# ducha-aiki/affnet

Hardware: AMD Instinct MI355X
Metric: keypoints/sec (detect+AffNet+OriNet+HardNet) per image, 2000 kp @1024x768 (higher is better)
Workload: dtype f32

## Files before the change

affnet_amd/SparseImgRepresenter.py:

```python
import ctypes as C

import torch
import torch.nn as nn

from . import _lib, engine
from ._lib import lib, check, ptr
from .architectures import _HipPatchNet
from .HandCraftedModules import AffineShapeEstimator, OrientationDetector, _HipHandCrafted
from .HardNet import HardTFeatNet
from .pytorch_sift import SIFTNet

_FOLLOW = (SIFTNet, HardTFeatNet)


class ScaleSpaceAffinePatchExtractor(nn.Module):
    def __init__(self, border=16, num_features=500, patch_size=32, mrSize=3.0, nlevels=3, num_Baum_iters=0,
                 init_sigma=1.6, th=None, RespNet=None, OriNet=None, AffNet=None, arith="fp32"):
        super(ScaleSpaceAffinePatchExtractor, self).__init__()
        self.arith = arith
        _lib.arith_code(arith)
        self.mrSize, self.PS, self.b = mrSize, patch_size, border
        self.num, self.nlevels = num_features, nlevels
        self.num_Baum_iters, self.init_sigma = num_Baum_iters, init_sigma
        self.th = th
        if th is not None:
            self.num = -1
        else:
            self.th = 0
        self.RespNet = RespNet
        if not 1 <= nlevels <= 6:
            raise NotImplementedError("nlevels must be 1..6 (levels per octave = nlevels + 2 <= 8)")
        self.OriNet = OriNet if OriNet is not None else OrientationDetector(patch_size=19)
        self.AffNet = AffNet if AffNet is not None else AffineShapeEstimator(patch_size=19)
        self.scale_pyr = self.sigmas = self.pix_dists = None
        self._ctx = None
        self._ctx_key = None
        self._fctx = self._fctx_key = self._pyr_ctx = None
        self.last_ids = None
        self.max_keep = 16384
        self.raw_div = 4
        self.lazy_shape_rows = -1

    def _context(self, x, allow_batch=False):
        engine.require_cuda(x, "image")
        if x.dim() != 4 or x.size(1) != 1 or x.size(0) < 1 or (x.size(0) != 1 and not allow_batch):
            raise ValueError("expected a (1,1,H,W) image; forward() is batch-size-1 like the reference "
                             "(HandCraftedModules.py:283-284) - use enqueue()/run_batch() for (B,1,H,W) batches")
        pre = int(1.5 * self.num) if self.num_Baum_iters > 0 else self.num
        key = (x.size(0), x.size(2), x.size(3), x.device, pre, self.num, float(self.th), self.mrSize, self.b, self.init_sigma,
               self.nlevels, self.max_keep, self.num_Baum_iters, self.raw_div, self.lazy_shape_rows)
        if self._ctx is not None and self._ctx_key == key and self._ctx.arith != _lib.arith_code(self.arith):
            self._ctx.set_arith(self.arith)
        if self._ctx is None or self._ctx_key != key:
            self._ctx = engine.Context(x.size(2), x.size(3), x.device, self.nlevels, self.init_sigma, self.b, self.mrSize,
                                       float(self.th), self.num, pre, self.max_keep, batch=x.size(0), baum_iters=self.num_Baum_iters, raw_div=self.raw_div,
                                       lazy_shape_rows=self.lazy_shape_rows, arith=self.arith)
            self._ctx_key = key
        return self._ctx

    def _publish_pyramid(self, ctx):
        self._pyr_ctx = ctx
        self.scale_pyr = ctx.pyramid_views()
        self.sigmas = [list(s) for s in ctx.plan.sigmas]
        self.pix_dists = [list(p) for p in ctx.plan.pix_dists]

    def _response_pyramid(self, ctx, img):
        dev = img.device
        st = engine.stream_of(dev)
        check(lib.affnet_pyramid_build(ctx.handle, ptr(img), st), ctx.handle, "affnet_pyramid_build")
        stride = lib.affnet_pyramid_image_stride(ctx.handle)
        base = lib.affnet_pyramid_level_offset(ctx.handle, 0, 0)
        resp = torch.zeros(ctx.batch * stride, dtype=torch.float32, device=dev)
        with torch.no_grad():
            for b in range(ctx.batch):
                pyr = ctx.pyramid_views(b)
                for o, (h, w) in enumerate(ctx.plan.sizes):
                    for l in range(ctx.plan.levels_per_octave):
                        off = b * stride + lib.affnet_pyramid_level_offset(ctx.handle, o, l) - base
                        r = self.RespNet(pyr[o][l], ctx.plan.sigmas[o][l])
                        resp[off:off + h * w].copy_(r.reshape(-1).to(dev, torch.float32))
        return resp

    @staticmethod
    def _native(slot):
        return slot is None or isinstance(slot, (_HipPatchNet, _HipHandCrafted))

    def enqueue(self, x, do_ori=False, desc=None, det_stream=None, input_ready=None):
        ctx = self._context(x, allow_batch=True)
        dev = x.device
        if not (self._native(self.AffNet) and self._native(self.OriNet)):
            raise NotImplementedError("the fused path needs the native AffNetFast / OriNetFast slots (foreign slots: forward())")
        img = x.contiguous().float()
        B, F = x.size(0), ctx.cap_final
        lafs = torch.empty(B, F, 2, 3, dtype=torch.float32, device=dev)
        resp = torch.empty(B, F, dtype=torch.float32, device=dev)
        ids = torch.empty(B, F, 3, dtype=torch.int32, device=dev)
        count = torch.zeros(B, dtype=torch.int32, device=dev)
        dsc = torch.empty(B, F, 128, dtype=torch.float32, device=dev) if desc is not None else None
        nets = self._nets(dev, do_ori, desc)
        follow = isinstance(desc, _FOLLOW)
        if isinstance(desc, HardTFeatNet):
            desc.check_usable()
        fused_dsc = None if follow else dsc
        if self.RespNet is not None:
            rmaps = self._response_pyramid(ctx, img)
            check(lib.affnet_detect_image_responses(ctx.handle, ptr(rmaps), engine.stream_of(dev)), ctx.handle, "affnet_detect_image_responses")
            rc = lib.affnet_describe_detected(ctx.handle, C.byref(nets), int(bool(do_ori)), ptr(lafs), ptr(resp), ptr(ids), ptr(fused_dsc),
                                              ptr(count), engine.stream_of(dev))
            check(rc, ctx.handle, "affnet_describe_detected")
        elif det_stream is None:
            rc = lib.affnet_extract_features(ctx.handle, C.byref(nets), ptr(img), int(bool(do_ori)), ptr(lafs), ptr(resp), ptr(ids),
                                             ptr(fused_dsc), ptr(count), engine.stream_of(dev))
            check(rc, ctx.handle, "affnet_extract_features")
        else:
            cur = torch.cuda.current_stream(dev)
            if input_ready is None:
                det_stream.wait_stream(cur)
            elif input_ready is not False:
                det_stream.wait_event(input_ready)
            if getattr(self, "_busy", None) is not None:
                det_stream.wait_event(self._busy)
            rc = lib.affnet_detect_image(ctx.handle, ptr(img), C.c_void_p(det_stream.cuda_stream))
            check(rc, ctx.handle, "affnet_detect_image")
            ev = torch.cuda.Event()
            ev.record(det_stream)
            cur.wait_event(ev)
            rc = lib.affnet_describe_detected(ctx.handle, C.byref(nets), int(bool(do_ori)), ptr(lafs), ptr(resp), ptr(ids), ptr(fused_dsc),
                                              ptr(count), engine.stream_of(dev))
            check(rc, ctx.handle, "affnet_describe_detected")
            self._busy = torch.cuda.Event()
            self._busy.record(cur)
        if follow:
            self._desc_follow(ctx, desc, lafs, count, dsc)
            if det_stream is not None:
                self._busy = torch.cuda.Event()
                self._busy.record(torch.cuda.current_stream(dev))
        if B == 1:
            lafs, resp, ids, dsc = lafs[0], resp[0], ids[0], (None if dsc is None else dsc[0])
        return {"LAFs": lafs, "responses": resp, "ids": ids, "descriptors": dsc, "count": count, "overflow": ctx.counter_view(0), "_img": img}

    def _desc_follow(self, ctx, desc, lafs, count, dsc):
        dev, (B, F) = lafs.device, lafs.shape[:2]
        st = engine.stream_of(dev)
        lvl = torch.empty(B, F, 3, dtype=torch.int32, device=dev)
        norm = torch.empty(B, F, 2, 3, dtype=torch.float32, device=dev)
        check(lib.affnet_level_select(ctx.handle, ptr(lafs), ptr(count), F, desc.PS, ptr(lvl), ptr(norm), st), ctx.handle, "affnet_level_select")
        if isinstance(desc, HardTFeatNet):
            floats = lib.affnet_tfeat_scratch_floats(B * F)
            cached = getattr(self, "_tfeat_scratch", None)
            if cached is None or cached.device != dev or cached.numel() < floats:
                cached = self._tfeat_scratch = torch.empty(floats, dtype=torch.float32, device=dev)
            check(lib.affnet_tfeat_forward_pyr(ctx.handle, ptr(desc.packed_weights(dev)), ptr(norm), ptr(lvl), ptr(count), F, ptr(dsc), ptr(cached), st),
                  ctx.handle, "affnet_tfeat_forward_pyr")
            return
        check(lib.affnet_sift_forward_pyr(ctx.handle, ptr(norm), ptr(lvl), ptr(count), F, ptr(desc.window(dev)), float(desc.clipval), ptr(dsc), st),
              ctx.handle, "affnet_sift_forward_pyr")

    def _nets(self, dev, do_ori, desc):
        nets = _lib.Nets()
        if self.num_Baum_iters > 0:
            if isinstance(self.AffNet, _HipHandCrafted):
                nets.h_baumberg_window = C.cast(self.AffNet.window(), C.c_void_p)
            else:
                nets.d_affnet = self.AffNet.packed_weights(dev).data_ptr()
        if do_ori:
            if isinstance(self.OriNet, _HipHandCrafted):
                nets.h_orientation_window = C.cast(self.OriNet.window(), C.c_void_p)
            else:
                nets.d_orinet = self.OriNet.packed_weights(dev).data_ptr()
        nets.d_hardnet = desc.packed_weights(dev).data_ptr() if desc is not None and not isinstance(desc, _FOLLOW) else None
        return nets

    def capture(self, x, do_ori=False, desc=None):
        if isinstance(desc, _FOLLOW):
            raise NotImplementedError("graph capture covers the fused C call (HardNet descriptors or none); the SIFT and HardTFeat descriptors "
                                      "follow it as further launches - use enqueue() / run()")
        return CapturedPath(self, x, do_ori, desc)

    def run_batch(self, x, do_ori=False, desc=None):
        r = self.enqueue(x, do_ori=do_ori, desc=desc)
        ctx = self._ctx
        ctx.read_counts(allow_empty=True)
        cnt = r["count"].cpu().tolist()
        if x.size(0) == 1:
            r = {k: (v.unsqueeze(0) if isinstance(v, torch.Tensor) and k not in ("count", "overflow", "_img") else v) for k, v in r.items()}
        out = []
        for b, n in enumerate(cnt):
            dsc = r["descriptors"]
            out.append({"LAFs": r["LAFs"][b, :n], "responses": r["responses"][b, :n], "ids": r["ids"][b, :n],
                        "descriptors": None if dsc is None else dsc[b, :n]})
        return out

    def run(self, x, do_ori=False, desc=None):
        if x.dim() == 4 and x.size(0) != 1:
            raise ValueError("run() is for a single (1,1,H,W) image; use run_batch() for (B,1,H,W) batches")
        r = self.enqueue(x, do_ori=do_ori, desc=desc)
        ctx = self._ctx
        self._publish_pyramid(ctx)
        n = int(ctx.read_counts()[1])
        self.last_ids = r["ids"][:n]
        dsc = r["descriptors"]
        return {"LAFs": r["LAFs"][:n], "responses": r["responses"][:n], "ids": r["ids"][:n],
                "descriptors": None if dsc is None else dsc[:n]}

    def _frames_context(self, x, n_max):
        engine.require_cuda(x, "image")
        if x.dim() != 4 or x.size(1) != 1 or x.size(0) < 1:
            raise ValueError("expected a (B,1,H,W) image batch")
        budget = self.num if (0 < self.num < n_max and self.num_Baum_iters > 0) else n_max
        key = (x.size(0), x.size(2), x.size(3), x.device, n_max, budget, self.mrSize, self.b, self.init_sigma, self.nlevels, self.num_Baum_iters,
               self.raw_div, self.lazy_shape_rows)
        if self._fctx is not None and self._fctx_key == key and self._fctx.arith != _lib.arith_code(self.arith):
            self._fctx.set_arith(self.arith)
        if self._fctx is None or self._fctx_key != key:
            self._fctx = engine.Context(x.size(2), x.size(3), x.device, self.nlevels, self.init_sigma, self.b, self.mrSize, float(self.th), budget, n_max,
                                        self.max_keep, batch=x.size(0), baum_iters=self.num_Baum_iters, raw_div=self.raw_div,
                                        lazy_shape_rows=self.lazy_shape_rows, arith=self.arith)
            self._fctx_key = key
        return self._fctx

    def enqueue_frames(self, x, LAFs, responses=None, counts=None, do_ori=True, desc=None):
        if not (self._native(self.AffNet) and self._native(self.OriNet)):
            raise NotImplementedError("the fused path needs the native AffNetFast / OriNetFast slots (foreign slots: getAffineShape / getOrientation)")
        engine.require_cuda(x, "image")
        engine.require_cuda(LAFs, "LAFs")
        dev, B = x.device, x.size(0)
        fr = LAFs.contiguous().float()
        if fr.dim() == 3:
            fr = fr.unsqueeze(0)
        if fr.dim() != 4 or fr.size(0) != B or tuple(fr.shape[2:]) != (2, 3):
            raise ValueError("LAFs must be (n,2,3) for one image or (B,n_max,2,3) for a (B,1,H,W) batch, got %s" % (tuple(LAFs.shape),))
        n_max = fr.size(1)
        if n_max == 0:
            fr, responses, counts, n_max = torch.zeros(B, 1, 2, 3, dtype=torch.float32, device=dev), None, [0] * B, 1
        rin = None
        if responses is not None:
            engine.require_cuda(responses, "responses")
            rin = responses.contiguous().float().view(B, n_max)
        cin = None
        if counts is not None:
            cin = counts if isinstance(counts, torch.Tensor) else torch.tensor(list(counts), dtype=torch.int32)
            cin = cin.to(dev, torch.int32).contiguous().view(B)
        ctx = self._frames_context(x, n_max)
        img = x.contiguous().float()
        F = ctx.cap_final
        lafs = torch.empty(B, F, 2, 3, dtype=torch.float32, device=dev)
        resp = torch.empty(B, F, dtype=torch.float32, device=dev)
        ids = torch.empty(B, F, 3, dtype=torch.int32, device=dev)
        count = torch.zeros(B, dtype=torch.int32, device=dev)
        dsc = torch.empty(B, F, 128, dtype=torch.float32, device=dev) if desc is not None else None
        nets = self._nets(dev, do_ori, desc)
        follow = isinstance(desc, _FOLLOW)
        if isinstance(desc, HardTFeatNet):
            desc.check_usable()
        rc = lib.affnet_describe_frames(ctx.handle, C.byref(nets), ptr(img), ptr(fr), ptr(rin), ptr(cin), n_max, int(bool(do_ori)), ptr(lafs), ptr(resp),
                                        ptr(ids), None if follow else ptr(dsc), ptr(count), engine.stream_of(dev))
        check(rc, ctx.handle, "affnet_describe_frames")
        if follow:
            self._desc_follow(ctx, desc, lafs, count, dsc)
        self._publish_pyramid(ctx)
        if B == 1:
            lafs, resp, ids, dsc = lafs[0], resp[0], ids[0], (None if dsc is None else dsc[0])
        return {"LAFs": lafs, "responses": resp, "ids": ids, "descriptors": dsc, "count": count, "overflow": ctx.counter_view(0), "_img": img,
                "_frames": (fr, rin, cin)}

    def describe_frames(self, x, LAFs, responses=None, counts=None, do_ori=True, desc=None):
        r = self.enqueue_frames(x, LAFs, responses=responses, counts=counts, do_ori=do_ori, desc=desc)
        ctx = self._fctx
        dsc = r["descriptors"]
        if x.size(0) == 1:
            n = int(ctx.read_counts()[1])
            self.last_ids = r["ids"][:n]
            return {"LAFs": r["LAFs"][:n], "responses": r["responses"][:n], "ids": r["ids"][:n], "descriptors": None if dsc is None else dsc[:n]}
        ctx.read_counts(allow_empty=True)
        return [{"LAFs": r["LAFs"][b, :n], "responses": r["responses"][b, :n], "ids": r["ids"][b, :n],
                 "descriptors": None if dsc is None else dsc[b, :n]} for b, n in enumerate(r["count"].cpu().tolist())]

    def _pyramid_ctx(self):
        ctx = self._pyr_ctx
        if ctx is None or self.scale_pyr is None:
            raise RuntimeError("call forward() / run() first: the pyramid of the last image is reused (stateful like the reference)")
        if ctx.batch != 1:
            raise RuntimeError("getAffineShape / getOrientation work on the pyramid of a single image")
        return ctx

    def _shape_stage(self, ctx, resp, lafs, ids, cnt, n):
        dev, st = lafs.device, engine.stream_of(lafs.device)
        P, F = ctx.cap_pre, ctx.cap_final
        PS = self.AffNet.PS
        patches = torch.empty(n, 1, PS, PS, dtype=torch.float32, device=dev)

        def shape_pass(frames):
            check(lib.affnet_pyr_grid_sample(ctx.handle, ptr(frames), ptr(ids), ptr(cnt), n, PS, ptr(patches), st), ctx.handle,
                  "affnet_pyr_grid_sample")
            with torch.no_grad():
                a = torch.cat([self.AffNet(patches[s:s + 256], {}) for s in range(0, n, 256)], 0)
            full = torch.zeros(P, 2, 2, dtype=torch.float32, device=dev)
            full[:n] = a.to(dev, torch.float32)
            return full
        A = shape_pass(lafs)
        if self.num_Baum_iters > 1:
            frames = torch.empty(P, 2, 3, dtype=torch.float32, device=dev)
            for _ in range(1, self.num_Baum_iters):
                check(lib.affnet_shape_iterate(ctx.handle, None, ptr(A), ptr(lafs), ptr(cnt), 0, ptr(frames), st), ctx.handle, "affnet_shape_iterate")
                Ai = shape_pass(frames)
                check(lib.affnet_shape_iterate(ctx.handle, ptr(Ai), ptr(A), ptr(lafs), ptr(cnt), 1, ptr(frames), st), ctx.handle, "affnet_shape_iterate")
        r2 = torch.empty(F, dtype=torch.float32, device=dev)
        l2 = torch.empty(F, 2, 3, dtype=torch.float32, device=dev)
        i2 = torch.empty(F, 3, dtype=torch.int32, device=dev)
        c2 = torch.zeros(1, dtype=torch.int32, device=dev)
        check(lib.affnet_shape_filter_select(ctx.handle, ptr(resp), ptr(lafs), ptr(ids), ptr(A), ptr(cnt), ptr(r2), ptr(l2),
                                             ptr(i2), ptr(c2), st), ctx.handle, "affnet_shape_filter_select")
        return r2, l2, i2, c2, int(c2.item())

    def _orientation_stage(self, ctx, lafs, ids, cnt, n):
        dev, st = lafs.device, engine.stream_of(lafs.device)
        PS = self.OriNet.PS
        patches = torch.empty(n, 1, PS, PS, dtype=torch.float32, device=dev)
        if n:
            check(lib.affnet_pyr_grid_sample(ctx.handle, ptr(lafs), ptr(ids), ptr(cnt), n, PS, ptr(patches), st), ctx.handle,
                  "affnet_pyr_grid_sample")
        with torch.no_grad():
            ang = self.OriNet(patches)
        if ang.dim() <= 2:
            c, s = torch.cos(ang).view(-1, 1, 1), torch.sin(ang).view(-1, 1, 1)
            ang = torch.cat([torch.cat([c, s], 2), torch.cat([-s, c], 2)], 1)
        R = ang.to(dev, torch.float32).contiguous()
        if n:
            check(lib.affnet_apply_rotation(ctx.handle, ptr(lafs), ptr(R), ptr(cnt), n, st), ctx.handle, "affnet_apply_rotation")

    @staticmethod
    def _frame_rows(ctx, LAFs, pyr_idxs, level_idxs, cap):
        engine.require_cuda(LAFs, "LAFs")
        dev, n = LAFs.device, LAFs.size(0)
        if n > cap:
            raise ValueError("%d frames, the context of the last forward() holds %d rows" % (n, cap))
        lafs = torch.zeros(cap, 2, 3, dtype=torch.float32, device=dev)
        lafs[:n] = LAFs.float()
        ids = torch.zeros(cap, 3, dtype=torch.int32, device=dev)
        ids[:n, 0] = torch.as_tensor(pyr_idxs).to(dev).view(-1).to(torch.int32)
        ids[:n, 1] = torch.as_tensor(level_idxs).to(dev).view(-1).to(torch.int32)
        ids[:n, 2] = torch.arange(n, dtype=torch.int32, device=dev)
        return lafs, ids, torch.full((1,), n, dtype=torch.int32, device=dev), n

    def getAffineShape(self, final_resp, LAFs, final_pyr_idxs, final_level_idxs, num_features=0):
        ctx = self._pyramid_ctx()
        if self.num_Baum_iters <= 0:
            raise ValueError("getAffineShape needs num_Baum_iters > 0 (the reference's loop body never runs otherwise, SparseImgRepresenter.py:127)")
        if num_features != self.num and not (num_features <= 0 and self.num <= 0):
            raise ValueError("num_features = %d: the context of the last forward() is sized for the extractor's own budget (%d)" % (num_features, self.num))
        lafs, ids, cnt, n = self._frame_rows(ctx, LAFs, final_pyr_idxs, final_level_idxs, ctx.cap_pre)
        resp = torch.zeros(ctx.cap_pre, dtype=torch.float32, device=lafs.device)
        resp[:n] = final_resp.to(lafs.device, torch.float32).view(-1)
        resp, lafs, ids, cnt, n = self._shape_stage(ctx, resp, lafs, ids, cnt, n)
        self.last_ids = ids[:n]
        return resp[:n], lafs[:n], ids[:n, 0].long(), ids[:n, 1].long()

    def getOrientation(self, LAFs, final_pyr_idxs, final_level_idxs):
        ctx = self._pyramid_ctx()
        lafs, ids, cnt, n = self._frame_rows(ctx, LAFs, final_pyr_idxs, final_level_idxs, LAFs.size(0))
        self._orientation_stage(ctx, lafs, ids, cnt, n)
        return lafs

    def _staged(self, x, do_ori):
        ctx = self._context(x)
        dev, st = x.device, engine.stream_of(x.device)
        img = x.contiguous().float()
        P = ctx.cap_pre
        rmaps = None
        if self.RespNet is not None:
            rmaps = self._response_pyramid(ctx, img)
        else:
            check(lib.affnet_pyramid_build(ctx.handle, ptr(img), st), ctx.handle, "affnet_pyramid_build")
        self._publish_pyramid(ctx)
        resp = torch.empty(P, dtype=torch.float32, device=dev)
        lafs = torch.empty(P, 2, 3, dtype=torch.float32, device=dev)
        ids = torch.empty(P, 3, dtype=torch.int32, device=dev)
        cnt = torch.zeros(1, dtype=torch.int32, device=dev)
        if rmaps is not None:
            check(lib.affnet_detect_responses(ctx.handle, ptr(rmaps), ptr(resp), ptr(lafs), ptr(ids), ptr(cnt), st), ctx.handle,
                  "affnet_detect_responses")
        else:
            check(lib.affnet_detect(ctx.handle, ptr(resp), ptr(lafs), ptr(ids), ptr(cnt), st), ctx.handle, "affnet_detect")
        n = int(cnt.item())
        ctx.read_counts()
        if self.num_Baum_iters > 0:
            resp, lafs, ids, cnt, n = self._shape_stage(ctx, resp, lafs, ids, cnt, n)
        if do_ori:
            self._orientation_stage(ctx, lafs, ids, cnt, n)
        out = torch.empty_like(lafs)
        check(lib.affnet_scale_lafs(ctx.handle, ptr(lafs), ptr(out), ptr(cnt), lafs.size(0), x.size(3), x.size(2), 0, st), ctx.handle,
              "affnet_scale_lafs")
        self.last_ids = ids[:n]
        return out[:n], resp[:n]

    def forward(self, x, do_ori=False):
        aff_native = self.num_Baum_iters == 0 or self._native(self.AffNet)
        ori_native = (not do_ori) or self._native(self.OriNet)
        if aff_native and ori_native:
            r = self.run(x, do_ori=do_ori)
            return r["LAFs"], r["responses"]
        return self._staged(x, do_ori)

    def extract_patches_from_pyr(self, dLAFs, PS=41):
        if self._ctx is None or self.scale_pyr is None:
            raise RuntimeError("call forward() first: the pyramid of the last image is reused (stateful like the reference)")
        ctx = self._ctx
        if ctx.batch != 1:
            raise RuntimeError("extract_patches_from_pyr works on the pyramid of a single-image forward()")
        engine.require_cuda(dLAFs, "dLAFs")
        dev, st = dLAFs.device, engine.stream_of(dLAFs.device)
        lafs = dLAFs.contiguous().float()
        n = lafs.size(0)
        out = torch.empty(n, 1, PS, PS, dtype=torch.float32, device=dev)
        if n == 0:
            return out
        ids = torch.empty(n, 3, dtype=torch.int32, device=dev)
        norm = torch.empty(n, 2, 3, dtype=torch.float32, device=dev)
        check(lib.affnet_level_select(ctx.handle, ptr(lafs), None, n, PS, ptr(ids), ptr(norm), st), ctx.handle, "affnet_level_select")
        check(lib.affnet_pyr_grid_sample(ctx.handle, ptr(norm), ptr(ids), None, n, PS, ptr(out), st), ctx.handle, "affnet_pyr_grid_sample")
        self.last_level_ids = ids
        return out


class CapturedPath(object):
    def __init__(self, det, x, do_ori, desc):
        if not (det._native(det.AffNet) and det._native(det.OriNet)) or det.RespNet is not None:
            raise NotImplementedError("graph capture needs the native slots (foreign slots run Python between the stages)")
        ctx = det._context(x, allow_batch=True)
        dev = x.device
        self.det, self.ctx, self.do_ori, self.desc = det, ctx, bool(do_ori), desc
        B, F = x.size(0), ctx.cap_final
        self.image = x.contiguous().float().clone()
        self.out = {"LAFs": torch.empty(B, F, 2, 3, dtype=torch.float32, device=dev), "responses": torch.empty(B, F, dtype=torch.float32, device=dev),
                    "ids": torch.empty(B, F, 3, dtype=torch.int32, device=dev), "count": torch.zeros(B, dtype=torch.int32, device=dev),
                    "descriptors": torch.empty(B, F, 128, dtype=torch.float32, device=dev) if desc is not None else None}
        self._nets = det._nets(dev, do_ori, desc)
        self._mods = [m for m in (det.AffNet, det.OriNet if do_ori else None, desc) if m is not None and hasattr(m, "packed_weights")]
        self._blobs = [m.packed_weights(dev) for m in self._mods]
        self._stamps = [m._weights_stamp() for m in self._mods]
        self._arith = ctx.arith
        self._stream = torch.cuda.Stream(device=dev)
        torch.cuda.synchronize(dev)
        o = self.out
        check(lib.affnet_graph_capture_extract(ctx.handle, C.byref(self._nets), ptr(self.image), int(self.do_ori), ptr(o["LAFs"]), ptr(o["responses"]),
                                               ptr(o["ids"]), ptr(o["descriptors"]), ptr(o["count"]), C.c_void_p(self._stream.cuda_stream)),
              ctx.handle, "affnet_graph_capture_extract")

    def launch(self, x=None, check_weights=True):
        if check_weights:
            for m, stamp in zip(self._mods, self._stamps):
                if m._weights_stamp() != stamp:
                    raise RuntimeError("the weights of %s changed after capture(): the graph holds the old packed weights - capture again" % type(m).__name__)
        if self.ctx.arith != self._arith:
            raise RuntimeError("the arithmetic mode of the extractor changed after capture(): the graph runs the mode it was captured with - capture again")
        if x is not None:
            self.image.copy_(x, non_blocking=True)
        busy = getattr(self.det, "_busy", None)
        if busy is not None:
            torch.cuda.current_stream(self.image.device).wait_event(busy)
        check(lib.affnet_graph_launch(self.ctx.handle, engine.stream_of(self.image.device)), self.ctx.handle, "affnet_graph_launch")
        out = dict(self.out, overflow=self.ctx.counter_view(0), _img=self.image)
        if self.image.size(0) == 1:
            return {k: (v[0] if (v is not None and k not in ("count", "overflow", "_img")) else v) for k, v in out.items()}
        return out

    def run(self, x=None, check_weights=True):
        if self.image.size(0) != 1:
            raise ValueError("run() is for single images; use launch() for batches")
        r = self.launch(x, check_weights=check_weights)
        self.det._publish_pyramid(self.ctx)
        n = int(self.ctx.read_counts()[1])
        dsc = r["descriptors"]
        return {"LAFs": r["LAFs"][:n], "responses": r["responses"][:n], "ids": r["ids"][:n], "descriptors": None if dsc is None else dsc[:n]}


def get_geometry_and_descriptors(img, det, desc, do_ori=True):
    from .HardNet import HardNet
    if isinstance(desc, (HardNet,) + _FOLLOW) and det._native(det.AffNet) and det._native(det.OriNet):
        r = det.run(img, do_ori=do_ori, desc=desc)
        return r["LAFs"], r["descriptors"]
    with torch.no_grad():
        LAFs, resp = det(img, do_ori=do_ori)
        patches = det.extract_patches_from_pyr(LAFs, PS=32)
        return LAFs, desc(patches)
```

affnet_amd/_lib.py:

```python
import ctypes as C
import os

_HERE = os.path.dirname(os.path.abspath(__file__))
LIB_PATH = os.environ.get("AFFNET_HIP_LIB") or os.path.join(_HERE, "libaffnet_hip.so")
PROBES_LIB_PATH = os.path.join(_HERE, "libaffnet_hip_probes.so")

MAX_OCTAVES, MAX_LEVELS, MAX_TAPS = 16, 8, 37
NET_AFFNET, NET_ORINET, NET_HARDNET, NET_AFFNET_FULLCONV = 0, 1, 2, 3
ARITH_FP32_MFMA, ARITH_FP32_SPLIT3, ARITH_FP32_SPLIT2H = 0, 1, 2
ARITH_NAMES = {"fp32": ARITH_FP32_MFMA, "fp32_mfma": ARITH_FP32_MFMA, "fp32_split3": ARITH_FP32_SPLIT3, "split3": ARITH_FP32_SPLIT3,
               "fp32_split2h": ARITH_FP32_SPLIT2H, "split2h": ARITH_FP32_SPLIT2H}


def arith_code(arith):
    if arith is None:
        return ARITH_FP32_MFMA
    if isinstance(arith, str):
        if arith.lower() not in ARITH_NAMES:
            raise ValueError("arith must be one of %s" % sorted(ARITH_NAMES))
        return ARITH_NAMES[arith.lower()]
    if int(arith) not in (ARITH_FP32_MFMA, ARITH_FP32_SPLIT3, ARITH_FP32_SPLIT2H):
        raise ValueError("arith must be AFFNET_ARITH_FP32_MFMA (0), AFFNET_ARITH_FP32_SPLIT3 (1) or AFFNET_ARITH_FP32_SPLIT2H (2)")
    return int(arith)
OK, ERR_INVALID, ERR_HIP, ERR_CAPACITY, ERR_EMPTY = 0, -1, -2, -3, -4


class Config(C.Structure):
    _fields_ = [
        ("height", C.c_int32), ("width", C.c_int32), ("n_octaves", C.c_int32), ("levels_per_octave", C.c_int32),
        ("oct_h", C.c_int32 * MAX_OCTAVES), ("oct_w", C.c_int32 * MAX_OCTAVES),
        ("level_sigma", (C.c_float * MAX_LEVELS) * MAX_OCTAVES),
        ("level_sigma4", (C.c_float * MAX_LEVELS) * MAX_OCTAVES),
        ("level_sigma_px", (C.c_double * MAX_LEVELS) * MAX_OCTAVES),
        ("first_blur_taps", C.c_int32), ("first_blur", C.c_float * (MAX_TAPS * MAX_TAPS)),
        ("level_blur_taps", C.c_int32 * MAX_LEVELS),
        ("level_blur", (C.c_float * (MAX_TAPS * MAX_TAPS)) * MAX_LEVELS),
        ("level_blur0_taps", C.c_int32 * MAX_LEVELS),
        ("level_blur0", (C.c_float * (MAX_TAPS * MAX_TAPS)) * MAX_LEVELS),
        ("lazy_shape_rows", C.c_int32),
        ("onepass", C.c_int32),
        ("mr_size", C.c_float), ("threshold", C.c_float),
        ("num_features", C.c_int32), ("num_prefilter", C.c_int32),
        ("max_raw_per_octave_div", C.c_int32), ("max_keep", C.c_int32), ("batch", C.c_int32), ("baum_iters", C.c_int32),
        ("arith", C.c_int32),
    ]


class Nets(C.Structure):
    _fields_ = [("d_affnet", C.c_void_p), ("d_orinet", C.c_void_p), ("d_hardnet", C.c_void_p),
                ("h_orientation_window", C.c_void_p), ("h_baumberg_window", C.c_void_p)]


_P, _I, _SZ = C.c_void_p, C.c_int, C.c_size_t
SYMBOLS = {
    "affnet_config_fill": (_I, [C.POINTER(Config), _I, _I, _I, C.c_double, _I, C.c_double, C.c_double, _I, _I, _I, _I]),
    "affnet_ctx_create": (_I, [C.POINTER(_P), _I, C.POINTER(Config)]),
    "affnet_ctx_destroy": (None, [_P]),
    "affnet_last_error": (C.c_char_p, [_P]),
    "affnet_version": (C.c_char_p, []),
    "affnet_set_arith": (_I, [_P, _I]),
    "affnet_get_arith": (_I, [_P]),
    "affnet_workspace_bytes": (_SZ, [_P]),
    "affnet_bind_workspace": (_I, [_P, _P, _SZ]),
    "affnet_pyramid_level_offset": (C.c_int64, [_P, _I, _I]),
    "affnet_pyramid_image_stride": (C.c_int64, [_P]),
    "affnet_batch": (_I, [_P]),
    "affnet_capacity_prefilter": (_I, [_P]),
    "affnet_capacity_final": (_I, [_P]),
    "affnet_gauss_blur": (_I, [_P, _P, _P, _I, _I, C.POINTER(C.c_float), _I, _P]),
    "affnet_pyramid_build": (_I, [_P, _P, _P]),
    "affnet_hessian_response": (_I, [_P, _P, _P, _I, _I, C.c_float, _P]),
    "affnet_detect": (_I, [_P, _P, _P, _P, _P, _P]),
    "affnet_detect_responses": (_I, [_P, _P, _P, _P, _P, _P, _P]),
    "affnet_laf_grid_sample": (_I, [_P, _P, _I, _I, _P, _I, _I, _P, _P]),
    "affnet_pyr_grid_sample": (_I, [_P, _P, _P, _P, _I, _I, _P, _P]),
    "affnet_cnn32_packed_floats": (_SZ, [_I]),
    "affnet_cnn32_winograd_offset": (C.c_int64, [_I, _I]),
    "affnet_cnn32_pack_weights": (_I, [_I, C.POINTER(_P), C.POINTER(_P), C.POINTER(_P), _P, _P, _P, _P, _P]),
    "affnet_cnn32_forward": (_I, [_P, _I, _P, _P, _P, _I, _P, _P, _P]),
    "affnet_cnn32_forward_pyr": (_I, [_P, _I, _P, _P, _P, _P, _I, _P, _P, _P]),
    "affnet_local_norm": (_I, [_P, _P, _P, _I, _I, _P]),
    "affnet_fullconv_scratch_bytes": (_SZ, [_I, _I]),
    "affnet_fullconv_forward": (_I, [_P, _P, _P, _I, _I, _P, _P, _P]),
    "affnet_nms2d": (_I, [_P, _P, _P, _I, _I, C.c_float, _P]),
    "affnet_shape_filter_select": (_I, [_P, _P, _P, _P, _P, _P, _P, _P, _P, _P, _P]),
    "affnet_apply_rotation": (_I, [_P, _P, _P, _P, _I, _P]),
    "affnet_scale_lafs": (_I, [_P, _P, _P, _P, _I, _I, _I, _I, _P]),
    "affnet_lafs_to_ellipses": (_I, [_P, _P, _P, _I, _P, _P]),
    "affnet_ellipses_to_lafs": (_I, [_P, _P, _P, _I, _P, _P]),
    "affnet_level_select": (_I, [_P, _P, _P, _I, _I, _P, _P, _P]),
    "affnet_handcrafted_forward": (_I, [_P, _I, _P, _I, _P, _P, _P, _P]),
    "affnet_handcrafted_forward_pyr": (_I, [_P, _I, _P, _P, _P, _I, _P, _P, _P]),
    "affnet_sift_host_window": (_I, [_I, C.POINTER(C.c_float)]),
    "affnet_sift_forward": (_I, [_P, _P, _I, _P, C.c_float, _P, _P]),
    "affnet_sift_forward_pyr": (_I, [_P, _P, _P, _P, _I, _P, C.c_float, _P, _P]),
    "affnet_tfeat_packed_floats": (_SZ, []),
    "affnet_tfeat_pack_weights": (_I, [_P, _P, _P, _P, _P, _P, _P]),
    "affnet_tfeat_scratch_floats": (_SZ, [_I]),
    "affnet_tfeat_forward": (_I, [_P, _P, _P, _P, _I, _P, _P, _P]),
    "affnet_tfeat_forward_pyr": (_I, [_P, _P, _P, _P, _P, _I, _P, _P, _P]),
    "affnet_match_scratch_bytes": (_SZ, [_I, _I]),
    "affnet_distance_matrix": (_I, [_P, _P, _I, _P, _I, _I, _P, _P, _P]),
    "affnet_match_snn": (_I, [_P, _P, _I, _P, _I, _I, C.c_float, _P, _P, _P, _P, _P, _P, _P]),
    "affnet_reproject_lafs": (_I, [_P, _P, _I, C.POINTER(C.c_float), _P, _P]),
    "affnet_centre_nn": (_I, [_P, _P, _I, _P, _I, _P, _P, _P]),
    "affnet_extract_features": (_I, [_P, C.POINTER(Nets), _P, _I, _P, _P, _P, _P, _P, _P]),
    "affnet_detect_image": (_I, [_P, _P, _P]),
    "affnet_detect_image_responses": (_I, [_P, _P, _P]),
    "affnet_detect_image_onepass": (_I, [_P, _P, _P, _P]),
    "affnet_detect_image_onepass_responses": (_I, [_P, _P, _P, _P]),
    "affnet_detected_list": (_I, [_P, _P, _P, _P, _P, _P]),
    "affnet_load_frames": (_I, [_P, _P, _I, _P, _P, _P, _I, _I, _P]),
    "affnet_describe_frames": (_I, [_P, C.POINTER(Nets), _P, _P, _P, _P, _I, _I, _P, _P, _P, _P, _P, _P]),
    "affnet_shape_iterate": (_I, [_P, _P, _P, _P, _P, _I, _P, _P]),
    "affnet_affmap_offset": (C.c_int64, [_P, _I]),
    "affnet_affmap_image_stride": (C.c_int64, [_P]),
    "affnet_describe_detected": (_I, [_P, C.POINTER(Nets), _I, _P, _P, _P, _P, _P, _P]),
    "affnet_graph_capture_extract": (_I, [_P, C.POINTER(Nets), _P, _I, _P, _P, _P, _P, _P, _P]),
    "affnet_graph_launch": (_I, [_P, _P]),
    "affnet_profile_enable": (_I, [_P, _I]),
    "affnet_profile_read": (_I, [_P, C.POINTER(C.c_double * 8), C.POINTER(C.c_int32)]),
    "affnet_read_counts": (_I, [_P, C.POINTER(C.c_int32 * 4), _P]),
    "affnet_counter_offset": (C.c_int64, [_P, _I]),
    "affnet_counter_stride": (C.c_int64, [_P]),
    "affnet_host_base_grid": (_I, [_I, C.POINTER(C.c_float)]),
}

DEBUG_SYMBOLS = {
    "affnet_cnn32_debug_timing": (_I, [_P, _P]),
    "affnet_cnn32_debug_layer": (_I, [_P, _I, _P, _P, _I, _P, _P]),
    "affnet_cnn32_debug_winograd_u": (_I, [_P, _I, _P, _I, _P, _P]),
    "affnet_selftest_mfma": (_I, [_P, _P, _P, _P]),
    "affnet_debug_split3_variant": (_I, [_P, _I]),
}

PROBE_SYMBOLS = {
    "affnet_cnn32_probe": (_I, [_P, _I, _I, _I, _I, _P, _P]),
    "affnet_split3_gemm": (_I, [_P, _P, _I, _I, _I, _I, _P, _P]),
    "affnet_split3_rate": (_I, [_I, _I, _I, _P, _P]),
    "affnet_debug_stream": (_I, [_P, _P, _SZ, _I, _I, _I, _P]),
}


class AffnetHipError(RuntimeError):
    pass


class AffnetEmptyError(AffnetHipError):
    """AFFNET_ERR_EMPTY: no image of the call produced a detection (the reference raises in torch.cat([]),
    SparseImgRepresenter.py:100)."""


def _load():
    if not os.path.isfile(LIB_PATH):
        if os.path.basename(LIB_PATH) == os.path.basename(PROBES_LIB_PATH):
            raise ImportError("affnet_amd: %s is missing - the tools under tools/ need the probe build of the library: "
                              "AFFNET_PROBES=1 bash affnet_amd/csrc/build.sh" % LIB_PATH)
        raise ImportError(
            "affnet_amd: %s is missing - the HIP extension is the only implementation of this path "
            "(no CPU fallback). Build it: bash affnet_amd/csrc/build.sh" % LIB_PATH)
    lib = C.CDLL(LIB_PATH)
    for table in (SYMBOLS, DEBUG_SYMBOLS):
        for name, (res, args) in table.items():
            fn = getattr(lib, name)
            fn.restype, fn.argtypes = res, args
    for name, (res, args) in PROBE_SYMBOLS.items():
        if hasattr(lib, name):
            fn = getattr(lib, name)
            fn.restype, fn.argtypes = res, args
    return lib


lib = _load()


def check(rc, ctx=None, what=""):
    if rc != OK:
        msg = lib.affnet_last_error(ctx).decode() if ctx else ""
        if rc == ERR_EMPTY:
            raise AffnetEmptyError("%s: %s" % (what or "libaffnet_hip call", msg))
        raise AffnetHipError("%s failed (code %d): %s" % (what or "libaffnet_hip call", rc, msg))


def ptr(t):
    return None if t is None else C.c_void_p(t.data_ptr())


def current_stream(device):
    import torch
    return C.c_void_p(torch.cuda.current_stream(device).cuda_stream)
```

affnet_amd/csrc/cnn32.hip:

```cpp
#include "common.h"

static void aff_fill_pyr_src(const affnet_ctx* ctx, PyrSrc* s) {
    memset(s, 0, sizeof(*s));
    if (ctx->ws) aff_fill_pyr_table(ctx, &s->t);
    aff_base_grid(32, s->base);
}

static int cnn_check(affnet_ctx* ctx, const CnnCall& c, int* rows) {
    *rows = 0;
    if (c.kind < 0 || c.kind > 2) return aff_fail(ctx, AFFNET_ERR_INVALID, "cnn32: unknown net kind %d", c.kind);
    if (!c.packed || !c.out || c.n_max < 0 || (!c.patches && (!c.lafs || !c.ids))) return aff_fail(ctx, AFFNET_ERR_INVALID, "cnn32: null argument");
    if (!c.patches && !ctx->ws) return aff_fail(ctx, AFFNET_ERR_INVALID, "cnn32: sampling from the pyramid needs a bound workspace");
    if (c.dbg_layer < 0 && !c.scratch)
        return aff_fail(ctx, AFFNET_ERR_INVALID, "cnn32: d_scratch is required (HardNet n*(8192+512) floats, AffNet / OriNet n*144 floats)");
    if (c.dbg_layer >= 0 && ctx->arith != AFFNET_ARITH_FP32_MFMA)
        return aff_fail(ctx, AFFNET_ERR_INVALID, "cnn32: layer dumps exist for AFFNET_ARITH_FP32_MFMA only (context is in arithmetic mode %d)", ctx->arith);
    if (c.n_max == 0) return AFFNET_OK;
    if (c.kind == AFFNET_NET_HARDNET && c.n_max > 65535)
        return aff_fail(ctx, AFFNET_ERR_INVALID, "cnn32: n_max=%d (HardNet head: max 65535 rows per image)", c.n_max);
    const int row_count = c.row_count < 0 ? c.n_max - c.row_begin : c.row_count;
    if (c.row_begin < 0 || row_count < 0 || c.row_begin + row_count > c.n_max) return aff_fail(ctx, AFFNET_ERR_INVALID, "cnn32: bad row window");
    *rows = row_count;
    return AFFNET_OK;
}

int aff_arith_index(const affnet_ctx* ctx) {
    return ctx->arith == AFFNET_ARITH_FP32_SPLIT2H ? 2 : (ctx->arith == AFFNET_ARITH_FP32_SPLIT3 ? 1 : 0);
}

static int trunk_launch(affnet_ctx* ctx, const CnnCall& c, const NetLayout& L, dim3 grid) {
    CnnArgs a;
    a.packed = c.packed; a.off = to_offsets(L, ctx->arith);
    a.wino_u = nullptr;
    if (c.kind == AFFNET_NET_ORINET && ctx->arith == AFFNET_ARITH_FP32_MFMA) {
        const int rc = aff_wino_derive_u(ctx, c.kind, c.packed, L, c.st, &a.wino_u);
        if (rc) return rc;
    }
    a.patches = c.patches; a.lafs = c.lafs; a.ids = c.ids; a.count = c.count; a.n_max = c.n_max;
    a.out = (c.dbg_layer < 0) ? c.scratch : c.out;
    a.dbg_layer = c.dbg_layer; a.dbg_out = c.dbg_out; a.dbg_time = ctx->dbg_time;
    a.row_begin = c.row_begin; a.skip_cnt = c.skip_cnt; a.skip_n = c.skip_n;
    a.shape_cnt = (c.fuse && c.shape_op) ? c.fuse->cnt : nullptr; a.shape_op = c.shape_op;
    a.s3_alt = ctx->split3_variant;
    PyrSrc ps;
    aff_fill_pyr_src(ctx, &ps);
    static_assert(AFFNET_NET_AFFNET == 0 && AFFNET_NET_ORINET == 1 && AFFNET_NET_HARDNET == 2, "trunk getter order");
    static TrunkKernel (*const trunk_of[3])(int, bool) = {aff_trunk_affnet, aff_trunk_orinet, aff_trunk_hardnet};
    hipLaunchKernelGGL(trunk_of[c.kind](aff_arith_index(ctx), a.dbg_time || c.dbg_layer >= 0), grid, dim3(512), 0, c.st, a, ps);
    AFF_LAUNCH_CHECK(ctx);
    return AFFNET_OK;
}

static int cnn_launch(affnet_ctx* ctx, const CnnCall& c) {
    int rows;
    int rc = cnn_check(ctx, c, &rows);
    if (rc || rows == 0) return rc;
    const NetLayout L = net_layout(c.kind);
    const int B = c.patches ? 1 : ctx->B;
    rc = trunk_launch(ctx, c, L, dim3(rows, B));
    if (rc) return rc;
    if (c.dbg_layer < 0 && c.kind != AFFNET_NET_HARDNET) {
        rc = c.kind == AFFNET_NET_AFFNET ? aff_finish_affnet(ctx, c, L, rows, B) : aff_finish_orinet(ctx, c, L, rows, B);
        if (rc) return rc;
    }
    if (c.mark_head) aff_prof_mark(ctx, 7, c.st);
    if (c.dbg_layer < 0 && c.kind == AFFNET_NET_HARDNET) return aff_hardnet_head(ctx, c, L, B);
    return AFFNET_OK;
}

extern "C" int affnet_cnn32_forward(affnet_ctx* ctx, int net_kind, const float* d_packed, const float* d_patches, const int32_t* d_count,
                                    int n_max, float* d_out, float* d_scratch, void* stream) {
    AFF_DEVICE(ctx);
    if (!ctx || !d_patches) return aff_fail(ctx, AFFNET_ERR_INVALID, "cnn32_forward: null argument");
    CnnCall c;
    c.kind = net_kind; c.packed = d_packed; c.patches = d_patches; c.count = d_count; c.n_max = n_max; c.out = d_out; c.scratch = d_scratch; c.st = (hipStream_t)stream;
    return cnn_launch(ctx, c);
}

extern "C" int affnet_cnn32_forward_pyr(affnet_ctx* ctx, int net_kind, const float* d_packed, const float* d_lafs, const int32_t* d_ids,
                                        const int32_t* d_count, int n_max, float* d_out, float* d_scratch, void* stream) {
    AFF_DEVICE(ctx);
    if (!ctx) return AFFNET_ERR_INVALID;
    CnnCall c;
    c.kind = net_kind; c.packed = d_packed; c.lafs = d_lafs; c.ids = d_ids; c.count = d_count; c.n_max = n_max; c.out = d_out; c.scratch = d_scratch; c.st = (hipStream_t)stream;
    return cnn_launch(ctx, c);
}

int aff_affnet_filter_rows(affnet_ctx* ctx, const float* packed, const float* resp, const float* lafs, const int32_t* ids, const int32_t* count,
                           float* out, float* scratch, int row_begin, int row_count, bool lazy, int shape_op, hipStream_t st) {
    ShapeFuse sf;
    sf.resp = resp; sf.lafs = lafs; sf.key = ctx->st_key; sf.good = ctx->st_good; sf.cnt = ctx->cnt;
    CnnCall c;
    c.kind = AFFNET_NET_AFFNET; c.packed = packed; c.lafs = lafs; c.ids = ids; c.count = count; c.n_max = ctx->cap_pre; c.out = out; c.scratch = scratch; c.st = st;
    c.row_begin = row_begin; c.row_count = row_count;
    c.skip_cnt = lazy ? ctx->cnt : nullptr; c.skip_n = ctx->cfg.num_features;
    c.fuse = &sf; c.shape_op = shape_op;
    return cnn_launch(ctx, c);
}

int aff_orinet_rotate(affnet_ctx* ctx, const float* packed, float* lafs, const int32_t* ids, const int32_t* count, int n_max, float* out, float* scratch,
                      hipStream_t st, const DenormSel* denorm) {
    CnnCall c;
    c.kind = AFFNET_NET_ORINET; c.packed = packed; c.lafs = lafs; c.ids = ids; c.count = count; c.n_max = n_max; c.out = out; c.scratch = scratch; c.st = st;
    c.rot_lafs = lafs; c.denorm = denorm;
    return cnn_launch(ctx, c);
}

int aff_hardnet_forward_pyr_marked(affnet_ctx* ctx, const float* packed, const float* lafs, const int32_t* ids, const int32_t* count,
                                   int n_max, float* out, float* scratch, hipStream_t st) {
    CnnCall c;
    c.kind = AFFNET_NET_HARDNET; c.packed = packed; c.lafs = lafs; c.ids = ids; c.count = count; c.n_max = n_max; c.out = out; c.scratch = scratch; c.st = st;
    c.mark_head = true;
    return cnn_launch(ctx, c);
}

extern "C" int affnet_debug_split3_variant(affnet_ctx* ctx, int bits) {
    if (!ctx) return AFFNET_ERR_INVALID;
    ctx->split3_variant = bits;
    return AFFNET_OK;
}

extern "C" int affnet_cnn32_debug_timing(affnet_ctx* ctx, unsigned long long* d_stamps) {
    if (!ctx) return AFFNET_ERR_INVALID;
    ctx->dbg_time = d_stamps;
    return AFFNET_OK;
}

extern "C" int affnet_cnn32_debug_layer(affnet_ctx* ctx, int net_kind, const float* d_packed, const float* d_patch, int layer, float* d_out,
                                        void* stream) {
    AFF_DEVICE(ctx);
    if (!ctx || !d_patch || !d_out || layer < 0 || layer > 5) return aff_fail(ctx, AFFNET_ERR_INVALID, "cnn32_debug_layer: bad argument");
    CnnCall c;
    c.kind = net_kind; c.packed = d_packed; c.patches = d_patch; c.n_max = 1; c.out = d_out; c.st = (hipStream_t)stream;
    c.dbg_layer = layer; c.dbg_out = d_out;
    return cnn_launch(ctx, c);
}

extern "C" int affnet_cnn32_debug_winograd_u(affnet_ctx* ctx, int net_kind, const float* d_packed, int layer, float* d_out, void* stream) {
    AFF_DEVICE(ctx);
    if (!ctx || !d_packed || !d_out || (net_kind != AFFNET_NET_AFFNET && net_kind != AFFNET_NET_ORINET) || (layer != 1 && layer != 3 && layer != 5))
        return aff_fail(ctx, AFFNET_ERR_INVALID, "cnn32_debug_winograd_u: AffNet / OriNet, layer 1, 3 or 5");
    const float* u;
    const int rc = aff_wino_derive_u(ctx, net_kind, d_packed, net_layout(net_kind), (hipStream_t)stream, &u);
    if (rc) return rc;
    return aff_copy_async(ctx, d_out, u + Wino16::offset(layer), (size_t)Wino16::floats(layer) * sizeof(float), (hipStream_t)stream);
}
```

affnet_amd/csrc/cnn_heads.hip:

```cpp
#include <stdlib.h>

#include "common.h"

#include "cnn_mfma.h"
#include "shape_filter.h"

__global__ __launch_bounds__(256) void affnet_finish_kernel(const float* __restrict__ part, const float* __restrict__ hb,
                                                            const int32_t* __restrict__ count, int n_max, float* __restrict__ out, int row_begin,
                                                            int row_end, const int32_t* __restrict__ skip_cnt, int skip_n, ShapeFuse sf) {
    const int row = row_begin + blockIdx.x * 256 + threadIdx.x;
    const int n_img = count ? min(count[blockIdx.y], n_max) : n_max;
    const int n = min(n_img, row_end);
    const bool skip = lazy_skip(skip_cnt, skip_n, blockIdx.y);
    const size_t pidx = (size_t)blockIdx.y * n_max + row;
    if (sf.key) {
        if (blockIdx.x == 0 && threadIdx.x == 0)
            sf.cnt[(size_t)blockIdx.y * CNT_TOTAL + CNT_AFF_EVAL] = skip ? min(n_img, row_begin) : min(n_img, row_end);
        if (skip && row < n) { sf.key[pidx] = 0.0f; sf.good[pidx] = 0; }
    }
    if (row >= n || skip) return;
    float* o = out + 4 * pidx;
    const f32x4* pp = reinterpret_cast<const f32x4*>(part + pidx * HEAD_PART_AFF);
    f32x4 r[8];
#pragma unroll
    for (int w = 0; w < 8; ++w) r[w] = pp[w];
    const f32x4 s = ((r[0] + r[1]) + (r[2] + r[3])) + ((r[4] + r[5]) + (r[6] + r[7]));
    const float x0 = tanhf(s.x + hb[0]), x1 = tanhf(s.y + hb[1]), x2 = tanhf(s.z + hb[2]);
    const float a00 = 1.0f + x0, a01 = 0.0f * x0, a10 = x1, a11 = 1.0f + x2;
    const float det = sqrtf(fabsf(a00 * a11 - a10 * a01 + 1e-10f));
    const float b2a2 = sqrtf(a01 * a01 + a00 * a00);
    const float o0 = b2a2 / det, o1 = 0.0f * det, o2 = (a11 * a01 + a10 * a00) / (b2a2 * det), o3 = det / b2a2;
    o[0] = o0; o[1] = o1; o[2] = o2; o[3] = o3;
    if (sf.key) {
        const size_t bi = blockIdx.y;
        aff_shape_filter_row(sf.resp + bi * n_max, sf.lafs + bi * n_max * 6, o0, o1, o2, o3, row, sf.key + bi * n_max, sf.good + bi * n_max,
                             sf.cnt + bi * CNT_TOTAL);
    }
}

__global__ __launch_bounds__(256) void orinet_finish_kernel(const float* __restrict__ part, const float* __restrict__ hb,
                                                            const int32_t* __restrict__ count, int n_max, float* __restrict__ out, int row_begin,
                                                            int row_end, float* __restrict__ rot_lafs, DenormSel ds) {
    const int row = row_begin + blockIdx.x * 4 + (threadIdx.x >> 6), lane = threadIdx.x & 63;
    const int n = min(count ? min(count[blockIdx.y], n_max) : n_max, row_end);
    if (row >= n) {
        if (ds.out_px && row < n_max && lane < 6) ds.out_px[6 * ((size_t)blockIdx.y * n_max + row) + lane] = 0.f;
        return;
    }
    const size_t pidx = (size_t)blockIdx.y * n_max + row;
    const float* pp = part + pidx * HEAD_PART_ORI;
    float th = 0.f;
    if (lane < 18) {
        float p[8];
#pragma unroll
        for (int w = 0; w < 8; ++w) p[w] = pp[w * 18 + lane];
        float r = 0.f;
#pragma unroll
        for (int w = 0; w < 8; w += 2) r += p[w] + p[w + 1];
        th = tanhf(r + hb[lane >= 9 ? 1 : 0]);
    }
    float t0 = 0.f, t1 = 0.f;
#pragma unroll
    for (int q = 0; q < 9; ++q) { t0 += __shfl(th, q, 64); t1 += __shfl(th, 9 + q, 64); }
    if (lane != 0 && !(rot_lafs && ds.out_px)) return;
    const float yv = t0 / 9.0f, xv = t1 / 9.0f;
    const float ang = atan2f(yv + 1e-8f, xv + 1e-8f);
    const float sn = sinf(ang), cs = cosf(ang);
    float* o = out + 4 * pidx;
    if (lane == 0) { o[0] = cs; o[1] = sn; o[2] = -sn; o[3] = cs; }
    if (rot_lafs) {
        float* L = rot_lafs + 6 * pidx;
        const float l00 = L[0], l01 = L[1], l10 = L[3], l11 = L[4], lx = L[2], ly = L[5];
        const float r0 = fmaf(l01, -sn, l00 * cs), r1 = fmaf(l01, cs, l00 * sn), r3 = fmaf(l11, -sn, l10 * cs), r4 = fmaf(l11, cs, l10 * sn);
        if (ds.out_px)
            aff_denorm_level_row_wave(lane, r0, r1, lx, r3, r4, ly, ds.c_a, ds.c_x, ds.c_y, ds.ps, ds.lt, ds.ca, ds.cx, ds.cy, ds.out_px + 6 * pidx, ds.ids + 3 * pidx,
                                      ds.lafs_norm + 6 * pidx);
        if (lane == 0) { L[0] = r0; L[1] = r1; L[3] = r3; L[4] = r4; }
    }
}

template <int MP>
__global__ __launch_bounds__(256, 2) void hardnet_head_kernel(const float* __restrict__ trunk, const float* __restrict__ Bw,
                                                              const int32_t* __restrict__ count, int n_max, float* __restrict__ partial) {
    constexpr int MI = MP / 16;
    constexpr int NA = MP * HEAD_KC / 4 / 256;
    __shared__ __attribute__((aligned(16))) float As[MP * HEAD_AS];
    const int n = count ? min(count[blockIdx.z], n_max) : n_max;
    const int p0 = blockIdx.x * MP;
    if (p0 >= n) return;
    const size_t rows_total = (size_t)gridDim.z * n_max;
    const int kbeg = blockIdx.y * (HEAD_K / HEAD_KSPLIT);
    const int tid = threadIdx.x, wave = tid >> 6, lane = tid & 63;
    const int m = lane & 15, kq = lane >> 4;
    const __amdgpu_buffer_rsrc_t rA = weight_rsrc(trunk + (size_t)blockIdx.z * n_max * HEAD_K, n * HEAD_K);
    const __amdgpu_buffer_rsrc_t rB = weight_rsrc(Bw, HEAD_K * 128);
    int offA[NA];
#pragma unroll
    for (int r = 0; r < NA; ++r) {
        const int f = tid + 256 * r, row = f >> 5, c4 = f & 31;
        offA[r] = ((p0 + row) * HEAD_K + 4 * c4) * 4;
    }
    const int offB = ((kq * 128) + wave * 32 + m) * 16;
    const unsigned a_addr = lds_byte_addr(As) + (m * HEAD_AS + 4 * kq) * 4;
    f32x4 acc[MI][2], stage[NA];
#pragma unroll
    for (int i = 0; i < MI; ++i)
#pragma unroll
        for (int j = 0; j < 2; ++j) acc[i][j] = (f32x4){0.f, 0.f, 0.f, 0.f};
#pragma unroll
    for (int r = 0; r < NA; ++r) stage[r] = buf_read4(rA, offA[r], kbeg * 4);
#pragma unroll 1
    for (int k0 = kbeg; k0 < kbeg + HEAD_K / HEAD_KSPLIT; k0 += HEAD_KC) {
        __syncthreads();
#pragma unroll
        for (int r = 0; r < NA; ++r) {
            const int f = tid + 256 * r, row = f >> 5, c4 = f & 31;
            *reinterpret_cast<f32x4*>(&As[row * HEAD_AS + 4 * c4]) = stage[r];
        }
        __syncthreads();
        if (k0 + HEAD_KC < kbeg + HEAD_K / HEAD_KSPLIT) {
#pragma unroll
            for (int r = 0; r < NA; ++r) stage[r] = buf_read4(rA, offA[r], (k0 + HEAD_KC) * 4);
        }
        f32x4 fa[2][MI], fb[2][2];
#pragma unroll
        for (int i = 0; i < MI; ++i) fa[0][i] = lds_read4(a_addr + i * 16 * HEAD_AS * 4);
#pragma unroll
        for (int j = 0; j < 2; ++j) fb[0][j] = buf_read4(rB, offB + j * 256, k0 * 512);
#pragma unroll
        for (int g = 0; g < HEAD_KC / 16; ++g) {
            const int cur = g & 1, nxt = cur ^ 1;
            if (g + 1 < HEAD_KC / 16) {
#pragma unroll
                for (int i = 0; i < MI; ++i) fa[nxt][i] = lds_read4(a_addr + i * 16 * HEAD_AS * 4 + (g + 1) * 64);
#pragma unroll
                for (int j = 0; j < 2; ++j) fb[nxt][j] = buf_read4(rB, offB + j * 256, (k0 + 16 * (g + 1)) * 512);
            }
#pragma unroll
            for (int s4 = 0; s4 < 4; ++s4)
#pragma unroll
                for (int i = 0; i < MI; ++i)
#pragma unroll
                    for (int j = 0; j < 2; ++j)
                        acc[i][j] = __builtin_amdgcn_mfma_f32_16x16x4f32(fa[cur][i][s4], fb[cur][j][s4], acc[i][j], 0, 0, 0);
        }
    }
    const int g = lane >> 4;
    float* dst = partial + ((size_t)blockIdx.y * rows_total + (size_t)blockIdx.z * n_max) * 128;
#pragma unroll
    for (int i = 0; i < MI; ++i)
#pragma unroll
        for (int r = 0; r < 4; ++r) {
            const int row = p0 + 16 * i + 4 * g + r;
            if (row >= n) continue;
            dst[(size_t)row * 128 + wave * 32 + m] = acc[i][0][r];
            dst[(size_t)row * 128 + wave * 32 + 16 + m] = acc[i][1][r];
        }
}

#define HEAD_S3_ROWB (HEAD_KC * 6 + 16)
template <int MP, int TERMS = 3>
__global__ __launch_bounds__(256, 2) void hardnet_head_s3_kernel(const float* __restrict__ trunk, const float* __restrict__ Bw3,
                                                                 const int32_t* __restrict__ count, int n_max, float* __restrict__ partial) {
    constexpr int MI = MP / 16;
    constexpr int NA = MP * HEAD_KC / 4 / 256;
    __shared__ __attribute__((aligned(16))) char As[MP * HEAD_S3_ROWB];
    const int n = count ? min(count[blockIdx.z], n_max) : n_max;
    const int p0 = blockIdx.x * MP;
    if (p0 >= n) return;
    const size_t rows_total = (size_t)gridDim.z * n_max;
    const int kbeg = blockIdx.y * (HEAD_K / HEAD_KSPLIT);
    const int tid = threadIdx.x, wave = tid >> 6, lane = tid & 63;
    const int m = lane & 15, kq = lane >> 4;
    const __amdgpu_buffer_rsrc_t rA = weight_rsrc(trunk + (size_t)blockIdx.z * n_max * HEAD_K, n * HEAD_K);
    const __amdgpu_buffer_rsrc_t rB = weight_rsrc(Bw3, HEAD_K * 128 * TERMS / 2);
    int offA[NA];
#pragma unroll
    for (int r = 0; r < NA; ++r) {
        const int f = tid + 256 * r, row = f >> 5, c4 = f & 31;
        offA[r] = ((p0 + row) * HEAD_K + 4 * c4) * 4;
    }
    const int offB = ((kq * 128) + wave * 32 + m) * 16;
    const unsigned a_addr = lds_byte_addr(reinterpret_cast<const float*>(As)) + m * HEAD_S3_ROWB + kq * 48;
    f32x4 acc[MI][2], stage[NA];
#pragma unroll
    for (int i = 0; i < MI; ++i)
#pragma unroll
        for (int j = 0; j < 2; ++j) acc[i][j] = (f32x4){0.f, 0.f, 0.f, 0.f};
#pragma unroll
    for (int r = 0; r < NA; ++r) stage[r] = buf_read4(rA, offA[r], kbeg * 4);
#pragma unroll 1
    for (int k0 = kbeg; k0 < kbeg + HEAD_K / HEAD_KSPLIT; k0 += HEAD_KC) {
        __syncthreads();
#pragma unroll
        for (int r = 0; r < NA; ++r) {
            const int f = tid + 256 * r, row = f >> 5, c4 = f & 31;
            char* dst = As + row * HEAD_S3_ROWB + (c4 >> 1) * 48 + (c4 & 1) * 8;
            split_store4<TERMS>(dst, stage[r]);
        }
        __syncthreads();
        if (k0 + HEAD_KC < kbeg + HEAD_K / HEAD_KSPLIT) {
#pragma unroll
            for (int r = 0; r < NA; ++r) stage[r] = buf_read4(rA, offA[r], (k0 + HEAD_KC) * 4);
        }
        bf16x8 fb[2][TERMS][2];
        auto load_b = [&](int buf, int ks) {
#pragma unroll
            for (int t = 0; t < TERMS; ++t)
#pragma unroll
                for (int j = 0; j < 2; ++j)
                    fb[buf][t][j] = __builtin_bit_cast(bf16x8, __builtin_amdgcn_raw_buffer_load_b128(rB, offB + j * 256, ((ks * TERMS + t) * 4 * 128) * 16, 0));
        };
        load_b(0, k0 >> 5);
#pragma unroll
        for (int s = 0; s < HEAD_KC / 32; ++s) {
            const int cur = s & 1;
            if (s + 1 < HEAD_KC / 32) load_b(cur ^ 1, (k0 >> 5) + s + 1);
            bf16x8 fa[MI][TERMS];
#pragma unroll
            for (int i = 0; i < MI; ++i)
#pragma unroll
                for (int t = 0; t < TERMS; ++t) fa[i][t] = __builtin_bit_cast(bf16x8, lds_read4(a_addr + i * 16 * HEAD_S3_ROWB + s * 192 + t * 16));
            constexpr int NPAIR = TERMS == 3 ? 6 : 3;
            constexpr int TA3[6] = {0, 0, 0, 1, 1, 2}, TB3[6] = {0, 1, 2, 0, 1, 0}, TA2[3] = {0, 0, 1}, TB2[3] = {0, 1, 0};
#pragma unroll
            for (int q = 0; q < NPAIR; ++q)
#pragma unroll
                for (int i = 0; i < MI; ++i)
#pragma unroll
                    for (int j = 0; j < 2; ++j)
                        acc[i][j] = split_mfma<TERMS>(fa[i][TERMS == 3 ? TA3[q] : TA2[q]], fb[cur][TERMS == 3 ? TB3[q] : TB2[q]][j], acc[i][j]);
        }
    }
    if constexpr (TERMS == 2) {
        const float osc = Bw3[(size_t)HEAD_K * 128];
#pragma unroll
        for (int i = 0; i < MI; ++i)
#pragma unroll
            for (int j = 0; j < 2; ++j) acc[i][j] *= osc;
    }
    const int g = lane >> 4;
    float* dst = partial + ((size_t)blockIdx.y * rows_total + (size_t)blockIdx.z * n_max) * 128;
#pragma unroll
    for (int i = 0; i < MI; ++i)
#pragma unroll
        for (int r = 0; r < 4; ++r) {
            const int row = p0 + 16 * i + 4 * g + r;
            if (row >= n) continue;
            dst[(size_t)row * 128 + wave * 32 + m] = acc[i][0][r];
            dst[(size_t)row * 128 + wave * 32 + 16 + m] = acc[i][1][r];
        }
}

__global__ __launch_bounds__(256) void hardnet_finish_kernel(const float* __restrict__ partial, const float* __restrict__ bias,
                                                             const int32_t* __restrict__ count, int n_max, float* __restrict__ out) {
    const int n = count ? min(count[blockIdx.y], n_max) : n_max;
    const int lrow = blockIdx.x * 4 + (threadIdx.x >> 6), lane = threadIdx.x & 63;
    if (lrow >= n_max) return;
    const size_t rows_total = (size_t)gridDim.y * n_max, row = (size_t)blockIdx.y * n_max + lrow;
    if (lrow >= n) { out[row * 128 + lane] = 0.0f; out[row * 128 + 64 + lane] = 0.0f; return; }
    float v0 = 0.f, v1 = 0.f;
#pragma unroll
    for (int s = 0; s < HEAD_KSPLIT; ++s) {
        const float* p = partial + ((size_t)s * rows_total + row) * 128;
        v0 += p[lane]; v1 += p[64 + lane];
    }
    v0 += bias[lane]; v1 += bias[64 + lane];
    const float tot = wave_sum(v0 * v0 + v1 * v1);
    const float nrm = sqrtf(tot + 1e-8f);
    out[row * 128 + lane] = v0 / nrm;
    out[row * 128 + 64 + lane] = v1 / nrm;
}

int aff_finish_affnet(affnet_ctx* ctx, const CnnCall& c, const NetLayout& L, int rows, int B) {
    ShapeFuse sf;
    memset(&sf, 0, sizeof(sf));
    if (c.fuse) sf = *c.fuse;
    hipLaunchKernelGGL(affnet_finish_kernel, dim3(aff_cdiv(rows, 256), B), dim3(256), 0, c.st, c.scratch, c.packed + L.head_b, c.count, c.n_max, c.out,
                       c.row_begin, c.row_begin + rows, c.skip_cnt, c.skip_n, sf);
    AFF_LAUNCH_CHECK(ctx);
    return AFFNET_OK;
}

int aff_finish_orinet(affnet_ctx* ctx, const CnnCall& c, const NetLayout& L, int rows, int B) {
    DenormSel ds;
    memset(&ds, 0, sizeof(ds));
    if (c.denorm && c.rot_lafs) ds = *c.denorm;
    hipLaunchKernelGGL(orinet_finish_kernel, dim3(aff_cdiv(rows, 4), B), dim3(256), 0, c.st, c.scratch, c.packed + L.head_b, c.count, c.n_max, c.out,
                       c.row_begin, c.row_begin + rows, c.rot_lafs, ds);
    AFF_LAUNCH_CHECK(ctx);
    return AFFNET_OK;
}

int aff_hardnet_head(affnet_ctx* ctx, const CnnCall& c, const NetLayout& L, int B) {
    const int n_max = c.n_max;
    float* partial = c.scratch + (size_t)B * n_max * HEAD_K;
    int mp = (aff_cdiv(n_max, 64) * HEAD_KSPLIT * B >= 256) ? 64 : ((aff_cdiv(n_max, 32) * HEAD_KSPLIT * B >= 256) ? 32 : 16);
    if (const char* e = getenv("AFFNET_HEAD_MP")) { const int v = atoi(e); if (v == 16 || v == 32 || v == 64) mp = v; }
    static void (*const heads[3][3])(const float*, const float*, const int32_t*, int, float*) = {
        {hardnet_head_kernel<64>, hardnet_head_kernel<32>, hardnet_head_kernel<16>},
        {hardnet_head_s3_kernel<64, 3>, hardnet_head_s3_kernel<32, 3>, hardnet_head_s3_kernel<16, 3>},
        {hardnet_head_s3_kernel<64, 2>, hardnet_head_s3_kernel<32, 2>, hardnet_head_s3_kernel<16, 2>}};
    const int ai = aff_arith_index(ctx);
    const float* hw = c.packed + (ai == 2 ? L.head_h2 : (ai == 1 ? L.head_s3 : L.head_w));
    hipLaunchKernelGGL(heads[ai][mp == 64 ? 0 : (mp == 32 ? 1 : 2)], dim3(aff_cdiv(n_max, mp), HEAD_KSPLIT, B), dim3(256), 0, c.st, c.scratch, hw, c.count,
                       n_max, partial);
    AFF_LAUNCH_CHECK(ctx);
    hipLaunchKernelGGL(hardnet_finish_kernel, dim3(aff_cdiv(n_max, 4), B), dim3(256), 0, c.st, partial, c.packed + L.head_b, c.count, n_max, c.out);
    AFF_LAUNCH_CHECK(ctx);
    return AFFNET_OK;
}

__global__ void mfma_selftest_kernel(const float* __restrict__ A, const float* __restrict__ B, float* __restrict__ out) {
    const int lane = threadIdx.x, m = lane & 15, kq = lane >> 4;
    f32x4 c = {0.f, 0.f, 0.f, 0.f};
    c = __builtin_amdgcn_mfma_f32_16x16x4f32(A[m * 4 + kq], B[kq * 16 + m], c, 0, 0, 0);
#pragma unroll
    for (int r = 0; r < 4; ++r) out[(4 * kq + r) * 16 + m] = c[r];
}

extern "C" int affnet_selftest_mfma(const float* d_A, const float* d_B, float* d_out, void* stream) {
    if (!d_A || !d_B || !d_out) return AFFNET_ERR_INVALID;
    hipLaunchKernelGGL(mfma_selftest_kernel, dim3(1), dim3(64), 0, (hipStream_t)stream, d_A, d_B, d_out);
    return hipGetLastError() == hipSuccess ? AFFNET_OK : AFFNET_ERR_HIP;
}
```

affnet_amd/csrc/cnn_trunk.h:

```cpp
#pragma once
#include <math.h>

#include <type_traits>

#include "common.h"

#include "cnn_mfma.h"

template <int TM>
__device__ __forceinline__ void head_partials(const float* __restrict__ hw, const f32x4 (&bias)[1], const f32x4 (&acc)[TM][1],
                                              float* __restrict__ part, int wave, int lane) {
    constexpr int MT = 4, MG = MT / TM;
    const int mg = wave % MG, ng = wave / MG;
    const int n = lane & 15, g = lane >> 4;
    const int c4 = ng * 16 + 4 * g;
    f32x4 v[TM];
#pragma unroll
    for (int i = 0; i < TM; ++i) {
        v[i] = acc[i][0] + bias[0];
        v[i].x = fmaxf(v[i].x, 0.0f); v[i].y = fmaxf(v[i].y, 0.0f); v[i].z = fmaxf(v[i].z, 0.0f); v[i].w = fmaxf(v[i].w, 0.0f);
    }
    const __amdgpu_buffer_rsrc_t r = weight_rsrc(hw, 3 * 4096);
    f32x4 w[3][TM];
#pragma unroll
// ... 10 lines not shown
        sacc = wave_sum(sacc);
        if (lane == 0) part[wave * 4 + o] = sacc;
    }
}

#define ORI_HP 68
struct OriHeadLane {
    int mg, n, c4;
    template <int TM>
    __device__ __forceinline__ static OriHeadLane of(int wave, int lane) {
        constexpr int MT = 4, MG = MT / TM;
        const int mg = wave % MG, ng = wave / MG;
        const int n = lane & 15, g = lane >> 4;
        return {mg, n, ng * 16 + 4 * g};
    }
};
template <int TM>
__device__ __forceinline__ void ori_head_weights(const float* __restrict__ hw, const OriHeadLane& L, f32x4 (&w)[2][TM]) {
    const __amdgpu_buffer_rsrc_t r = weight_rsrc(hw, 2 * 4096);
#pragma unroll
    for (int o = 0; o < 2; ++o)
#pragma unroll
        for (int i = 0; i < TM; ++i) w[o][i] = buf_read4(r, (L.n * 64 + L.c4) * 4, (o * 4096 + (L.mg * TM + i) * 16 * 64) * 4);
}
template <int NTHR>
__device__ __forceinline__ void ori_head_zero_halo(float* act, int tid) {
    for (int e = tid; e < 36 * 16; e += NTHR) {
        const int hp = e >> 4, q4 = e & 15;
        const int y = hp < 10 ? 0 : (hp < 20 ? 9 : 1 + ((hp - 20) >> 1)), x = hp < 10 ? hp : (hp < 20 ? hp - 10 : ((hp - 20) & 1) * 9);
        *reinterpret_cast<f32x4*>(&act[(y * 10 + x) * ORI_HP + 4 * q4]) = (f32x4){0.f, 0.f, 0.f, 0.f};
    }
}
template <int TM>
__device__ __forceinline__ void ori_head_pbase(const OriHeadLane& L, int (&pbase)[TM]) {
#pragma unroll
    for (int i = 0; i < TM; ++i) {
        const int p = (L.mg * TM + i) * 16 + L.n;
        pbase[i] = ((p >> 3) * 10 + (p & 7)) * ORI_HP + L.c4;
    }
}
template <int TM>
__device__ __forceinline__ void ori_head_reduce(const f32x4 (&w)[2][TM], const int (&pbase)[TM], float* __restrict__ part, const float* act, int wave, int lane) {
    __syncthreads();
#pragma unroll
    for (int q = 0; q < 9; ++q) {
        float s0 = 0.f, s1 = 0.f;
#pragma unroll
        for (int i = 0; i < TM; ++i) {
            const f32x4 av = *reinterpret_cast<const f32x4*>(&act[pbase[i] + ((q / 3) * 10 + q % 3) * ORI_HP]);
#pragma unroll
            for (int j = 0; j < 4; ++j) { s0 = fmaf(av[j], w[0][i][j], s0); s1 = fmaf(av[j], w[1][i][j], s1); }
        }
        s0 = wave_sum(s0);
        s1 = wave_sum(s1);
        if (lane == 0) { part[wave * 18 + q] = s0; part[wave * 18 + 9 + q] = s1; }
    }
}
template <int TM, int NTHR>
__device__ __forceinline__ void head_partials_ori_lds(const float* __restrict__ hw, const f32x4 (&bias)[1], const f32x4 (&acc)[TM][1],
                                                      float* __restrict__ part, float* act, int wave, int lane, int tid) {
    constexpr int MT = 4, MG = MT / TM;
    const int mg = wave % MG, ng = wave / MG;
    const int n = lane & 15, g = lane >> 4;
    const int c4 = ng * 16 + 4 * g;
    f32x4 v[TM];
#pragma unroll
    for (int i = 0; i < TM; ++i) {
        v[i] = acc[i][0] + bias[0];
        v[i].x = fmaxf(v[i].x, 0.0f); v[i].y = fmaxf(v[i].y, 0.0f); v[i].z = fmaxf(v[i].z, 0.0f); v[i].w = fmaxf(v[i].w, 0.0f);
    }
    const __amdgpu_buffer_rsrc_t r = weight_rsrc(hw, 2 * 4096);
    f32x4 w[2][TM];
#pragma unroll
    for (int o = 0; o < 2; ++o)
#pragma unroll
        for (int i = 0; i < TM; ++i) w[o][i] = buf_read4(r, (n * 64 + c4) * 4, (o * 4096 + (mg * TM + i) * 16 * 64) * 4);
    __syncthreads();
    for (int e = tid; e < 36 * 16; e += NTHR) {
        const int hp = e >> 4, q4 = e & 15;
        const int y = hp < 10 ? 0 : (hp < 20 ? 9 : 1 + ((hp - 20) >> 1)), x = hp < 10 ? hp : (hp < 20 ? hp - 10 : ((hp - 20) & 1) * 9);
        *reinterpret_cast<f32x4*>(&act[(y * 10 + x) * ORI_HP + 4 * q4]) = (f32x4){0.f, 0.f, 0.f, 0.f};
    }
    int pbase[TM];
#pragma unroll
    for (int i = 0; i < TM; ++i) {
        const int p = (mg * TM + i) * 16 + n;
        pbase[i] = ((p >> 3) * 10 + (p & 7)) * ORI_HP + c4;
        *reinterpret_cast<f32x4*>(&act[pbase[i] + 11 * ORI_HP]) = v[i];
    }
    __syncthreads();
#pragma unroll
    for (int q = 0; q < 9; ++q) {
        float s0 = 0.f, s1 = 0.f;
#pragma unroll
        for (int i = 0; i < TM; ++i) {
            const f32x4 av = *reinterpret_cast<const f32x4*>(&act[pbase[i] + ((q / 3) * 10 + q % 3) * ORI_HP]);
#pragma unroll
            for (int j = 0; j < 4; ++j) { s0 = fmaf(av[j], w[0][i][j], s0); s1 = fmaf(av[j], w[1][i][j], s1); }
        }
        s0 = wave_sum(s0);
        s1 = wave_sum(s1);
        if (lane == 0) { part[wave * 18 + q] = s0; part[wave * 18 + 9 + q] = s1; }
    }
}

#define CNN_STAMP(k)                                                                                     \
    do {                                                                                                 \
        if (STAMPS && a.dbg_time && lane == 0) a.dbg_time[((size_t)pidx * NW + wave) * 32 + (k)] = __builtin_readcyclecounter(); \
    } while (0)

template <int CB>
struct TrunkLds {
    static constexpr int ACT = (CB / 4) * LayC0::PSG;
    static constexpr int PATCH = WP32 * WP32;
    static constexpr int RED = 256;
    static constexpr int TOTAL = ACT + PATCH + RED;
};

template <int KIND, int NW>
struct TrunkShape {
    static constexpr int CB = (KIND == AFFNET_NET_HARDNET) ? 32 : 16;
    static constexpr int NTHR = NW * 64;
    static constexpr int T1M = (CB == 16) ? 8 : 64 / NW, T1N = CB / 16;
    static constexpr int T2M = (CB == 16) ? 4 : 64 / NW, T2N = 1;
    static constexpr int T4M = (CB == 16) ? 2 : 32 / NW, T4N = 1;
    static constexpr int AREG = (NW == 8 && CB == 32) ? 128 : 48;
    static constexpr int G2 = pick_groups(CB, T2M, T2N, 32, AREG), G3 = pick_groups(2 * CB, T2M, T2N, 32, AREG);
    static constexpr int G4 = pick_groups(2 * CB, T4M, T4N, 32, AREG), G5 = pick_groups(4 * CB, T4M, T4N, 32, AREG);
};

template <int C, typename L, int NTHR>
__device__ __forceinline__ void dump_planes(const float* act, float* dst) {
    constexpr int H = L::H;
    for (int i = threadIdx.x; i < C * H * H; i += NTHR) {
        const int c = i / (H * H), r = i - c * H * H, y = r / H, x = r - y * H;
        dst[i] = act[L::at(c, y, x)];
    }
}

template <int CB>
struct SplitLays {
    typedef LayQ<16, 32, 34, CB, 0, 3> LQH;
    typedef LayQ<16, 32, 34, CB, 16, 3> LQH2;
    using LR0 = LayR<32, 32, 34, CB, 0>;
    using LR0H = LayR<16, 32, 34, CB, 0, 34>;
    using LR1 = LayR<32, 32, 34, CB, 16>;
    using LR1H = LayR<16, 32, 34, CB, 16, 34>;
    static_assert(LR0::BYTES <= TrunkLds<CB>::ACT * 4 && LR1::BYTES <= TrunkLds<CB>::ACT * 4 && LR0H::GS == LR0::GS && LR1H::GS == LR1::GS, "whole-patch split layouts");
    static_assert(LQH::BYTES <= TrunkLds<CB>::ACT * 4 && LQH2::BYTES <= TrunkLds<CB>::ACT * 4, "pre-split layouts must fit the activation buffer");
};

template <int KIND, int NW, bool STAMPS, int S3 = 0>
__global__ __launch_bounds__(NW * 64, (KIND == AFFNET_NET_HARDNET) ? NW / 4 : 4) void cnn32_trunk_kernel(CnnArgs a, PyrSrc ps) {
    static_assert(S3 == 0 || S3 == 2 || S3 == 3, "S3 = number of terms of the split arithmetic");
    using S = TrunkShape<KIND, NW>;
    constexpr int CB = S::CB, NTHR = S::NTHR;
    static_assert((CB / 4) * LayC1::PSG <= TrunkLds<CB>::ACT && (CB / 2) * LayC3::PSG <= TrunkLds<CB>::ACT, "LDS layout");
    __shared__ __attribute__((aligned(16))) float lds[TrunkLds<CB>::TOTAL];
    float* act = lds;
    float* patch = lds + TrunkLds<CB>::ACT;
    float* red = patch + TrunkLds<CB>::PATCH;
    const int n = a.count ? min(a.count[blockIdx.y], a.n_max) : a.n_max;
    const int prow = blockIdx.x + a.row_begin;
    if (KIND == AFFNET_NET_AFFNET && a.shape_cnt && blockIdx.x == 0 && threadIdx.x == 0) {
        int32_t* c = a.shape_cnt + (size_t)blockIdx.y * CNT_TOTAL;
        if (a.shape_op == 1) { c[CNT_SURVIVED] = 0; c[CNT_SURVIVED1] = 0; c[CNT_AFF_EVAL] = 0; }
        else if (a.shape_op == 2) c[CNT_SURVIVED1] = c[CNT_SURVIVED];
    }
    if (prow >= n || lazy_skip(a.skip_cnt, a.skip_n, blockIdx.y, CNT_SURVIVED)) return;
    const size_t pidx = (size_t)blockIdx.y * a.n_max + prow;
    const int tid = threadIdx.x, wave = tid >> 6, lane = tid & 63;
    if (KIND == AFFNET_NET_HARDNET) __builtin_amdgcn_s_setprio(3);
    CNN_STAMP(0);
    if (STAMPS && a.dbg_time && lane == 0) {
        a.dbg_time[((size_t)pidx * NW + wave) * 32 + 14] = __builtin_amdgcn_s_getreg((31 << 11) | 4);
        a.dbg_time[((size_t)pidx * NW + wave) * 32 + 15] = __builtin_amdgcn_s_getreg((31 << 11) | 20);
    }
    float w0[3][S::T1N];
    f32x4 bias0[S::T1N];
    conv0_load_w<NW, CB, S::T1M, S::T1N>(a.packed + a.off.w[0], a.packed + a.off.b[0], w0, bias0, wave, lane);
    f32x4 b1[1][S::T1N];
    f32x4 Ur[4];
    if constexpr (S3 == 0 && KIND == AFFNET_NET_AFFNET) prefetch_b0<NW, CB, 32, S::T1M, S::T1N, 1>(a.packed + a.off.w[1], b1, wave, lane);
    if constexpr (S3 == 0 && KIND == AFFNET_NET_ORINET) wino_prefetch_u_row<NW, CB, CB, 32, Wino16::NB1>(a.wino_u, Ur, wave, lane);

    constexpr int PPT = 1024 / NTHR;
    constexpr int RPT = 32 / PPT;
    float v[PPT];
    if (a.patches) {
        const float* src = a.patches + pidx * 1024;
#pragma unroll
        for (int q = 0; q < PPT; ++q) v[q] = src[tid + q * NTHR];
    } else {
        int o = a.ids[3 * pidx], l = a.ids[3 * pidx + 1];
        o = o < 0 ? 0 : (o >= ps.t.n_octaves ? ps.t.n_octaves - 1 : o);
        l = l < 0 ? 0 : (l >= ps.t.n_levels ? ps.t.n_levels - 1 : l);
        const float* img = ps.t.lvl[o][l] + blockIdx.y * ps.t.img_stride;
        const int h = ps.t.h[o], w = ps.t.w[o];
        const float* L = a.lafs + 6 * pidx;
        const float m = (float)(h < w ? h : w);
        const float t00 = L[0] * m, t01 = L[1] * m, t02 = L[2] * (float)w;
        const float t10 = L[3] * m, t11 = L[4] * m, t12 = L[5] * (float)h;
#pragma unroll
        for (int q = 0; q < PPT; ++q)
            v[q] = aff_sample_bilinear(img, h, w, t00, t01, t02, t10, t11, t12, ps.base[tid & 31], ps.base[(tid >> 5) + q * RPT]);
    }
    CNN_STAMP(16);
    if (tid < 4 * 33) {
        const int e = tid;
        const int y = e < 34 ? 0 : (e < 68 ? 33 : 1 + ((e - 68) >> 1)), x = e < 34 ? e : (e < 68 ? e - 34 : ((e - 68) & 1) * 33);
        patch[y * WP32 + x] = 0.0f;
    }
    if constexpr (S3 == 0) zero_halo<LayC0, NTHR>(act, CB);
    else if constexpr (S3 == 2) zero_halo_q<typename SplitLays<CB>::LR0, NTHR>(act);
    else zero_halo_q<typename SplitLays<CB>::LQH, NTHR>(act);
    float sum = 0.f;
#pragma unroll
    for (int q = 0; q < PPT; ++q) sum += v[q];
    const float mean = block_sum<NW>(sum, red) * (1.0f / 1024.0f);
    CNN_STAMP(17);
    float sq = 0.f;
#pragma unroll
    for (int q = 0; q < PPT; ++q) { v[q] -= mean; sq += v[q] * v[q]; }
    const float var = block_sum<NW>(sq, red + NW) * (1.0f / 1023.0f);
    const float sd = sqrtf(var) + 1e-7f;
    CNN_STAMP(18);
#pragma unroll
    for (int q = 0; q < PPT; ++q) patch[((tid >> 5) + q * RPT + 1) * WP32 + (tid & 31) + 1] = v[q] / sd;
    __syncthreads();
    CNN_STAMP(1);

    if constexpr (S3 == 0 && KIND == AFFNET_NET_HARDNET) {
        constexpr int T1M = S::T1M, T1N = S::T1N, T2M = S::T2M, T2N = S::T2N, T4M = S::T4M, T4N = S::T4N;
        constexpr int NB1 = (16 * 16 / 16) * (CB / 16) / NW, NB3 = (8 * 8 / 16) * (2 * CB / 16) / NW, NB5 = (4 * 4 / 16) * (4 * CB / 16) / NW;

        f32x4 Up[2][4];
        f32x4 Uw[16];
        {
            f32x4 acc[T1M][T1N];
            conv0_mfma<NW, CB, T1M, T1N>(patch, w0, bias0, acc, wave, lane);
            CNN_STAMP(19);
            store_tiles_lds<CB, LayC0, T1M, T1N, false>(act, bias0, acc, wave, lane);
            CNN_STAMP(20);
            wino_prefetch_u_pair<NW, CB, CB, 32, NB1>(a.packed + a.off.w_wino[0], Up, wave, lane);
            __syncthreads();
        }
        if (STAMPS && a.dbg_layer == 0) { dump_planes<CB, LayC0, NTHR>(act, a.dbg_out); return; }
        CNN_STAMP(2);

        f32x4 b2[S::G2][T2N];
        f32x4 bias2[T2N];
        {
            f32x4 y[NB1][4], bw[NB1];
            __builtin_amdgcn_s_setprio(0);
            conv3x3_wino_mfma_pair_rows<NW, CB, CB, LayC0, NB1>(act, a.packed + a.off.w_wino[0], Up, y, wave, lane);
            __builtin_amdgcn_s_setprio(3);
            CNN_STAMP(3);
            prefetch_b0<NW, 2 * CB, 16, T2M, T2N, S::G2>(a.packed + a.off.w[2], b2, wave, lane);
            prefetch_bias<NW, 16, T2M, T2N>(a.packed + a.off.b[2], bias2, wave, lane);
            wino_bias<NW, 32, CB, NB1>(a.packed + a.off.b[1], bw, wave, lane);
            __syncthreads();
            CNN_STAMP(21);
            zero_halo<LayC1, NTHR>(act, CB);
            wino_store_lds<CB, LayC1, NB1>(act, bw, y, wave, lane);
            CNN_STAMP(22);
            __syncthreads();
            CNN_STAMP(4);
        }
        if (STAMPS && a.dbg_layer == 1) { dump_planes<CB, LayC1, NTHR>(act, a.dbg_out); return; }

        {
            f32x4 acc[T2M][T2N];
            __builtin_amdgcn_s_setprio(0);
            conv3x3_mfma<NW, CB, 2 * CB, LayC1, 2, T2M, T2N, S::G2>(act, a.packed + a.off.w[2], b2, acc, wave, lane);
            __builtin_amdgcn_s_setprio(3);
            CNN_STAMP(5);
            wino_prefetch_u_pair<NW, 2 * CB, 2 * CB, 16, NB3>(a.packed + a.off.w_wino[1], Up, wave, lane);
            __syncthreads();
            zero_halo<LayC2, NTHR>(act, 2 * CB);
            store_tiles_lds<2 * CB, LayC2, T2M, T2N>(act, bias2, acc, wave, lane);
            __syncthreads();
            CNN_STAMP(6);
        }
        if (STAMPS && a.dbg_layer == 2) { dump_planes<2 * CB, LayC2, NTHR>(act, a.dbg_out); return; }

        f32x4 b4[S::G4][T4N];
        f32x4 bias4[T4N];
        {
            f32x4 y[NB3][4], bw[NB3];
            __builtin_amdgcn_s_setprio(0);
            conv3x3_wino_mfma_pair_rows<NW, 2 * CB, 2 * CB, LayC2, NB3>(act, a.packed + a.off.w_wino[1], Up, y, wave, lane);
            __builtin_amdgcn_s_setprio(3);
            CNN_STAMP(7);
            prefetch_b0<NW, 4 * CB, 8, T4M, T4N, S::G4>(a.packed + a.off.w[4], b4, wave, lane);
            prefetch_bias<NW, 8, T4M, T4N>(a.packed + a.off.b[4], bias4, wave, lane);
            wino_bias<NW, 16, 2 * CB, NB3>(a.packed + a.off.b[3], bw, wave, lane);
            __syncthreads();
            zero_halo<LayC3, NTHR>(act, 2 * CB);
            wino_store_lds<2 * CB, LayC3, NB3>(act, bw, y, wave, lane);
            __syncthreads();
            CNN_STAMP(8);
        }
        if (STAMPS && a.dbg_layer == 3) { dump_planes<2 * CB, LayC3, NTHR>(act, a.dbg_out); return; }

        {
            f32x4 acc[T4M][T4N];
            __builtin_amdgcn_s_setprio(0);
            conv3x3_mfma<NW, 2 * CB, 4 * CB, LayC3, 2, T4M, T4N, S::G4>(act, a.packed + a.off.w[4], b4, acc, wave, lane);
            __builtin_amdgcn_s_setprio(3);
            CNN_STAMP(9);
            wino_prefetch_u<NW, 4 * CB, 4 * CB, 8, NB5>(a.packed + a.off.w_wino[2], Uw, wave, lane);
            __syncthreads();
            zero_halo<LayC4, NTHR>(act, 4 * CB);
            store_tiles_lds<4 * CB, LayC4, T4M, T4N>(act, bias4, acc, wave, lane);
            __syncthreads();
            CNN_STAMP(10);
        }
        if (STAMPS && a.dbg_layer == 4) { dump_planes<4 * CB, LayC4, NTHR>(act, a.dbg_out); return; }

        f32x4 y[NB5][4], bw[NB5];
        __builtin_amdgcn_s_setprio(0);
        static_assert(NB5 == 1 && (4 * CB / 16) * 4096 <= TrunkLds<CB>::ACT, "conv5: one pass per wave, V of the layer fits the activation buffer");
        conv3x3_wino_mfma_shared_v<NW, 4 * CB, 4 * CB, LayC4>(act, a.packed + a.off.w_wino[2], Uw, y, wave, lane);
        __builtin_amdgcn_s_setprio(3);
        CNN_STAMP(11);
        wino_bias<NW, 8, 4 * CB, NB5>(a.packed + a.off.b[5], bw, wave, lane);
        if (!STAMPS || a.dbg_layer < 0) {
            wino_store_global<4 * CB, 8, NB5>(a.out + pidx * (64 * 4 * CB), bw, y, wave, lane);
            CNN_STAMP(13);
            return;
        }
        __syncthreads();
        wino_store_lds<4 * CB, LayC5, NB5>(act, bw, y, wave, lane);
        __syncthreads();
        CNN_STAMP(12);
        if (STAMPS && a.dbg_layer == 5) { dump_planes<4 * CB, LayC5, NTHR>(act, a.dbg_out); return; }
    } else if constexpr (S3 == 0) {
        constexpr int T1M = S::T1M, T1N = S::T1N, T2M = S::T2M, T2N = S::T2N, T4M = S::T4M, T4N = S::T4N;
        static_assert(NW == 8 && CB == 16, "Wino16 describes the 16-channel trunks on 8 waves");
        f32x4 b4[S::G4][T4N];
        f32x4 bias4[T4N];
        if constexpr (KIND == AFFNET_NET_ORINET) {
            constexpr int NB1 = Wino16::NB1, NB3 = Wino16::NB3;
            {
                f32x4 acc[T1M][T1N];
                conv0_mfma<NW, CB, T1M, T1N>(patch, w0, bias0, acc, wave, lane);
                CNN_STAMP(19);
                store_tiles_lds<CB, LayC0, T1M, T1N, false>(act, bias0, acc, wave, lane);
                CNN_STAMP(20);
                __syncthreads();
            }
            if (STAMPS && a.dbg_layer == 0) { dump_planes<CB, LayC0, NTHR>(act, a.dbg_out); return; }
            CNN_STAMP(2);

            f32x4 b2[S::G2][T2N];
            f32x4 bias2[T2N];
            {
                f32x4 y[NB1][4], bw[NB1];
                conv3x3_wino_mfma_rows<NW, CB, CB, LayC0, NB1>(act, a.wino_u, Ur, y, wave, lane);
                CNN_STAMP(3);
                prefetch_b0<NW, 2 * CB, 16, T2M, T2N, S::G2>(a.packed + a.off.w[2], b2, wave, lane);
                prefetch_bias<NW, 16, T2M, T2N>(a.packed + a.off.b[2], bias2, wave, lane);
                wino_bias<NW, 32, CB, NB1>(a.packed + a.off.b[1], bw, wave, lane);
                __syncthreads();
                CNN_STAMP(21);
                zero_halo<LayC1, NTHR>(act, CB);
                wino_store_lds<CB, LayC1, NB1>(act, bw, y, wave, lane);
                CNN_STAMP(22);
                __syncthreads();
                CNN_STAMP(4);
            }
            if (STAMPS && a.dbg_layer == 1) { dump_planes<CB, LayC1, NTHR>(act, a.dbg_out); return; }

            {
                f32x4 acc[T2M][T2N];
                conv3x3_mfma<NW, CB, 2 * CB, LayC1, 2, T2M, T2N, S::G2>(act, a.packed + a.off.w[2], b2, acc, wave, lane);
                CNN_STAMP(5);
                wino_prefetch_u_row<NW, 2 * CB, 2 * CB, 16, NB3>(a.wino_u + Wino16::offset(3), Ur, wave, lane);
                __syncthreads();
                zero_halo<LayC2, NTHR>(act, 2 * CB);
                store_tiles_lds<2 * CB, LayC2, T2M, T2N>(act, bias2, acc, wave, lane);
                __syncthreads();
                CNN_STAMP(6);
            }
            if (STAMPS && a.dbg_layer == 2) { dump_planes<2 * CB, LayC2, NTHR>(act, a.dbg_out); return; }

            {
                f32x4 y[NB3][4], bw[NB3];
                conv3x3_wino_mfma_rows<NW, 2 * CB, 2 * CB, LayC2, NB3>(act, a.wino_u + Wino16::offset(3), Ur, y, wave, lane);
                CNN_STAMP(7);
                prefetch_b0<NW, 4 * CB, 8, T4M, T4N, S::G4>(a.packed + a.off.w[4], b4, wave, lane);
                prefetch_bias<NW, 8, T4M, T4N>(a.packed + a.off.b[4], bias4, wave, lane);
                wino_bias<NW, 16, 2 * CB, NB3>(a.packed + a.off.b[3], bw, wave, lane);
                __syncthreads();
                zero_halo<LayC3, NTHR>(act, 2 * CB);
                wino_store_lds<2 * CB, LayC3, NB3>(act, bw, y, wave, lane);
                __syncthreads();
                CNN_STAMP(8);
            }
            if (STAMPS && a.dbg_layer == 3) { dump_planes<2 * CB, LayC3, NTHR>(act, a.dbg_out); return; }

        } else {
            static_assert(T1M * 8 > S::AREG, "conv1: two A sets of T1M float4 do not fit -> rolling single set (conv3x3_mfma_roll)");
            f32x4 bias1[T1N];
            {
                f32x4 acc[T1M][T1N];
                conv0_mfma<NW, CB, T1M, T1N>(patch, w0, bias0, acc, wave, lane);
                CNN_STAMP(19);
                prefetch_bias<NW, 32, T1M, T1N>(a.packed + a.off.b[1], bias1, wave, lane);
                store_tiles_lds<CB, LayC0, T1M, T1N, false>(act, bias0, acc, wave, lane);
                CNN_STAMP(20);
                __syncthreads();
            }
            if (STAMPS && a.dbg_layer == 0) { dump_planes<CB, LayC0, NTHR>(act, a.dbg_out); return; }
            CNN_STAMP(2);

            f32x4 b2[S::G2][T2N];
            f32x4 bias2[T2N];
            {
                f32x4 acc[T1M][T1N];
                conv3x3_mfma_roll<NW, CB, CB, LayC0, 1, T1M, T1N>(act, a.packed + a.off.w[1], b1, acc, wave, lane);
                CNN_STAMP(3);
                prefetch_b0<NW, 2 * CB, 16, T2M, T2N, S::G2>(a.packed + a.off.w[2], b2, wave, lane);
                prefetch_bias<NW, 16, T2M, T2N>(a.packed + a.off.b[2], bias2, wave, lane);
                __syncthreads();
                CNN_STAMP(21);
                zero_halo<LayC1, NTHR>(act, CB);
                store_tiles_lds<CB, LayC1, T1M, T1N>(act, bias1, acc, wave, lane);
                CNN_STAMP(22);
                __syncthreads();
                CNN_STAMP(4);
            }
            if (STAMPS && a.dbg_layer == 1) { dump_planes<CB, LayC1, NTHR>(act, a.dbg_out); return; }

            f32x4 b3[S::G3][T2N];
            f32x4 bias3[T2N];
            {
                f32x4 acc[T2M][T2N];
                conv3x3_mfma<NW, CB, 2 * CB, LayC1, 2, T2M, T2N, S::G2>(act, a.packed + a.off.w[2], b2, acc, wave, lane);
                CNN_STAMP(5);
                prefetch_b0<NW, 2 * CB, 16, T2M, T2N, S::G3>(a.packed + a.off.w[3], b3, wave, lane);
                prefetch_bias<NW, 16, T2M, T2N>(a.packed + a.off.b[3], bias3, wave, lane);
                __syncthreads();
                zero_halo<LayC2, NTHR>(act, 2 * CB);
                store_tiles_lds<2 * CB, LayC2, T2M, T2N>(act, bias2, acc, wave, lane);
                __syncthreads();
                CNN_STAMP(6);
            }
            if (STAMPS && a.dbg_layer == 2) { dump_planes<2 * CB, LayC2, NTHR>(act, a.dbg_out); return; }

            {
                f32x4 acc[T2M][T2N];
                conv3x3_mfma<NW, 2 * CB, 2 * CB, LayC2, 1, T2M, T2N, S::G3>(act, a.packed + a.off.w[3], b3, acc, wave, lane);
                CNN_STAMP(7);
                prefetch_b0<NW, 4 * CB, 8, T4M, T4N, S::G4>(a.packed + a.off.w[4], b4, wave, lane);
                prefetch_bias<NW, 8, T4M, T4N>(a.packed + a.off.b[4], bias4, wave, lane);
                __syncthreads();
                zero_halo<LayC3, NTHR>(act, 2 * CB);
                store_tiles_lds<2 * CB, LayC3, T2M, T2N>(act, bias3, acc, wave, lane);
                __syncthreads();
                CNN_STAMP(8);
            }
            if (STAMPS && a.dbg_layer == 3) { dump_planes<2 * CB, LayC3, NTHR>(act, a.dbg_out); return; }

        }

        f32x4 b5[S::G5][T4N];
        f32x4 bias5[T4N];
        {
            f32x4 acc[T4M][T4N];
            conv3x3_mfma<NW, 2 * CB, 4 * CB, LayC3, 2, T4M, T4N, S::G4>(act, a.packed + a.off.w[4], b4, acc, wave, lane);
            CNN_STAMP(9);
            if constexpr (KIND == AFFNET_NET_ORINET) {
                wino5_prefetch_u(a.wino_u + Wino16::offset(5), Ur, wave, lane);
            } else {
                prefetch_b0<NW, 4 * CB, 8, T4M, T4N, S::G5>(a.packed + a.off.w[5], b5, wave, lane);
                prefetch_bias<NW, 8, T4M, T4N>(a.packed + a.off.b[5], bias5, wave, lane);
            }
            __syncthreads();
            zero_halo<LayC4, NTHR>(act, 4 * CB);
            store_tiles_lds<4 * CB, LayC4, T4M, T4N>(act, bias4, acc, wave, lane);
            __syncthreads();
            CNN_STAMP(10);
        }
        if (STAMPS && a.dbg_layer == 4) { dump_planes<4 * CB, LayC4, NTHR>(act, a.dbg_out); return; }

        if constexpr (KIND == AFFNET_NET_ORINET) {
            static_assert(Wino5::X >= 16 * LayC4::PSG && Wino5::X + Wino5::X_FLOATS <= TrunkLds<CB>::TOTAL && Wino5::HEAD + 100 * ORI_HP <= Wino5::X,
                          "conv5: the exchange lies behind conv4's output inside the LDS array, the head copy in front of the exchange");
            f32x4 acc[2][4], y[2], hw[2][T4M];
            conv3x3_wino_mfma_half_rows<NW, LayC4>(act, a.wino_u + Wino16::offset(5), Ur, acc, wave, lane);
            CNN_STAMP(11);
            const f32x4 bw = *reinterpret_cast<const f32x4*>(&a.packed[a.off.b[5] + (wave >> 1) * 16 + 4 * (lane >> 4)]);
            const OriHeadLane HL = OriHeadLane::of<T4M>(wave, lane);
            if (!STAMPS || a.dbg_layer < 0) ori_head_weights<T4M>(a.packed + a.off.head_w, HL, hw);
// ... 293 lines not shown
```

affnet_amd/csrc/cnn_trunk_affnet.hip:

```cpp
#include "cnn_trunk.h"

TrunkKernel aff_trunk_affnet(int arith_index, bool stamps) {
    static const TrunkKernel k[3][2] = {{cnn32_trunk_kernel<AFFNET_NET_AFFNET, 8, false>, cnn32_trunk_kernel<AFFNET_NET_AFFNET, 8, true>},
                                        {cnn32_trunk_kernel<AFFNET_NET_AFFNET, 8, false, 3>, cnn32_trunk_kernel<AFFNET_NET_AFFNET, 8, true, 3>},
                                        {cnn32_trunk_kernel<AFFNET_NET_AFFNET, 8, false, 2>, cnn32_trunk_kernel<AFFNET_NET_AFFNET, 8, true, 2>}};
    return k[arith_index][stamps];
}
```

affnet_amd/csrc/common.h:

```cpp
#pragma once
#include <hip/hip_runtime.h>
#include <stdint.h>
#include <stdio.h>
#include <string.h>

#include <string>
#include <vector>

#include "../../include/affnet_hip.h"
#include "../../include/affnet_hip_debug.h"
#include "weights_layout.h"

#define AFF_WAVE 64

enum {
    CNT_RAW0 = 0,
    CNT_CAND = AFFNET_MAX_OCTAVES,
    CNT_OVERFLOW,
    CNT_SEL,
    CNT_EQ_TAKEN,
    CNT_SEL_MODE,
    CNT_SEL_THRESH,
    CNT_SEL_NEED_EQ,
    CNT_DET,
    CNT_SHAPED,
    CNT_SURVIVED,
    CNT_CAND2,
    CNT_AFF_EVAL,
    CNT_SURVIVED1,
    CNT_SEL_EQ_TOTAL,
    CNT_SEL_TIE_LO, CNT_SEL_TIE_HI,
    CNT_POS0 = AFFNET_MAX_OCTAVES + 24,
    CNT_HYP0 = AFFNET_MAX_OCTAVES + 24 + (AFFNET_MAX_LEVELS - 2) * AFFNET_MAX_OCTAVES,
    CNT_TOTAL = AFFNET_MAX_OCTAVES + 24 + (AFFNET_MAX_LEVELS - 2) * AFFNET_MAX_OCTAVES + 8 * AFFNET_MAX_OCTAVES
};

#define OVF_FRAMES_COUNT 16
#define OVF_FRAMES_NONFINITE 32

#define SEL_HIST_BINS 2048

struct RawMax {
    int32_t pix;
    int32_t lvl;
    float val;
    float s, y, x;
    float prev[2];
};

struct OctaveGeom {
    int32_t h, w;
    int64_t pyr_off;
    int64_t map_off;
    int64_t raw_off;
    int32_t raw_cap;
};

struct affnet_ctx {
    int device = 0;
    affnet_config cfg;
    int B = 1;
    size_t pyr_stride = 0;
    size_t map_stride = 0;
    size_t raw_stride = 0;
    std::string err;
    OctaveGeom oct[AFFNET_MAX_OCTAVES];
    size_t off_pyr = 0, off_map = 0, off_raw = 0, off_cnt = 0, off_hist = 0, off_cand = 0, off_sel = 0, off_stage = 0;
    size_t off_affmap = 0, off_dense = 0, off_cand2 = 0, off_lvltab = 0;
    size_t aff_stride = 0;
    size_t aff_off[AFFNET_MAX_OCTAVES] = {0};
    size_t dense_stride = 0;
    float* affmap = nullptr; float* dense = nullptr;
    float* cand2_resp = nullptr; float* cand2_syx = nullptr; int32_t* cand2_ids = nullptr;
    int32_t* lvltab = nullptr;
    size_t ws_bytes = 0;
    size_t pyr_floats = 0, map_bytes = 0, raw_total = 0, cand_cap = 0;
    int cap_pre = 0, cap_final = 0;
    char* ws = nullptr;
    float* pyr = nullptr;
    uint8_t* omap = nullptr;
    RawMax* raw = nullptr;
    int32_t* cnt = nullptr;
    uint32_t* sel_hist = nullptr;
    float* cand_resp = nullptr; float* cand_syx = nullptr; int32_t* cand_ids = nullptr;
    float* sel_resp = nullptr; float* sel_syx = nullptr; int32_t* sel_ids = nullptr;
    float* st_det_resp = nullptr; float* st_det_lafs = nullptr; int32_t* st_det_ids = nullptr;
    int32_t* st_det_count = nullptr;
    float* st_A = nullptr; float* st_key = nullptr; int32_t* st_good = nullptr;
    float* st_A2 = nullptr; float* st_lafs_iter = nullptr;
    float* st_R = nullptr; float* st_lafs_norm = nullptr; int32_t* st_lvl_ids = nullptr;
    float* st_hard_scratch = nullptr;
    float* st_lafs_shaped = nullptr;
    int32_t* st_rank = nullptr;
    bool prof_on = false;
    std::vector<hipEvent_t> prof_ev;
    int prof_calls = 0;
    unsigned long long* dbg_time = nullptr;
    int arith = AFFNET_ARITH_FP32_MFMA;
    int split3_variant = 0;
    hipGraph_t graph = nullptr;
    hipGraphExec_t graph_exec = nullptr;
    float* wino_u = nullptr;
    ~affnet_ctx() {
        if (wino_u) (void)hipFree(wino_u);
        if (graph_exec) (void)hipGraphExecDestroy(graph_exec);
        if (graph) (void)hipGraphDestroy(graph);
        for (auto& e : prof_ev) (void)hipEventDestroy(e);
    }
};

struct AffDeviceGuard {
    int prev = -1;
    bool switched = false;
    explicit AffDeviceGuard(const affnet_ctx* ctx) {
        if (!ctx) return;
        if (hipGetDevice(&prev) != hipSuccess) { (void)hipGetLastError(); prev = -1; return; }
        if (prev != ctx->device) switched = hipSetDevice(ctx->device) == hipSuccess;
    }
    ~AffDeviceGuard() {
        if (switched) (void)hipSetDevice(prev);
    }
    AffDeviceGuard(const AffDeviceGuard&) = delete;
    AffDeviceGuard& operator=(const AffDeviceGuard&) = delete;
};
#define AFF_DEVICE(ctx) AffDeviceGuard aff_device_guard_(ctx)

#define PROF_RING 256
#define PROF_EVENTS (AFFNET_PROFILE_STAGES + 2)

#define AFF_HIP(ctx, expr)                                                                         \
    do {                                                                                           \
        hipError_t e_ = (expr);                                                                    \
        if (e_ != hipSuccess)                                                                      \
            return aff_fail(ctx, AFFNET_ERR_HIP, "%s failed: %s (%s:%d)", #expr, hipGetErrorString(e_), \
                            __FILE__, __LINE__);                                                   \
    } while (0)

#define AFF_LAUNCH_CHECK(ctx)                                                                      \
    do {                                                                                           \
        hipError_t e_ = hipGetLastError();                                                         \
        if (e_ != hipSuccess)                                                                      \
            return aff_fail(ctx, AFFNET_ERR_HIP, "kernel launch failed: %s (%s:%d)",                \
                            hipGetErrorString(e_), __FILE__, __LINE__);                            \
    } while (0)

struct AffZeroSegs {
    unsigned char* p[8];
    size_t bytes[8];
    int n = 0;
    bool overflow = false;
    void add(void* ptr, size_t nbytes) {
        if (!ptr || !nbytes) return;
        if (n >= 8) { overflow = true; return; }
        p[n] = (unsigned char*)ptr; bytes[n] = nbytes; ++n;
    }
};

static inline size_t aff_align(size_t x, size_t a = 256) { return (x + a - 1) / a * a; }
static inline int aff_cdiv(int a, int b) { return (a + b - 1) / b; }

struct PyrTable {
    const float* lvl[AFFNET_MAX_OCTAVES][AFFNET_MAX_LEVELS];
    int h[AFFNET_MAX_OCTAVES], w[AFFNET_MAX_OCTAVES];
    int n_octaves, n_levels;
    size_t img_stride;
};

struct LevelTable { double sig[AFFNET_MAX_OCTAVES * AFFNET_MAX_LEVELS]; int n_oct, n_lvl; };
struct DenormSel {
    float* out_px; int32_t* ids; float* lafs_norm;
    float c_a, c_x, c_y, ps, ca, cx, cy;
    LevelTable lt;
};


#define HEAD_PART_AFF 32
#define HEAD_PART_ORI 144
#define HEAD_KSPLIT 4
#define HEAD_KC 128
#define HEAD_AS (HEAD_KC + 4)

struct PyrSrc {
    PyrTable t;
    float base[32];
};

struct CnnArgs {
    const float* packed;
    NetOffsets off;
    const float* wino_u;
    const float* patches;
    const float* lafs;
    const int32_t* ids;
    const int32_t* count;
    int n_max;
    float* out;
    int dbg_layer;
    int s3_alt;
    float* dbg_out;
    unsigned long long* dbg_time;
    int row_begin;
    const int32_t* skip_cnt;
    int skip_n;
    int32_t* shape_cnt;
    int shape_op;
};

__device__ __forceinline__ bool lazy_skip(const int32_t* skip_cnt, int skip_n, int image, int which = CNT_SURVIVED1) {
    if (!skip_cnt) return false;
    const int32_t* c = skip_cnt + (size_t)image * CNT_TOTAL;
    return c[CNT_SEL_MODE] == 1 && c[which] >= skip_n;
}

struct Wino16 {
    static constexpr int U1 = 16 * 16 * 16, U3 = 16 * 32 * 32, U5 = 16 * 64 * 64, FLOATS = U1 + U3 + U5;
    static constexpr int PAIRS = 16 * 16 + 32 * 32 + 64 * 64;
    static constexpr int NB1 = 2, NB3 = 1;
    static constexpr int offset(int layer) { return layer == 1 ? 0 : (layer == 3 ? U1 : U1 + U3); }
    static constexpr int floats(int layer) { return layer == 1 ? U1 : (layer == 3 ? U3 : U5); }
};

struct ShapeFuse {
    const float* resp; const float* lafs; float* key; int32_t* good; int32_t* cnt;
};

struct CnnCall {
    int kind = -1;
    const float* packed = nullptr;
    const float* patches = nullptr;
    const float* lafs = nullptr; const int32_t* ids = nullptr;
    const int32_t* count = nullptr; int n_max = 0;
    float* out = nullptr; float* scratch = nullptr;
    hipStream_t st = nullptr;
    int dbg_layer = -1; float* dbg_out = nullptr;
    bool mark_head = false;
    int row_begin = 0, row_count = -1;
    const int32_t* skip_cnt = nullptr; int skip_n = 0;
    const ShapeFuse* fuse = nullptr; int shape_op = 0;
    float* rot_lafs = nullptr; const DenormSel* denorm = nullptr;
};

typedef void (*TrunkKernel)(CnnArgs, PyrSrc);

int aff_fail(affnet_ctx* ctx, int code, const char* fmt, ...);
int aff_zero_async(affnet_ctx* ctx, void* dst, size_t bytes, hipStream_t st);
int aff_zero_multi_async(affnet_ctx* ctx, const AffZeroSegs& z, hipStream_t st);
int aff_copy_async(affnet_ctx* ctx, void* dst, const void* src, size_t bytes, hipStream_t st);
int aff_copy2d_async(affnet_ctx* ctx, void* dst, size_t dpitch, const void* src, size_t spitch, size_t width_bytes, size_t rows, hipStream_t st);
void aff_base_grid(int ps, float* base);

void aff_prof_mark(affnet_ctx* ctx, int idx, hipStream_t st);

int aff_detect_impl(affnet_ctx* ctx, const float* d_responses, float* d_resp, float* d_lafs, int32_t* d_ids, int32_t* d_count, void* stream);
int aff_detect_onepass_impl(affnet_ctx* ctx, const float* d_packed_fullconv, const float* d_responses, hipStream_t st);

int aff_fullconv_launch(affnet_ctx* ctx, const float* packed, const float* img, size_t img_stride, int h, int w, float* out, size_t out_stride,
                        float* scratch, size_t scratch_stride, int B, hipStream_t st);

int aff_handcrafted_launch(affnet_ctx* ctx, int kind, const float* patches, const float* lafs, const int32_t* ids, const int32_t* count,
                           int n_max, const float* h_weights, float* out, float* out_angle, hipStream_t st);

void aff_fill_pyr_table(const affnet_ctx* ctx, PyrTable* t);
int aff_shape_select(affnet_ctx* ctx, const float* d_resp_in, const float* d_lafs_in, const int32_t* d_ids_in, const float* d_A,
                     const int32_t* d_count_in, float* d_resp_out, float* d_lafs_out, int32_t* d_ids_out, int32_t* d_count_out, hipStream_t st);
int aff_shape_iterate(affnet_ctx* ctx, const float* A, float* base, const float* lafs, const int32_t* count, int mode, float* lafs_out,
                      hipStream_t st);
void aff_denorm_sel_fill(affnet_ctx* ctx, int ps, float* d_lafs_px, int32_t* d_ids, float* d_lafs_norm, DenormSel* ds);
int aff_denorm_level_select(affnet_ctx* ctx, const float* d_lafs_norm_in, float* d_lafs_px, const int32_t* d_count, int n_max, int ps, int32_t* d_ids,
                            float* d_lafs_norm, hipStream_t st);

int aff_arith_index(const affnet_ctx* ctx);
int aff_affnet_filter_rows(affnet_ctx* ctx, const float* packed, const float* resp, const float* lafs, const int32_t* ids, const int32_t* count,
                           float* out, float* scratch, int row_begin, int row_count, bool lazy, int shape_op, hipStream_t st);
int aff_orinet_rotate(affnet_ctx* ctx, const float* packed, float* lafs, const int32_t* ids, const int32_t* count, int n_max, float* out, float* scratch,
                      hipStream_t st, const DenormSel* denorm);
int aff_hardnet_forward_pyr_marked(affnet_ctx* ctx, const float* packed, const float* lafs, const int32_t* ids, const int32_t* count,
                                   int n_max, float* out, float* scratch, hipStream_t st);

TrunkKernel aff_trunk_affnet(int arith_index, bool stamps);
TrunkKernel aff_trunk_orinet(int arith_index, bool stamps);
TrunkKernel aff_trunk_hardnet(int arith_index, bool stamps);
int aff_wino_u_ensure(affnet_ctx* ctx);
int aff_wino_derive_u(affnet_ctx* ctx, int kind, const float* packed, const NetLayout& L, hipStream_t st, const float** u);

int aff_finish_affnet(affnet_ctx* ctx, const CnnCall& c, const NetLayout& L, int rows, int B);
int aff_finish_orinet(affnet_ctx* ctx, const CnnCall& c, const NetLayout& L, int rows, int B);
int aff_hardnet_head(affnet_ctx* ctx, const CnnCall& c, const NetLayout& L, int B);

struct AffTile {
    int x0, y0, tw, th;
};

__device__ __forceinline__ AffTile aff_tile_box(float t00, float t01, float t02, float t10, float t11, float t12, int ps, int cap) {
    const float um = (float)(ps - 1) / (float)ps;
    const float hx = (fabsf(t00) + fabsf(t01)) * um, hy = (fabsf(t10) + fabsf(t11)) * um;
    const float cx = t02 - 0.5f, cy = t12 - 0.5f;
    AffTile t;
    t.tw = 0; t.th = 0; t.x0 = 0; t.y0 = 0;
    if (!(hx < 4096.0f && hy < 4096.0f && fabsf(cx) < 1.0e6f && fabsf(cy) < 1.0e6f)) return t;
    const int x0 = (int)floorf(cx - hx) - 1, x1 = (int)floorf(cx + hx) + 2;
    const int y0 = (int)floorf(cy - hy) - 1, y1 = (int)floorf(cy + hy) + 2;
    const int tw = x1 - x0 + 1, th = y1 - y0 + 1;
    if (tw * th > cap || tw * th > 2 * ps * ps) return t;
    t.x0 = x0; t.y0 = y0; t.tw = tw; t.th = th;
    return t;
}

template <int NTHR>
__device__ __forceinline__ void aff_tile_load(float* tile, const AffTile t, const float* __restrict__ img, int h, int w, int tid) {
    const int n = t.tw * t.th;
    for (int i = tid; i < n; i += NTHR) {
        const int ty = i / t.tw, tx = i - ty * t.tw;
        const int gy = t.y0 + ty, gx = t.x0 + tx;
        tile[i] = (gy >= 0 && gy < h && gx >= 0 && gx < w) ? img[(size_t)gy * w + gx] : 0.0f;
    }
}

__device__ __forceinline__ float aff_sample_bilinear(const float* __restrict__ img, int h, int w,
                                                     float t00, float t01, float t02, float t10,
                                                     float t11, float t12, float u, float v) {
    float gx = fmaf(1.0f, t02, fmaf(v, t01, u * t00));
    float gy = fmaf(1.0f, t12, fmaf(v, t11, u * t10));
    const float fw = (float)w, fh = (float)h;
    gx = 2.0f * gx / fw - 1.0f;
    gy = 2.0f * gy / fh - 1.0f;
    const float ix = fmaf(gx + 1.0f, fw * 0.5f, -0.5f);
    const float iy = fmaf(gy + 1.0f, fh * 0.5f, -0.5f);
    const float x0f = floorf(ix), y0f = floorf(iy);
    const float x1f = x0f + 1.0f, y1f = y0f + 1.0f;
    const float wx1 = ix - x0f, wx0 = x1f - ix, wy1 = iy - y0f, wy0 = y1f - iy;
    const float nw = wx0 * wy0, ne = wx1 * wy0, sw = wx0 * wy1, se = wx1 * wy1;
    const float cx0 = fminf(fmaxf(x0f, -2.0f), fw + 1.0f), cy0 = fminf(fmaxf(y0f, -2.0f), fh + 1.0f);
    const int x0 = (int)cx0, y0 = (int)cy0, x1 = x0 + 1, y1 = y0 + 1;
    const bool xin0 = (x0 >= 0) & (x0 < w), xin1 = (x1 >= 0) & (x1 < w);
    const bool yin0 = (y0 >= 0) & (y0 < h), yin1 = (y1 >= 0) & (y1 < h);
    const float vnw = (xin0 & yin0) ? img[(size_t)y0 * w + x0] : 0.0f;
    const float vne = (xin1 & yin0) ? img[(size_t)y0 * w + x1] : 0.0f;
    const float vsw = (xin0 & yin1) ? img[(size_t)y1 * w + x0] : 0.0f;
    const float vse = (xin1 & yin1) ? img[(size_t)y1 * w + x1] : 0.0f;
    return fmaf(vse, se, fmaf(vsw, sw, fmaf(vne, ne, vnw * nw)));
}

__device__ __forceinline__ float aff_sample_bilinear_tile(const float* tile, const AffTile tl, const float* __restrict__ img, int h, int w,
                                                          float t00, float t01, float t02, float t10, float t11, float t12, float u, float v) {
    float gx = fmaf(1.0f, t02, fmaf(v, t01, u * t00));
    float gy = fmaf(1.0f, t12, fmaf(v, t11, u * t10));
    const float fw = (float)w, fh = (float)h;
    gx = 2.0f * gx / fw - 1.0f;
    gy = 2.0f * gy / fh - 1.0f;
    const float ix = fmaf(gx + 1.0f, fw * 0.5f, -0.5f);
    const float iy = fmaf(gy + 1.0f, fh * 0.5f, -0.5f);
    const float x0f = floorf(ix), y0f = floorf(iy);
    const float x1f = x0f + 1.0f, y1f = y0f + 1.0f;
    const float wx1 = ix - x0f, wx0 = x1f - ix, wy1 = iy - y0f, wy0 = y1f - iy;
    const float nw = wx0 * wy0, ne = wx1 * wy0, sw = wx0 * wy1, se = wx1 * wy1;
    const float cx0 = fminf(fmaxf(x0f, -2.0f), fw + 1.0f), cy0 = fminf(fmaxf(y0f, -2.0f), fh + 1.0f);
    const int x0 = (int)cx0, y0 = (int)cy0;
    const int lx = x0 - tl.x0, ly = y0 - tl.y0;
    float vnw, vne, vsw, vse;
    if (lx >= 0 && ly >= 0 && lx + 1 < tl.tw && ly + 1 < tl.th) {
        const float* p = tile + ly * tl.tw + lx;
        vnw = p[0]; vne = p[1]; vsw = p[tl.tw]; vse = p[tl.tw + 1];
    } else {
        const int x1 = x0 + 1, y1 = y0 + 1;
        const bool xin0 = (x0 >= 0) & (x0 < w), xin1 = (x1 >= 0) & (x1 < w);
        const bool yin0 = (y0 >= 0) & (y0 < h), yin1 = (y1 >= 0) & (y1 < h);
        vnw = (xin0 & yin0) ? img[(size_t)y0 * w + x0] : 0.0f;
        vne = (xin1 & yin0) ? img[(size_t)y0 * w + x1] : 0.0f;
        vsw = (xin0 & yin1) ? img[(size_t)y1 * w + x0] : 0.0f;
        vse = (xin1 & yin1) ? img[(size_t)y1 * w + x1] : 0.0f;
    }
    return fmaf(vse, se, fmaf(vsw, sw, fmaf(vne, ne, vnw * nw)));
}
```

affnet_amd/csrc/context.hip:

```cpp
#include <stdarg.h>

#include "common.h"

int aff_fail(affnet_ctx* ctx, int code, const char* fmt, ...) {
    char buf[1024];
    va_list ap;
    va_start(ap, fmt);
    vsnprintf(buf, sizeof(buf), fmt, ap);
    va_end(ap);
    if (ctx) ctx->err = buf;
    return code;
}

__global__ __launch_bounds__(256) void aff_zero_kernel(unsigned char* __restrict__ p, size_t bytes) {
    const size_t head = ((16 - ((size_t)p & 15)) & 15) < bytes ? ((16 - ((size_t)p & 15)) & 15) : bytes;
    const size_t n16 = (bytes - head) / 16, tail0 = head + n16 * 16;
    uint4* q = reinterpret_cast<uint4*>(p + head);
    for (size_t i = (size_t)blockIdx.x * 256 + threadIdx.x; i < n16; i += (size_t)gridDim.x * 256) q[i] = make_uint4(0u, 0u, 0u, 0u);
    if (blockIdx.x == 0) {
        for (size_t i = threadIdx.x; i < head; i += 256) p[i] = 0;
        for (size_t i = tail0 + threadIdx.x; i < bytes; i += 256) p[i] = 0;
    }
}

// ... 40 lines not shown
    return AFFNET_OK;
}

int aff_copy2d_async(affnet_ctx* ctx, void* dst, size_t dpitch, const void* src, size_t spitch, size_t width_bytes, size_t rows, hipStream_t st) {
    if (rows == 0 || width_bytes == 0) return AFFNET_OK;
    if (!dst || !src || ((size_t)dst & 3) || ((size_t)src & 3) || (dpitch & 3) || (spitch & 3) || (width_bytes & 3) || rows > 65535)
        return aff_fail(ctx, AFFNET_ERR_INVALID, "copy2d: pointers, pitches and width must be multiples of 4 bytes, rows <= 65535");
    size_t bx = (width_bytes / 4 + 255) / 256;
    bx = bx < 1 ? 1 : (bx > 2048 ? 2048 : bx);
    hipLaunchKernelGGL(aff_copy2d_kernel, dim3((unsigned)bx, (unsigned)rows), dim3(256), 0, st, (uint32_t*)dst, dpitch / 4, (const uint32_t*)src, spitch / 4,
                       width_bytes / 4);
    AFF_LAUNCH_CHECK(ctx);
    return AFFNET_OK;
}

int aff_copy_async(affnet_ctx* ctx, void* dst, const void* src, size_t bytes, hipStream_t st) {
    return aff_copy2d_async(ctx, dst, bytes, src, bytes, bytes, 1, st);
}

extern "C" const char* affnet_version(void) { return "affnet_hip 0.2 (gfx950, hipcc, fp32 MFMA 16x16x4)"; }

extern "C" const char* affnet_last_error(const affnet_ctx* ctx) { return ctx ? ctx->err.c_str() : "null context"; }

void aff_base_grid(int ps, float* base) {
    if (ps == 1) { base[0] = 0.0f; return; }
    const float step = 2.0f / (float)(ps - 1);
    const int half = ps / 2;
    for (int i = 0; i < ps; ++i) {
        float v = (i < half) ? fmaf(step, (float)i, -1.0f) : fmaf(-step, (float)(ps - 1 - i), 1.0f);
        base[i] = (v * (float)(ps - 1)) / (float)ps;
    }
}

extern "C" int affnet_host_base_grid(int ps, float* out) {
    if (ps < 1 || !out) return AFFNET_ERR_INVALID;
    aff_base_grid(ps, out);
    return AFFNET_OK;
}

static int validate(affnet_ctx* ctx, const affnet_config* c) {
    if (c->height < 8 || c->width < 8) return aff_fail(ctx, AFFNET_ERR_INVALID, "image %dx%d too small", c->height, c->width);
    if (c->batch > 4096) return aff_fail(ctx, AFFNET_ERR_INVALID, "batch=%d (max 4096)", c->batch);
    if (c->arith < AFFNET_ARITH_FP32_MFMA || c->arith > AFFNET_ARITH_FP32_SPLIT2H) return aff_fail(ctx, AFFNET_ERR_INVALID, "arith=%d (AFFNET_ARITH_*)", c->arith);
    if (c->n_octaves < 1 || c->n_octaves > AFFNET_MAX_OCTAVES) return aff_fail(ctx, AFFNET_ERR_INVALID, "n_octaves=%d", c->n_octaves);
    if (c->levels_per_octave < 3 || c->levels_per_octave > AFFNET_MAX_LEVELS)
        return aff_fail(ctx, AFFNET_ERR_INVALID, "levels_per_octave=%d", c->levels_per_octave);
    if (c->oct_h[0] != c->height || c->oct_w[0] != c->width) return aff_fail(ctx, AFFNET_ERR_INVALID, "octave 0 size mismatch");
    for (int o = 1; o < c->n_octaves; ++o)
        if (c->oct_h[o] != (c->oct_h[o - 1] - 1) / 2 + 1 || c->oct_w[o] != (c->oct_w[o - 1] - 1) / 2 + 1)
            return aff_fail(ctx, AFFNET_ERR_INVALID, "octave %d size is not ceil(prev/2)", o);
    if (c->first_blur_taps != 0 && (c->first_blur_taps % 2 == 0 || c->first_blur_taps > AFFNET_MAX_TAPS))
        return aff_fail(ctx, AFFNET_ERR_INVALID, "first_blur_taps=%d", c->first_blur_taps);
    for (int l = 1; l < c->levels_per_octave; ++l)
        if (c->level_blur_taps[l] % 2 == 0 || c->level_blur_taps[l] < 1 || c->level_blur_taps[l] > AFFNET_MAX_TAPS)
            return aff_fail(ctx, AFFNET_ERR_INVALID, "level_blur_taps[%d]=%d", l, c->level_blur_taps[l]);
    if (c->level_blur0_taps[1] != 0)
        for (int l = 1; l < c->levels_per_octave; ++l)
            if (c->level_blur0_taps[l] % 2 == 0 || c->level_blur0_taps[l] < 1 || c->level_blur0_taps[l] > AFFNET_MAX_TAPS)
                return aff_fail(ctx, AFFNET_ERR_INVALID, "level_blur0_taps[%d]=%d", l, c->level_blur0_taps[l]);
    return AFFNET_OK;
}

extern "C" int affnet_ctx_create(affnet_ctx** out, int device, const affnet_config* cfg) {
    if (!out) return AFFNET_ERR_INVALID;
    affnet_ctx* ctx = new affnet_ctx();
    ctx->device = device;
    if (!cfg) {
        memset(&ctx->cfg, 0, sizeof(ctx->cfg));
        *out = ctx;
        return AFFNET_OK;
    }
    ctx->cfg = *cfg;
    ctx->arith = cfg->arith;
    int rc = validate(ctx, cfg);
    if (rc != AFFNET_OK) { *out = ctx; return rc; }
    const affnet_config& c = ctx->cfg;
    const int div = c.max_raw_per_octave_div > 0 ? c.max_raw_per_octave_div : 4;
    size_t pyr = 0, mapb = 0, raw = 0;
    for (int o = 0; o < c.n_octaves; ++o) {
        OctaveGeom& g = ctx->oct[o];
        g.h = c.oct_h[o]; g.w = c.oct_w[o];
        g.pyr_off = (int64_t)pyr; pyr += (size_t)c.levels_per_octave * g.h * g.w;
        g.map_off = (int64_t)mapb; mapb += aff_align((size_t)g.h * g.w, 16);
        int cap = (int)((size_t)g.h * g.w / div); if (cap < 256) cap = 256;
        g.raw_off = (int64_t)raw; g.raw_cap = cap; raw += cap;
    }
    ctx->B = c.batch > 0 ? c.batch : 1;
    const size_t B = (size_t)ctx->B;
    ctx->pyr_floats = pyr; ctx->map_bytes = mapb; ctx->raw_total = raw; ctx->cand_cap = raw;
    ctx->pyr_stride = aff_align(pyr * sizeof(float)) / sizeof(float);
    ctx->map_stride = aff_align(mapb);
    ctx->raw_stride = raw;
    const int keep = c.max_keep > 0 ? c.max_keep : 65536;
    ctx->cap_pre = c.num_prefilter > 0 ? c.num_prefilter : keep;
    ctx->cap_final = c.num_features > 0 ? c.num_features : ctx->cap_pre;
    if (ctx->cap_final > ctx->cap_pre) ctx->cap_final = ctx->cap_pre;
    size_t off = 0;
    ctx->off_pyr = off; off += B * ctx->pyr_stride * sizeof(float);
    ctx->off_map = off; off += B * ctx->map_stride;
    ctx->off_raw = off; off += aff_align(B * raw * sizeof(RawMax));
    ctx->off_cnt = off; off += aff_align(B * CNT_TOTAL * sizeof(int32_t));
    ctx->off_hist = off; off += aff_align(B * SEL_HIST_BINS * sizeof(uint32_t));
    ctx->off_cand = off; off += aff_align(B * ctx->cand_cap * 7 * sizeof(float));
    ctx->off_sel = off; off += aff_align(B * (size_t)ctx->cap_pre * 7 * sizeof(float));
    ctx->off_stage = off;
    const size_t P = B * (size_t)ctx->cap_pre, F = B * (size_t)ctx->cap_final;
    off += aff_align(P * 10 * sizeof(float));
    off += aff_align(P * 4 * sizeof(float));
    off += aff_align(P * 10 * sizeof(float));
    off += aff_align(P * 2 * sizeof(float));
    off += aff_align(P * sizeof(int32_t));
    off += aff_align(B * sizeof(int32_t));
    off += aff_align(F * 6 * sizeof(float));
    off += aff_align(F * 4 * sizeof(float));
    off += aff_align(F * 9 * sizeof(float));
    {
        const size_t hard = F * (8192 + 4 * 128), aff = P * 144;
        off += aff_align((hard > aff ? hard : aff) * sizeof(float));
    }
    if (c.onepass) {
        if (c.num_prefilter != c.num_features) { *out = ctx; return aff_fail(ctx, AFFNET_ERR_INVALID, "onepass: num_prefilter must equal num_features"); }
        size_t aff = 0;
        for (int o = 0; o < c.n_octaves; ++o) {
            if (c.oct_h[o] < 34 || c.oct_w[o] < 34) {
                *out = ctx;
                return aff_fail(ctx, AFFNET_ERR_INVALID, "onepass: octave %d is %dx%d, LocalNorm2d(33) needs >= 34 px in this library (17 in the reference: use "
                                "border >= 15 like its scripts, so that the pyramid stops earlier)", o, c.oct_w[o], c.oct_h[o]);
            }
            ctx->aff_off[o] = aff; aff += aff_align((size_t)4 * c.oct_h[o] * c.oct_w[o] * sizeof(float)) / sizeof(float);
        }
        ctx->aff_stride = aff;
        ctx->dense_stride = affnet_fullconv_scratch_bytes(c.oct_h[0], c.oct_w[0]) / sizeof(float);
        ctx->off_affmap = off; off += aff_align(B * aff * sizeof(float));
        ctx->off_dense = off; off += aff_align(B * ctx->dense_stride * sizeof(float));
        ctx->off_cand2 = off; off += aff_align(B * ctx->cand_cap * 7 * sizeof(float));
        ctx->off_lvltab = off; off += aff_align(B * (size_t)AFFNET_MAX_OCTAVES * AFFNET_MAX_LEVELS * 4 * sizeof(int32_t));
    }
    ctx->ws_bytes = off;
    *out = ctx;
    return AFFNET_OK;
}

extern "C" void affnet_ctx_destroy(affnet_ctx* ctx) { delete ctx; }

extern "C" int affnet_set_arith(affnet_ctx* ctx, int arith) {
    if (!ctx) return AFFNET_ERR_INVALID;
    if (arith < AFFNET_ARITH_FP32_MFMA || arith > AFFNET_ARITH_FP32_SPLIT2H) return aff_fail(ctx, AFFNET_ERR_INVALID, "arith=%d (AFFNET_ARITH_*)", arith);
    ctx->arith = arith;
    ctx->cfg.arith = arith;
    return AFFNET_OK;
}
extern "C" int affnet_get_arith(const affnet_ctx* ctx) { return ctx ? ctx->arith : AFFNET_ERR_INVALID; }

extern "C" size_t affnet_workspace_bytes(const affnet_ctx* ctx) { return ctx ? ctx->ws_bytes : 0; }

extern "C" int affnet_capacity_prefilter(const affnet_ctx* ctx) { return ctx ? ctx->cap_pre : 0; }
extern "C" int affnet_capacity_final(const affnet_ctx* ctx) { return ctx ? ctx->cap_final : 0; }

extern "C" int64_t affnet_pyramid_level_offset(const affnet_ctx* ctx, int octave, int level) {
    if (!ctx || octave < 0 || octave >= ctx->cfg.n_octaves || level < 0 || level >= ctx->cfg.levels_per_octave) return -1;
    const OctaveGeom& g = ctx->oct[octave];
    return (int64_t)(ctx->off_pyr / sizeof(float)) + g.pyr_off + (int64_t)level * g.h * g.w;
}

extern "C" int64_t affnet_pyramid_image_stride(const affnet_ctx* ctx) { return ctx ? (int64_t)ctx->pyr_stride : 0; }

extern "C" int64_t affnet_counter_offset(const affnet_ctx* ctx, int which) {
    if (!ctx || ctx->ws_bytes == 0 || which < 0 || which > 3) return -1;
    const int idx = which == 0 ? CNT_OVERFLOW : (which == 1 ? CNT_DET : (which == 2 ? CNT_SHAPED : CNT_AFF_EVAL));
    return (int64_t)(ctx->off_cnt / sizeof(int32_t)) + idx;
}
extern "C" int64_t affnet_counter_stride(const affnet_ctx* ctx) { return ctx ? (int64_t)CNT_TOTAL : 0; }

extern "C" int64_t affnet_affmap_offset(const affnet_ctx* ctx, int octave) {
    if (!ctx || !ctx->cfg.onepass || octave < 0 || octave >= ctx->cfg.n_octaves) return -1;
    return (int64_t)(ctx->off_affmap / sizeof(float)) + (int64_t)ctx->aff_off[octave];
}
extern "C" int64_t affnet_affmap_image_stride(const affnet_ctx* ctx) { return (ctx && ctx->cfg.onepass) ? (int64_t)ctx->aff_stride : 0; }
extern "C" int affnet_batch(const affnet_ctx* ctx) { return ctx ? ctx->B : 0; }

extern "C" int affnet_bind_workspace(affnet_ctx* ctx, void* d_workspace, size_t bytes) {
    if (!ctx) return AFFNET_ERR_INVALID;
    if (!d_workspace || bytes < ctx->ws_bytes)
        return aff_fail(ctx, AFFNET_ERR_INVALID, "workspace too small: %zu < %zu", bytes, ctx->ws_bytes);
    if (((uintptr_t)d_workspace & 255) != 0) return aff_fail(ctx, AFFNET_ERR_INVALID, "workspace must be 256-byte aligned");
    {
        hipPointerAttribute_t at;
        if (hipPointerGetAttributes(&at, d_workspace) == hipSuccess) {
            if (at.type == hipMemoryTypeDevice && at.device != ctx->device)
                return aff_fail(ctx, AFFNET_ERR_INVALID, "workspace belongs to device %d, the context to device %d", at.device, ctx->device);
        } else {
            (void)hipGetLastError();
        }
    }
    char* b = (char*)d_workspace;
    ctx->ws = b;
    ctx->pyr = (float*)(b + ctx->off_pyr);
    ctx->omap = (uint8_t*)(b + ctx->off_map);
    ctx->raw = (RawMax*)(b + ctx->off_raw);
    ctx->cnt = (int32_t*)(b + ctx->off_cnt);
    ctx->sel_hist = (uint32_t*)(b + ctx->off_hist);
    const size_t B = (size_t)ctx->B;
    float* cand = (float*)(b + ctx->off_cand);
    const size_t CC = B * ctx->cand_cap;
    ctx->cand_resp = cand; ctx->cand_syx = cand + CC; ctx->cand_ids = (int32_t*)(cand + 4 * CC);
    float* sel = (float*)(b + ctx->off_sel);
    const size_t P = B * (size_t)ctx->cap_pre, F = B * (size_t)ctx->cap_final;
    ctx->sel_resp = sel; ctx->sel_syx = sel + P; ctx->sel_ids = (int32_t*)(sel + 4 * P);
    char* s = b + ctx->off_stage;
    ctx->st_det_resp = (float*)s; ctx->st_det_lafs = (float*)s + P; ctx->st_det_ids = (int32_t*)((float*)s + 7 * P);
    s += aff_align(P * 10 * sizeof(float));
    ctx->st_A = (float*)s; s += aff_align(P * 4 * sizeof(float));
    ctx->st_A2 = (float*)s; ctx->st_lafs_iter = (float*)s + 4 * P; s += aff_align(P * 10 * sizeof(float));
    ctx->st_key = (float*)s; ctx->st_good = (int32_t*)((float*)s + P); s += aff_align(P * 2 * sizeof(float));
    ctx->st_rank = (int32_t*)s; s += aff_align(P * sizeof(int32_t));
    ctx->st_det_count = (int32_t*)s; s += aff_align(B * sizeof(int32_t));
    ctx->st_lafs_shaped = (float*)s; s += aff_align(F * 6 * sizeof(float));
    ctx->st_R = (float*)s; s += aff_align(F * 4 * sizeof(float));
    ctx->st_lafs_norm = (float*)s; ctx->st_lvl_ids = (int32_t*)((float*)s + 6 * F); s += aff_align(F * 9 * sizeof(float));
    ctx->st_hard_scratch = (float*)s;
    if (ctx->cfg.onepass) {
        ctx->affmap = (float*)(b + ctx->off_affmap);
        ctx->dense = (float*)(b + ctx->off_dense);
        float* c2 = (float*)(b + ctx->off_cand2);
        ctx->cand2_resp = c2; ctx->cand2_syx = c2 + CC; ctx->cand2_ids = (int32_t*)(c2 + 4 * CC);
        ctx->lvltab = (int32_t*)(b + ctx->off_lvltab);
    }
    return AFFNET_OK;
}

extern "C" int affnet_read_counts(affnet_ctx* ctx, int32_t out[4], void* stream) {
    AFF_DEVICE(ctx);
    if (!ctx || !ctx->ws) return AFFNET_ERR_INVALID;
    std::vector<int32_t> all((size_t)ctx->B * CNT_TOTAL);
    AFF_HIP(ctx, hipMemcpyAsync(all.data(), ctx->cnt, all.size() * sizeof(int32_t), hipMemcpyDeviceToHost, (hipStream_t)stream));
    AFF_HIP(ctx, hipStreamSynchronize((hipStream_t)stream));
    int32_t host[CNT_TOTAL];
    memset(host, 0, sizeof(host));
    int raw = 0;
    for (int b = 0; b < ctx->B; ++b) {
        const int32_t* h = all.data() + (size_t)b * CNT_TOTAL;
        host[CNT_DET] += h[CNT_DET]; host[CNT_SHAPED] += h[CNT_SHAPED]; host[CNT_OVERFLOW] |= h[CNT_OVERFLOW];
        for (int o = 0; o < ctx->cfg.n_octaves; ++o) raw += h[CNT_RAW0 + o];
    }
    out[0] = host[CNT_DET]; out[1] = host[CNT_SHAPED]; out[2] = host[CNT_OVERFLOW];
    out[3] = raw;
    if (host[CNT_OVERFLOW] & OVF_FRAMES_NONFINITE)
        return aff_fail(ctx, AFFNET_ERR_INVALID, "load_frames: a caller-supplied frame or response was not finite (stored as a zero row; flag %d)",
                        host[CNT_OVERFLOW]);
    if (host[CNT_OVERFLOW]) return aff_fail(ctx, AFFNET_ERR_CAPACITY, "a fixed-capacity detector list overflowed (flag %d)", host[CNT_OVERFLOW]);
    if (host[CNT_DET] == 0)
        return aff_fail(ctx, AFFNET_ERR_EMPTY, "no keypoints detected in %d image(s) (the reference raises in torch.cat, SparseImgRepresenter.py:100)", ctx->B);
    return AFFNET_OK;
}
```

affnet_amd/csrc/debug.hip:

```cpp
#include "common.h"

#include "../../include/affnet_hip_probes.h"

template <typename T>
__global__ __launch_bounds__(256) void stream_read_kernel(const T* __restrict__ src, float* __restrict__ dst, size_t n_items) {
    float acc = 0.f;
    for (size_t i = (size_t)blockIdx.x * 256 + threadIdx.x; i < n_items; i += (size_t)gridDim.x * 256) {
        const T v = src[i];
        const float* f = reinterpret_cast<const float*>(&v);
#pragma unroll
        for (int k = 0; k < (int)(sizeof(T) / 4); ++k) acc += f[k];
    }
    if (acc == 123.456f) dst[blockIdx.x] = acc;
    if (threadIdx.x == 0 && blockIdx.x == 0) dst[0] = acc;
}

template <typename T>
__global__ __launch_bounds__(256) void stream_write_kernel(T* __restrict__ dst, size_t n_items) {
    T v;
    float* f = reinterpret_cast<float*>(&v);
#pragma unroll
    for (int k = 0; k < (int)(sizeof(T) / 4); ++k) f[k] = (float)(threadIdx.x + k);
    for (size_t i = (size_t)blockIdx.x * 256 + threadIdx.x; i < n_items; i += (size_t)gridDim.x * 256) dst[i] = v;
}

__global__ __launch_bounds__(256) void tile_read_kernel(const float* __restrict__ img, float* __restrict__ dst, int h, int w, int halo) {
    const int LW = 64 + 2 * halo, n_el = LW * LW;
    const int x0 = blockIdx.x * 64, y0 = blockIdx.y * 64;
    float acc = 0.f;
    for (int i = threadIdx.x; i < n_el; i += 256) {
        const int ty = i / LW, tx = i - ty * LW;
        int gy = y0 + ty - halo, gx = x0 + tx - halo;
        gy = gy < 0 ? 0 : (gy >= h ? h - 1 : gy);
        gx = gx < 0 ? 0 : (gx >= w ? w - 1 : gx);
        acc += img[(size_t)gy * w + gx];
    }
    if (acc == 123.456f) dst[blockIdx.x] = acc;
}

struct f32x2s { float a, b; };

extern "C" int affnet_debug_stream(const void* d_src, void* d_dst, size_t n_bytes, int width, int mode, int halo, void* stream) {
    if (!d_dst || n_bytes == 0 || (n_bytes & 65535) != 0) return AFFNET_ERR_INVALID;
    hipStream_t st = (hipStream_t)stream;
    const int blocks = 256 * 16;
    if (mode == 0) {
        if (!d_src) return AFFNET_ERR_INVALID;
        if (width == 4) hipLaunchKernelGGL(stream_read_kernel<float>, dim3(blocks), dim3(256), 0, st, (const float*)d_src, (float*)d_dst, n_bytes / 4);
        else if (width == 8) hipLaunchKernelGGL(stream_read_kernel<f32x2s>, dim3(blocks), dim3(256), 0, st, (const f32x2s*)d_src, (float*)d_dst, n_bytes / 8);
        else if (width == 16) hipLaunchKernelGGL(stream_read_kernel<float4>, dim3(blocks), dim3(256), 0, st, (const float4*)d_src, (float*)d_dst, n_bytes / 16);
        else return AFFNET_ERR_INVALID;
    } else if (mode == 1) {
        if (width == 4) hipLaunchKernelGGL(stream_write_kernel<float>, dim3(blocks), dim3(256), 0, st, (float*)d_dst, n_bytes / 4);
        else if (width == 8) hipLaunchKernelGGL(stream_write_kernel<f32x2s>, dim3(blocks), dim3(256), 0, st, (f32x2s*)d_dst, n_bytes / 8);
        else if (width == 16) hipLaunchKernelGGL(stream_write_kernel<float4>, dim3(blocks), dim3(256), 0, st, (float4*)d_dst, n_bytes / 16);
        else return AFFNET_ERR_INVALID;
    } else if (mode == 2) {
        if (!d_src || halo < 0 || halo > 16) return AFFNET_ERR_INVALID;
        const int w = 4096, h = (int)(n_bytes / 4 / w);
        hipLaunchKernelGGL(tile_read_kernel, dim3(w / 64, (h + 63) / 64), dim3(256), 0, st, (const float*)d_src, (float*)d_dst, h, w, halo);
    } else {
        return AFFNET_ERR_INVALID;
    }
    return hipGetLastError() == hipSuccess ? AFFNET_OK : AFFNET_ERR_HIP;
}
```

affnet_amd/csrc/pipeline.hip:

```cpp
#include "common.h"

void aff_prof_mark(affnet_ctx* ctx, int idx, hipStream_t st) {
    if (!ctx->prof_on || ctx->prof_calls >= PROF_RING) return;
    (void)hipEventRecord(ctx->prof_ev[(size_t)ctx->prof_calls * PROF_EVENTS + idx], st);
}

extern "C" int affnet_profile_enable(affnet_ctx* ctx, int on) {
    if (!ctx) return AFFNET_ERR_INVALID;
    if (on && ctx->prof_ev.empty()) {
        ctx->prof_ev.resize((size_t)PROF_RING * PROF_EVENTS);
        for (auto& e : ctx->prof_ev) AFF_HIP(ctx, hipEventCreate(&e));
    }
    ctx->prof_on = on != 0;
    ctx->prof_calls = 0;
    return AFFNET_OK;
}

extern "C" int affnet_profile_read(affnet_ctx* ctx, double sum_ms[AFFNET_PROFILE_STAGES], int32_t* n_calls) {
    AFF_DEVICE(ctx);
    if (!ctx || !sum_ms || !n_calls) return AFFNET_ERR_INVALID;
    for (int s = 0; s < AFFNET_PROFILE_STAGES; ++s) sum_ms[s] = 0.0;
    *n_calls = ctx->prof_calls;
    for (int c = 0; c < ctx->prof_calls; ++c)
        for (int s = 0; s < AFFNET_PROFILE_STAGES; ++s) {
            float ms = 0.f;
            const size_t b = (size_t)c * PROF_EVENTS;
            AFF_HIP(ctx, hipEventElapsedTime(&ms, ctx->prof_ev[b + s], ctx->prof_ev[b + (s == 1 ? 9 : s + 1)]));
            sum_ms[s] += ms;
        }
    ctx->prof_calls = 0;
    return AFFNET_OK;
}

static int detect_half(affnet_ctx* ctx, const float* d_img, bool onepass, const float* d_packed_fullconv, const float* d_responses, void* stream) {
    hipStream_t st = (hipStream_t)stream;
    aff_prof_mark(ctx, 0, st);
    if (d_img) {
        int rc = affnet_pyramid_build(ctx, d_img, stream);
        if (rc) return rc;
    }
    aff_prof_mark(ctx, 1, st);
    int rc = onepass ? aff_detect_onepass_impl(ctx, d_packed_fullconv, d_responses, st)
                     : aff_detect_impl(ctx, d_responses, ctx->st_det_resp, ctx->st_det_lafs, ctx->st_det_ids, ctx->st_det_count, stream);
    if (rc) return rc;
    aff_prof_mark(ctx, 9, st);
    return AFFNET_OK;
}

extern "C" int affnet_detect_image_responses(affnet_ctx* ctx, const float* d_responses, void* stream) {
    AFF_DEVICE(ctx);
    if (!ctx || !ctx->ws || !d_responses) return aff_fail(ctx, AFFNET_ERR_INVALID, "detect_image_responses: context not bound or null responses");
    return detect_half(ctx, nullptr, false, nullptr, d_responses, stream);
}

extern "C" int affnet_detect_image(affnet_ctx* ctx, const float* d_img, void* stream) {
    AFF_DEVICE(ctx);
    if (!ctx || !ctx->ws || !d_img) return aff_fail(ctx, AFFNET_ERR_INVALID, "detect_image: context not bound or null image");
    return detect_half(ctx, d_img, false, nullptr, nullptr, stream);
}

extern "C" int affnet_detect_image_onepass(affnet_ctx* ctx, const float* d_packed_fullconv, const float* d_img, void* stream) {
    AFF_DEVICE(ctx);
    if (!ctx || !ctx->ws) return aff_fail(ctx, AFFNET_ERR_INVALID, "detect_image_onepass: context not bound");
    return detect_half(ctx, d_img, true, d_packed_fullconv, nullptr, stream);
}

extern "C" int affnet_detect_image_onepass_responses(affnet_ctx* ctx, const float* d_packed_fullconv, const float* d_responses, void* stream) {
    AFF_DEVICE(ctx);
    if (!ctx || !ctx->ws || !d_responses) return aff_fail(ctx, AFFNET_ERR_INVALID, "detect_image_onepass_responses: context not bound or null responses");
    return detect_half(ctx, nullptr, true, d_packed_fullconv, d_responses, stream);
}

extern "C" int affnet_detected_list(affnet_ctx* ctx, float* d_resp, float* d_lafs, int32_t* d_ids, int32_t* d_count, void* stream) {
    AFF_DEVICE(ctx);
    if (!ctx || !ctx->ws || !d_resp || !d_lafs || !d_ids || !d_count) return aff_fail(ctx, AFFNET_ERR_INVALID, "detected_list: context not bound or null output");
    hipStream_t st = (hipStream_t)stream;
    const size_t P = (size_t)ctx->B * ctx->cap_pre;
    int rc = aff_copy_async(ctx, d_resp, ctx->st_det_resp, P * sizeof(float), st);
    if (!rc) rc = aff_copy_async(ctx, d_lafs, ctx->st_det_lafs, P * 6 * sizeof(float), st);
    if (!rc) rc = aff_copy_async(ctx, d_ids, ctx->st_det_ids, P * 3 * sizeof(int32_t), st);
    if (!rc) rc = aff_copy_async(ctx, d_count, ctx->st_det_count, (size_t)ctx->B * sizeof(int32_t), st);
    return rc;
}

extern "C" int affnet_shape_iterate(affnet_ctx* ctx, const float* d_A, float* d_base, const float* d_lafs, const int32_t* d_count, int mode,
                                    float* d_lafs_out, void* stream) {
    AFF_DEVICE(ctx);
    if (!ctx || !ctx->ws || !d_base || !d_lafs || !d_count || !d_lafs_out || (mode != 0 && mode != 1) || (mode == 1 && !d_A))
        return aff_fail(ctx, AFFNET_ERR_INVALID, "shape_iterate: bad argument");
    return aff_shape_iterate(ctx, d_A, d_base, d_lafs, d_count, mode, d_lafs_out, (hipStream_t)stream);
}

extern "C" int affnet_describe_detected(affnet_ctx* ctx, const affnet_nets* nets, int do_ori, float* d_lafs_px, float* d_resp,
                                        int32_t* d_ids, float* d_desc, int32_t* d_count, void* stream) {
    AFF_DEVICE(ctx);
    if (!ctx || !ctx->ws || !nets || !d_lafs_px || !d_resp || !d_ids || !d_count)
        return aff_fail(ctx, AFFNET_ERR_INVALID, "describe_detected: context not bound or null argument");
    if (do_ori && !nets->d_orinet && !nets->h_orientation_window)
        return aff_fail(ctx, AFFNET_ERR_INVALID, "describe_detected: do_ori needs OriNet weights or the OrientationDetector window");
    if (d_desc && !nets->d_hardnet) return aff_fail(ctx, AFFNET_ERR_INVALID, "describe_detected: descriptors need HardNet weights");
    hipStream_t st = (hipStream_t)stream;
    const int P = ctx->cap_pre, F = ctx->cap_final;
    const size_t B = (size_t)ctx->B;
    int rc;
    int32_t* det_count = ctx->st_det_count;
    aff_prof_mark(ctx, 2, st);
    const bool baumberg = !nets->d_affnet && nets->h_baumberg_window && ctx->cfg.baum_iters > 0;
    auto shape_pass = [&](const float* lafs, float* A_out) -> int {
        if (baumberg)
            return aff_handcrafted_launch(ctx, AFFNET_HC_BAUMBERG, nullptr, lafs, ctx->st_det_ids, det_count, P, nets->h_baumberg_window, A_out,
                                          nullptr, st);
        return affnet_cnn32_forward_pyr(ctx, AFFNET_NET_AFFNET, nets->d_affnet, lafs, ctx->st_det_ids, det_count, P, A_out, ctx->st_hard_scratch,
                                        stream);
    };
    const int N = ctx->cfg.num_features;
    const int lazy = (nets->d_affnet && ctx->cfg.baum_iters <= 1 && N > 0 && ctx->cfg.lazy_shape_rows != 0)
                         ? (ctx->cfg.lazy_shape_rows > 0 ? ctx->cfg.lazy_shape_rows : N + (N + 4) / 5) : 0;
    if (lazy > 0 && lazy < P) {
        rc = aff_affnet_filter_rows(ctx, nets->d_affnet, ctx->st_det_resp, ctx->st_det_lafs, ctx->st_det_ids, det_count, ctx->st_A, ctx->st_hard_scratch,
                                    0, lazy, false, 1, st);
        if (rc) return rc;
        rc = aff_affnet_filter_rows(ctx, nets->d_affnet, ctx->st_det_resp, ctx->st_det_lafs, ctx->st_det_ids, det_count, ctx->st_A, ctx->st_hard_scratch,
                                    lazy, P - lazy, true, 2, st);
        if (rc) return rc;
        aff_prof_mark(ctx, 3, st);
        rc = aff_shape_select(ctx, ctx->st_det_resp, ctx->st_det_lafs, ctx->st_det_ids, ctx->st_A, det_count, d_resp, ctx->st_lafs_shaped, d_ids,
                              d_count, st);
        if (rc) return rc;
    } else if (nets->d_affnet || baumberg) {
        rc = shape_pass(ctx->st_det_lafs, ctx->st_A);
        if (rc) return rc;
        const int iters = ctx->cfg.baum_iters > 0 ? ctx->cfg.baum_iters : 1;
        for (int it = 1; it < iters; ++it) {
            rc = aff_shape_iterate(ctx, nullptr, ctx->st_A, ctx->st_det_lafs, det_count, 0, ctx->st_lafs_iter, st);
            if (rc) return rc;
            rc = shape_pass(ctx->st_lafs_iter, ctx->st_A2);
            if (rc) return rc;
            rc = aff_shape_iterate(ctx, ctx->st_A2, ctx->st_A, ctx->st_det_lafs, det_count, 1, ctx->st_lafs_iter, st);
            if (rc) return rc;
        }
        aff_prof_mark(ctx, 3, st);
        rc = affnet_shape_filter_select(ctx, ctx->st_det_resp, ctx->st_det_lafs, ctx->st_det_ids, ctx->st_A, det_count, d_resp,
                                        ctx->st_lafs_shaped, d_ids, d_count, stream);
        if (rc) return rc;
    } else {
        aff_prof_mark(ctx, 3, st);
        if (F != P) return aff_fail(ctx, AFFNET_ERR_INVALID, "describe_detected: without AffNet num_prefilter must equal num_features");
        { int crc = aff_copy_async(ctx, d_resp, ctx->st_det_resp, B * F * sizeof(float), st); if (crc) return crc; }
        { int crc = aff_copy_async(ctx, ctx->st_lafs_shaped, ctx->st_det_lafs, B * F * 6 * sizeof(float), st); if (crc) return crc; }
        { int crc = aff_copy_async(ctx, d_ids, ctx->st_det_ids, B * F * 3 * sizeof(int32_t), st); if (crc) return crc; }
        { int crc = aff_copy_async(ctx, d_count, det_count, B * sizeof(int32_t), st); if (crc) return crc; }
        { int crc = aff_copy2d_async(ctx, ctx->cnt + CNT_SHAPED, CNT_TOTAL * sizeof(int32_t), det_count, sizeof(int32_t), sizeof(int32_t), B, st); if (crc) return crc; }
    }
    aff_prof_mark(ctx, 4, st);
    bool denorm_done = false;
    if (do_ori) {
        if (nets->d_orinet) {
            DenormSel ds;
            if (d_desc) aff_denorm_sel_fill(ctx, 32, d_lafs_px, ctx->st_lvl_ids, ctx->st_lafs_norm, &ds);
            rc = aff_orinet_rotate(ctx, nets->d_orinet, ctx->st_lafs_shaped, d_ids, d_count, F, ctx->st_R, ctx->st_hard_scratch, st, d_desc ? &ds : nullptr);
            if (rc) return rc;
            denorm_done = d_desc != nullptr;
        } else {
            rc = aff_handcrafted_launch(ctx, AFFNET_HC_ORIENTATION, nullptr, ctx->st_lafs_shaped, d_ids, d_count, F, nets->h_orientation_window,
                                        ctx->st_R, nullptr, st);
            if (rc) return rc;
            rc = affnet_apply_rotation(ctx, ctx->st_lafs_shaped, ctx->st_R, d_count, F, stream);
            if (rc) return rc;
        }
    }
    aff_prof_mark(ctx, 5, st);
    if (d_desc) {
        if (!denorm_done) {
            rc = aff_denorm_level_select(ctx, ctx->st_lafs_shaped, d_lafs_px, d_count, F, 32, ctx->st_lvl_ids, ctx->st_lafs_norm, st);
            if (rc) return rc;
        }
        aff_prof_mark(ctx, 6, st);
        rc = aff_hardnet_forward_pyr_marked(ctx, nets->d_hardnet, ctx->st_lafs_norm, ctx->st_lvl_ids, d_count, F, d_desc,
                                            ctx->st_hard_scratch, st);
        if (rc) return rc;
    } else {
        rc = affnet_scale_lafs(ctx, ctx->st_lafs_shaped, d_lafs_px, d_count, F, ctx->cfg.width, ctx->cfg.height, 0, stream);
        if (rc) return rc;
        aff_prof_mark(ctx, 6, st);
        aff_prof_mark(ctx, 7, st);
    }
    aff_prof_mark(ctx, 8, st);
    if (ctx->prof_on && ctx->prof_calls < PROF_RING) ++ctx->prof_calls;
    return AFFNET_OK;
}

extern "C" int affnet_extract_features(affnet_ctx* ctx, const affnet_nets* nets, const float* d_img, int do_ori, float* d_lafs_px,
                                       float* d_resp, int32_t* d_ids, float* d_desc, int32_t* d_count, void* stream) {
    AFF_DEVICE(ctx);
    int rc = affnet_detect_image(ctx, d_img, stream);
    if (rc) return rc;
    return affnet_describe_detected(ctx, nets, do_ori, d_lafs_px, d_resp, d_ids, d_desc, d_count, stream);
}

extern "C" int affnet_describe_frames(affnet_ctx* ctx, const affnet_nets* nets, const float* d_img, const float* d_lafs_px, const float* d_resp_in,
                                      const int32_t* d_count_in, int n_max, int do_ori, float* d_lafs_px_out, float* d_resp, int32_t* d_ids,
                                      float* d_desc, int32_t* d_count, void* stream) {
    AFF_DEVICE(ctx);
    if (!ctx || !ctx->ws || !nets || !d_lafs_px || !d_lafs_px_out || !d_resp || !d_ids || !d_count)
        return aff_fail(ctx, AFFNET_ERR_INVALID, "describe_frames: context not bound or null argument");
    if (do_ori && !nets->d_orinet && !nets->h_orientation_window)
        return aff_fail(ctx, AFFNET_ERR_INVALID, "describe_frames: do_ori needs OriNet weights or the OrientationDetector window");
    if (d_desc && !nets->d_hardnet) return aff_fail(ctx, AFFNET_ERR_INVALID, "describe_frames: descriptors need HardNet weights");
    hipStream_t st = (hipStream_t)stream;
    aff_prof_mark(ctx, 0, st);
    if (d_img) {
        int rc = affnet_pyramid_build(ctx, d_img, stream);
        if (rc) return rc;
    }
    aff_prof_mark(ctx, 1, st);
    int ps = 32;
    if (nets->d_affnet) ps = 32;
    else if (nets->h_baumberg_window && ctx->cfg.baum_iters > 0) ps = 19;
    else if (do_ori && !nets->d_orinet) ps = 19;
    int rc = affnet_load_frames(ctx, d_lafs_px, 0, d_resp_in, nullptr, d_count_in, n_max, ps, stream);
    if (rc) return rc;
    aff_prof_mark(ctx, 9, st);
    return affnet_describe_detected(ctx, nets, do_ori, d_lafs_px_out, d_resp, d_ids, d_desc, d_count, stream);
}


extern "C" int affnet_graph_capture_extract(affnet_ctx* ctx, const affnet_nets* nets, const float* d_img, int do_ori, float* d_lafs_px, float* d_resp,
                                            int32_t* d_ids, float* d_desc, int32_t* d_count, void* stream) {
    AFF_DEVICE(ctx);
    if (!ctx || !ctx->ws) return aff_fail(ctx, AFFNET_ERR_INVALID, "graph_capture: context not bound");
    hipStream_t st = (hipStream_t)stream;
    if (!st) return aff_fail(ctx, AFFNET_ERR_INVALID, "graph_capture: needs an explicit (non-null) stream - the legacy null stream cannot be captured");
    if (ctx->prof_on) return aff_fail(ctx, AFFNET_ERR_INVALID, "graph_capture: switch stage profiling off first (its events are per call)");
    if (ctx->graph_exec) { (void)hipGraphExecDestroy(ctx->graph_exec); ctx->graph_exec = nullptr; }
    if (ctx->graph) { (void)hipGraphDestroy(ctx->graph); ctx->graph = nullptr; }
    { const int rcu = aff_wino_u_ensure(ctx); if (rcu) return rcu; }
    AFF_HIP(ctx, hipStreamBeginCapture(st, hipStreamCaptureModeThreadLocal));
    const int rc = affnet_extract_features(ctx, nets, d_img, do_ori, d_lafs_px, d_resp, d_ids, d_desc, d_count, stream);
    hipGraph_t g = nullptr;
    const hipError_t e = hipStreamEndCapture(st, &g);
    if (rc != AFFNET_OK) { if (g) (void)hipGraphDestroy(g); return rc; }
    if (e != hipSuccess || !g) return aff_fail(ctx, AFFNET_ERR_HIP, "hipStreamEndCapture failed: %s", hipGetErrorString(e));
    ctx->graph = g;
    AFF_HIP(ctx, hipGraphInstantiate(&ctx->graph_exec, ctx->graph, nullptr, nullptr, 0));
    return AFFNET_OK;
}

extern "C" int affnet_graph_launch(affnet_ctx* ctx, void* stream) {
    AFF_DEVICE(ctx);
    if (!ctx || !ctx->graph_exec) return aff_fail(ctx, AFFNET_ERR_INVALID, "graph_launch: nothing captured (affnet_graph_capture_extract first)");
    AFF_HIP(ctx, hipGraphLaunch(ctx->graph_exec, (hipStream_t)stream));
    return AFFNET_OK;
}
```

affnet_amd/csrc/shape_filter.h:

```cpp
#pragma once
#include "common.h"

__device__ __forceinline__ void aff_shape_filter_row(const float* __restrict__ resp, const float* __restrict__ lafs, float a00, float a01, float a10,
                                                     float a11, int i, float* __restrict__ key, int32_t* __restrict__ good, int32_t* cnt) {
    const float* L = lafs + 6 * (size_t)i;
    const float n00 = fmaf(a01, L[3], a00 * L[0]), n01 = fmaf(a01, L[4], a00 * L[1]);
    const float n10 = fmaf(a11, L[3], a10 * L[0]), n11 = fmaf(a11, L[4], a10 * L[1]);
    const float cx = L[2], cy = L[5];
    const float tr = a00 + a11;
    const float p1 = a00 * a11, p2 = a10 * a01;
    const float d1 = tr * tr - 4.0f * (p1 - p2);
    const float mk = d1 > 0.f ? 1.0f : 0.0f;
    const float dl = sqrtf(fabsf(d1));
    const float l1 = mk * (tr + dl) / 2.0f + 1000.0f * (1.0f - mk);
    const float l2 = mk * (tr - dl) / 2.0f + 0.0001f * (1.0f - mk);
    const float ratio = fabsf(l1 / (l2 + 1e-8f));
    bool ok = (ratio < 6.0f) && (ratio > (float)(1.0 / 6.0));
    const float px[4] = {-1.f, -1.f, 1.f, 1.f}, py[4] = {-1.f, 1.f, -1.f, 1.f};
#pragma unroll
    for (int k = 0; k < 4; ++k) {
        const float ox = fmaf(cx, 1.0f, fmaf(n01, py[k], n00 * px[k]));
        const float oy = fmaf(cy, 1.0f, fmaf(n11, py[k], n10 * px[k]));
        if (ox > 1.0f || ox < 0.0f || oy > 1.0f || oy < 0.0f) ok = false;
    }
    good[i] = ok ? 1 : 0;
    key[i] = resp[i] * (ok ? 1.0f : 0.0f);
    if (ok) atomicAdd(&cnt[CNT_SURVIVED], 1);
}

__device__ __forceinline__ int aff_level_argmin(float q0, float q1, float q3, float q4, float ps, const LevelTable& lt) {
    const float p1 = q0 * q4, p2 = q1 * q3;
    const float sc = sqrtf(fabsf(p1 - p2) + 1e-12f);
    const double need = (double)(sc / ps);
    int best = 0;
    double bd = INFINITY;
    const int tot = lt.n_oct * lt.n_lvl;
    for (int k = 0; k < tot; ++k) {
        const double df = lt.sig[k] - need;
        const double d = sqrt(df * df);
        if (d < bd) { bd = d; best = k; }
    }
    return best;
}

__device__ __forceinline__ void aff_denorm_level_row(float l0, float l1, float l2, float l3, float l4, float l5, float c_a, float c_x, float c_y, float ps,
                                                     const LevelTable& lt, float ca, float cx, float cy, float* __restrict__ P, int32_t* __restrict__ I,
                                                     float* __restrict__ O) {
    const float q0 = c_a * l0, q1 = c_a * l1, q2 = c_x * l2, q3 = c_a * l3, q4 = c_a * l4, q5 = c_y * l5;
    P[0] = q0; P[1] = q1; P[2] = q2; P[3] = q3; P[4] = q4; P[5] = q5;
    const int best = aff_level_argmin(q0, q1, q3, q4, ps, lt);
    I[0] = best / lt.n_lvl; I[1] = best % lt.n_lvl; I[2] = 0;
    O[0] = ca * q0; O[1] = ca * q1; O[2] = cx * q2;
    O[3] = ca * q3; O[4] = ca * q4; O[5] = cy * q5;
}

__device__ __forceinline__ void aff_denorm_level_row_wave(int lane, float l0, float l1, float l2, float l3, float l4, float l5, float c_a, float c_x, float c_y, float ps,
                                                          const LevelTable& lt, float ca, float cx, float cy, float* __restrict__ P, int32_t* __restrict__ I,
                                                          float* __restrict__ O) {
    const float q0 = c_a * l0, q1 = c_a * l1, q2 = c_x * l2, q3 = c_a * l3, q4 = c_a * l4, q5 = c_y * l5;
    const float p1 = q0 * q4, p2 = q1 * q3;
    const float sc = sqrtf(fabsf(p1 - p2) + 1e-12f);
    const double need = (double)(sc / ps);
    const int tot = lt.n_oct * lt.n_lvl;
    double bd = INFINITY;
    int best = 0x7fffffff;
    for (int k = lane; k < tot; k += 64) {
        const double df = lt.sig[k] - need;
        const double d = sqrt(df * df);
        if (d < bd) { bd = d; best = k; }
    }
#pragma unroll
    for (int off = 32; off >= 1; off >>= 1) {
        const double od = __shfl_xor(bd, off, 64);
        const int ok = __shfl_xor(best, off, 64);
        if (od < bd || (od == bd && ok < best)) { bd = od; best = ok; }
    }
    if (lane != 0) return;
    if (best == 0x7fffffff) best = 0;
    P[0] = q0; P[1] = q1; P[2] = q2; P[3] = q3; P[4] = q4; P[5] = q5;
    I[0] = best / lt.n_lvl; I[1] = best % lt.n_lvl; I[2] = 0;
    O[0] = ca * q0; O[1] = ca * q1; O[2] = cx * q2;
    O[3] = ca * q3; O[4] = ca * q4; O[5] = cy * q5;
}
```

affnet_amd/engine.py:

```python
import ctypes as C

import numpy as np
import torch

from . import _lib
from ._lib import lib, check, ptr
from .host_plan import PyramidPlan

_UTILITY = {}


def require_cuda(t, what="tensor"):
    if not (isinstance(t, torch.Tensor) and t.is_cuda):
        raise RuntimeError("affnet_amd: %s must live on the MI355X (tensor.cuda()); this implementation has no CPU path" % what)


def utility_ctx(device, arith=0):
    idx = device.index if device.index is not None else torch.cuda.current_device()
    key = (idx, _lib.arith_code(arith))
    if key not in _UTILITY:
        h = C.c_void_p()
        check(lib.affnet_ctx_create(C.byref(h), idx, None), None, "affnet_ctx_create(utility)")
        check(lib.affnet_set_arith(h, key[1]), h, "affnet_set_arith")
        _UTILITY[key] = h
    h = _UTILITY[key]
    if lib.affnet_get_arith(h) != key[1]:
        check(lib.affnet_set_arith(h, key[1]), h, "affnet_set_arith")
    return h


def stream_of(device):
    return C.c_void_p(torch.cuda.current_stream(device).cuda_stream)


class Context(object):

    def __init__(self, height, width, device, n_levels, init_sigma, border, mr_size, threshold,
                 num_features, num_prefilter, max_keep=16384, batch=1, baum_iters=0, raw_div=4, onepass=False, lazy_shape_rows=-1, arith=0):
        self.plan = PyramidPlan(height, width, n_levels, init_sigma, border)
        self.batch = int(batch)
        self.onepass = bool(onepass)
        self.cfg = self.plan.fill_config(mr_size, threshold, num_features, num_prefilter, max_keep, raw_div=raw_div, batch=self.batch, baum_iters=baum_iters,
                                         onepass=onepass, lazy_shape_rows=lazy_shape_rows, arith=arith)
        self.arith = _lib.arith_code(arith)
        self.device = device
        self.handle = C.c_void_p()
        idx = device.index if device.index is not None else torch.cuda.current_device()
        rc = lib.affnet_ctx_create(C.byref(self.handle), idx, C.byref(self.cfg))
        check(rc, self.handle, "affnet_ctx_create")
        nbytes = lib.affnet_workspace_bytes(self.handle)
        self.workspace = torch.empty(nbytes, dtype=torch.uint8, device=device)
        check(lib.affnet_bind_workspace(self.handle, ptr(self.workspace), nbytes), self.handle, "affnet_bind_workspace")
        self.cap_pre = lib.affnet_capacity_prefilter(self.handle)
        self.cap_final = lib.affnet_capacity_final(self.handle)
        self._ws_f32 = self.workspace.view(torch.float32)

    def set_arith(self, arith):
        self.arith = _lib.arith_code(arith)
        check(lib.affnet_set_arith(self.handle, self.arith), self.handle, "affnet_set_arith")

    def pyramid_views(self, image=0):
        pyr = []
        base = image * lib.affnet_pyramid_image_stride(self.handle)
        for o, (h, w) in enumerate(self.plan.sizes):
            levels = []
            for l in range(self.plan.levels_per_octave):
                off = base + lib.affnet_pyramid_level_offset(self.handle, o, l)
                levels.append(self._ws_f32[off:off + h * w].view(1, 1, h, w))
            pyr.append(levels)
        return pyr

    def affmap_views(self, image=0):
        base = image * lib.affnet_affmap_image_stride(self.handle)
        out = []
        for o, (h, w) in enumerate(self.plan.sizes):
            off = base + lib.affnet_affmap_offset(self.handle, o)
            out.append(self._ws_f32[off:off + 4 * h * w].view(1, 4, h, w))
        return out

    def counter_view(self, which=0):
        off, stride = lib.affnet_counter_offset(self.handle, which), lib.affnet_counter_stride(self.handle)
        return self.workspace.view(torch.int32)[off:off + stride * self.batch:stride]

    def read_counts(self, allow_empty=False):
        out = (C.c_int32 * 4)()
        rc = lib.affnet_read_counts(self.handle, C.byref(out), stream_of(self.device))
        if not (allow_empty and rc == _lib.ERR_EMPTY):
            check(rc, self.handle, "affnet_read_counts")
        return list(out)

    def __del__(self):
        try:
            if self.handle:
                lib.affnet_ctx_destroy(self.handle)
                self.handle = None
        except Exception:
            pass


def pack_state_dict(kind, sd, winograd=False):
    conv_idx, bn_idx = (0, 3, 6, 9, 12, 15), (1, 4, 7, 10, 13, 16)

    def f32(name):
        return sd[name].detach().to("cpu", torch.float32).contiguous()

    keep = []
    convs = [f32("features.%d.weight" % i) for i in conv_idx]
    means = [f32("features.%d.running_mean" % i) for i in bn_idx]
    vars_ = [f32("features.%d.running_var" % i) for i in bn_idx]
    head_w = f32("features.19.weight")
    head_b = f32("features.19.bias") if "features.19.bias" in sd else None
    if kind == _lib.NET_AFFNET_FULLCONV and head_b is None:
        raise ValueError("AffNetFastFullConv: features.19.bias missing from the state dict")
    hbm = f32("features.20.running_mean") if kind == _lib.NET_HARDNET else None
    hbv = f32("features.20.running_var") if kind == _lib.NET_HARDNET else None
    keep += convs + means + vars_ + [head_w, head_b, hbm, hbv]
    arr = lambda ts: (C.c_void_p * 6)(*[t.data_ptr() for t in ts])
    n = lib.affnet_cnn32_packed_floats(kind)
    out = torch.empty(n, dtype=torch.float32)
    rc = lib.affnet_cnn32_pack_weights(kind, arr(convs), arr(means), arr(vars_), ptr(head_w), ptr(head_b), ptr(hbm), ptr(hbv), ptr(out))
    check(rc, None, "affnet_cnn32_pack_weights")
    del keep
    if not winograd:
        offs = [lib.affnet_cnn32_winograd_offset(kind, i) for i in range(6)]
        offs = [o for o in offs if o >= 0]
        if offs:
            out = out[:min(offs)].clone()
    return out


def save_flat_weights(kind, sd, path):
    conv_idx, bn_idx = (0, 3, 6, 9, 12, 15), (1, 4, 7, 10, 13, 16)
    names = ["features.%d.weight" % i for i in conv_idx] + ["features.%d.running_mean" % i for i in bn_idx] + \
            ["features.%d.running_var" % i for i in bn_idx] + ["features.19.weight"]
    names += ["features.20.running_mean", "features.20.running_var"] if kind == _lib.NET_HARDNET else ["features.19.bias"]
    flat = np.concatenate([sd[n].detach().to("cpu", torch.float32).contiguous().numpy().reshape(-1) for n in names])
    with open(path, "wb") as f:
        f.write(b"AFNW0001")
        f.write(np.array([kind, flat.size], dtype=np.int32).tobytes())
        f.write(flat.astype(np.float32).tobytes())
    return flat.size


def cnn_forward(kind, packed, patches, scratch=None, arith=0):
    require_cuda(patches, "patches")
    if patches.dim() == 4:
        if patches.size(1) != 1:
            raise ValueError("expected single-channel patches")
        patches = patches[:, 0]
    if tuple(patches.shape[1:]) != (32, 32):
        raise ValueError("the HIP CNN kernels are specialised for 32x32 patches, got %s" % (tuple(patches.shape),))
    patches = patches.contiguous().float()
    if packed.numel() != lib.affnet_cnn32_packed_floats(kind):
        raise ValueError("packed blob of %d floats, the kernels of net kind %d read %d (pack_state_dict(..., winograd=True))"
                         % (packed.numel(), kind, lib.affnet_cnn32_packed_floats(kind)))
    n = patches.size(0)
    dev = patches.device
    out = torch.empty((n, 128) if kind == _lib.NET_HARDNET else (n, 2, 2), dtype=torch.float32, device=dev)
    if n == 0:
        return out
    if scratch is None:
        scratch = torch.empty(n * ((8192 + 512) if kind == _lib.NET_HARDNET else 144), dtype=torch.float32, device=dev)
    ctx = utility_ctx(dev, arith)
    rc = lib.affnet_cnn32_forward(ctx, kind, ptr(packed), ptr(patches), None, n, ptr(out), ptr(scratch), stream_of(dev))
    check(rc, ctx, "affnet_cnn32_forward")
    return out


def fullconv_forward(packed, img, arith=0):
    img = img.contiguous().float()
    h, w = img.size(2), img.size(3)
    nbytes = lib.affnet_fullconv_scratch_bytes(h, w)
    if nbytes == 0:
        raise ValueError("image %dx%d too small for AffNetFastFullConv (this library requires H, W >= 34; the reference's LocalNorm2d(33) needs 17)" % (w, h))
    dev = img.device
    scratch = torch.empty(nbytes // 4, dtype=torch.float32, device=dev)
    out = torch.empty(1, 4, h, w, dtype=torch.float32, device=dev)
    ctx = utility_ctx(dev, arith)
    check(lib.affnet_fullconv_forward(ctx, ptr(packed), ptr(img), h, w, ptr(out), ptr(scratch), stream_of(dev)), ctx, "affnet_fullconv_forward")
    return out


def local_norm(img):
    require_cuda(img, "image")
    img = img.contiguous().float()
    out = torch.empty_like(img)
    ctx = utility_ctx(img.device)
    check(lib.affnet_local_norm(ctx, ptr(img), ptr(out), img.size(2), img.size(3), stream_of(img.device)), ctx, "affnet_local_norm")
    return out


def base_grid(ps):
    buf = (C.c_float * ps)()
    check(lib.affnet_host_base_grid(ps, buf), None, "affnet_host_base_grid")
    return np.array(buf, dtype=np.float32)
```

include/affnet_hip.h:

```cpp
#ifndef AFFNET_HIP_H
#define AFFNET_HIP_H

#include <stddef.h>
#include <stdint.h>

#ifdef __cplusplus
extern "C" {
#endif

#define AFFNET_OK 0
#define AFFNET_ERR_INVALID (-1)
#define AFFNET_ERR_HIP (-2)
#define AFFNET_ERR_CAPACITY (-3)
#define AFFNET_ERR_EMPTY (-4)

#define AFFNET_MAX_OCTAVES 16
#define AFFNET_MAX_LEVELS 8
#define AFFNET_MAX_TAPS 37

#define AFFNET_NET_AFFNET 0
#define AFFNET_NET_ORINET 1
#define AFFNET_NET_HARDNET 2
#define AFFNET_NET_AFFNET_FULLCONV 3

#define AFFNET_ARITH_FP32_MFMA 0
#define AFFNET_ARITH_FP32_SPLIT3 1
#define AFFNET_ARITH_FP32_SPLIT2H 2

typedef struct affnet_ctx affnet_ctx;

typedef struct affnet_config {
    int32_t height, width;
    int32_t n_octaves;
    int32_t levels_per_octave;
    int32_t oct_h[AFFNET_MAX_OCTAVES];
    int32_t oct_w[AFFNET_MAX_OCTAVES];
    float level_sigma[AFFNET_MAX_OCTAVES][AFFNET_MAX_LEVELS];
    float level_sigma4[AFFNET_MAX_OCTAVES][AFFNET_MAX_LEVELS];
    double level_sigma_px[AFFNET_MAX_OCTAVES][AFFNET_MAX_LEVELS];
    int32_t first_blur_taps;
    float first_blur[AFFNET_MAX_TAPS * AFFNET_MAX_TAPS];
    int32_t level_blur_taps[AFFNET_MAX_LEVELS];
    float level_blur[AFFNET_MAX_LEVELS][AFFNET_MAX_TAPS * AFFNET_MAX_TAPS];
    int32_t level_blur0_taps[AFFNET_MAX_LEVELS];
    float level_blur0[AFFNET_MAX_LEVELS][AFFNET_MAX_TAPS * AFFNET_MAX_TAPS];
    int32_t lazy_shape_rows;
    int32_t onepass;
    float mr_size;
    float threshold;
    int32_t num_features;
    int32_t num_prefilter;
    int32_t max_raw_per_octave_div;
    int32_t max_keep;
    int32_t batch;
    int32_t baum_iters;
    int32_t arith;
} affnet_config;

int affnet_config_fill(affnet_config* cfg, int height, int width, int n_levels, double init_sigma, int border, double mr_size,
                       double threshold, int num_features, int num_prefilter, int batch, int baum_iters);


int affnet_ctx_create(affnet_ctx** out, int device, const affnet_config* cfg);
void affnet_ctx_destroy(affnet_ctx* ctx);
const char* affnet_last_error(const affnet_ctx* ctx);
const char* affnet_version(void);
int affnet_set_arith(affnet_ctx* ctx, int arith);
int affnet_get_arith(const affnet_ctx* ctx);

size_t affnet_workspace_bytes(const affnet_ctx* ctx);
int affnet_bind_workspace(affnet_ctx* ctx, void* d_workspace, size_t bytes);
int64_t affnet_pyramid_level_offset(const affnet_ctx* ctx, int octave, int level);
int64_t affnet_pyramid_image_stride(const affnet_ctx* ctx);
int affnet_batch(const affnet_ctx* ctx);
int affnet_capacity_prefilter(const affnet_ctx* ctx);
int affnet_capacity_final(const affnet_ctx* ctx);


int affnet_gauss_blur(affnet_ctx* ctx, const float* d_in, float* d_out, int h, int w,
                      const float* h_taps, int k, void* stream);

int affnet_pyramid_build(affnet_ctx* ctx, const float* d_img, void* stream);

int affnet_hessian_response(affnet_ctx* ctx, const float* d_in, float* d_out, int h, int w,
                            float sigma4, void* stream);

int affnet_detect(affnet_ctx* ctx, float* d_resp, float* d_lafs, int32_t* d_ids,
                  int32_t* d_count, void* stream);

int affnet_detect_responses(affnet_ctx* ctx, const float* d_responses, float* d_resp, float* d_lafs, int32_t* d_ids,
                            int32_t* d_count, void* stream);

int affnet_laf_grid_sample(affnet_ctx* ctx, const float* d_img, int h, int w,
                           const float* d_lafs, int n, int ps, float* d_out, void* stream);

int affnet_pyr_grid_sample(affnet_ctx* ctx, const float* d_lafs, const int32_t* d_ids,
                           const int32_t* d_count, int n_max, int ps, float* d_out, void* stream);


size_t affnet_cnn32_packed_floats(int net_kind);
int64_t affnet_cnn32_winograd_offset(int net_kind, int layer);
int affnet_cnn32_pack_weights(int net_kind, const float* const* conv_w, const float* const* bn_mean,
                              const float* const* bn_var, const float* head_w, const float* head_b,
                              const float* head_bn_mean, const float* head_bn_var, float* h_out);

int affnet_cnn32_forward(affnet_ctx* ctx, int net_kind, const float* d_packed, const float* d_patches,
                         const int32_t* d_count, int n_max, float* d_out, float* d_scratch, void* stream);

int affnet_cnn32_forward_pyr(affnet_ctx* ctx, int net_kind, const float* d_packed, const float* d_lafs,
                             const int32_t* d_ids, const int32_t* d_count, int n_max, float* d_out,
                             float* d_scratch, void* stream);


int affnet_local_norm(affnet_ctx* ctx, const float* d_in, float* d_out, int h, int w, void* stream);

size_t affnet_fullconv_scratch_bytes(int h, int w);

int affnet_fullconv_forward(affnet_ctx* ctx, const float* d_packed, const float* d_img, int h, int w, float* d_out, float* d_scratch,
                            void* stream);

int affnet_nms2d(affnet_ctx* ctx, const float* d_in, float* d_out, int h, int w, float threshold, void* stream);


#define AFFNET_HC_ORIENTATION 0
#define AFFNET_HC_BAUMBERG 1

int affnet_handcrafted_forward(affnet_ctx* ctx, int kind, const float* d_patches, int n, const float* h_weights, float* d_out,
                               float* d_angles, void* stream);
int affnet_handcrafted_forward_pyr(affnet_ctx* ctx, int kind, const float* d_lafs, const int32_t* d_ids, const int32_t* d_count,
                                   int n_max, const float* h_weights, float* d_out, void* stream);


int affnet_sift_host_window(int patch_size, float* h_out);
int affnet_sift_forward(affnet_ctx* ctx, const float* d_patches, int n, const float* d_window, float clipval, float* d_desc, void* stream);
int affnet_sift_forward_pyr(affnet_ctx* ctx, const float* d_lafs_norm, const int32_t* d_ids, const int32_t* d_count, int n_max,
                            const float* d_window, float clipval, float* d_desc, void* stream);


size_t affnet_tfeat_packed_floats(void);
int affnet_tfeat_pack_weights(const float* conv1_w, const float* conv1_b, const float* conv2_w, const float* conv2_b, const float* cls_w,
                              const float* cls_b, float* h_out);
size_t affnet_tfeat_scratch_floats(int rows);
int affnet_tfeat_forward(affnet_ctx* ctx, const float* d_packed, const float* d_patches, const int32_t* d_count, int n_max, float* d_desc,
                         float* d_scratch, void* stream);
int affnet_tfeat_forward_pyr(affnet_ctx* ctx, const float* d_packed, const float* d_lafs_norm, const int32_t* d_ids, const int32_t* d_count,
                             int n_max, float* d_desc, float* d_scratch, void* stream);


int affnet_shape_filter_select(affnet_ctx* ctx, const float* d_resp_in, const float* d_lafs_in,
                               const int32_t* d_ids_in, const float* d_A, const int32_t* d_count_in,
                               float* d_resp_out, float* d_lafs_out, int32_t* d_ids_out,
                               int32_t* d_count_out, void* stream);

int affnet_shape_iterate(affnet_ctx* ctx, const float* d_A, float* d_base, const float* d_lafs, const int32_t* d_count, int mode,
                         float* d_lafs_out, void* stream);

int affnet_apply_rotation(affnet_ctx* ctx, float* d_lafs, const float* d_R, const int32_t* d_count,
                          int n_max, void* stream);

int affnet_scale_lafs(affnet_ctx* ctx, const float* d_in, float* d_out, const int32_t* d_count, int n_max,
                      int w, int h, int inverse, void* stream);

int affnet_lafs_to_ellipses(affnet_ctx* ctx, const float* d_lafs, const int32_t* d_count, int n_max, float* d_out, void* stream);

int affnet_ellipses_to_lafs(affnet_ctx* ctx, const float* d_ell, const int32_t* d_count, int n_max, float* d_lafs, void* stream);

int affnet_level_select(affnet_ctx* ctx, const float* d_lafs_px, const int32_t* d_count, int n_max,
                        int ps, int32_t* d_ids, float* d_lafs_norm, void* stream);


size_t affnet_match_scratch_bytes(int n1, int n2);

int affnet_distance_matrix(affnet_ctx* ctx, const float* d_desc1, int n1, const float* d_desc2, int n2, int dim, float* d_out,
                           void* d_scratch, void* stream);

int affnet_match_snn(affnet_ctx* ctx, const float* d_desc1, int n1, const float* d_desc2, int n2, int dim, float snn_threshold,
                     float* d_min_dist, int32_t* d_idx, float* d_min2_dist, int32_t* d_tent, int32_t* d_count, void* d_scratch,
                     void* stream);

int affnet_reproject_lafs(affnet_ctx* ctx, const float* d_lafs, int n, const float* h_H, float* d_out, void* stream);

int affnet_centre_nn(affnet_ctx* ctx, const float* d_query_lafs, int nq, const float* d_ref_lafs, int nr, float* d_min_dist,
                     int32_t* d_idx, void* stream);


typedef struct affnet_nets {
    const float* d_affnet;
    const float* d_orinet;
    const float* d_hardnet;
    const float* h_orientation_window;
    const float* h_baumberg_window;
} affnet_nets;

int affnet_extract_features(affnet_ctx* ctx, const affnet_nets* nets, const float* d_img, int do_ori,
                            float* d_lafs_px, float* d_resp, int32_t* d_ids, float* d_desc,
                            int32_t* d_count, void* stream);

int affnet_detect_image(affnet_ctx* ctx, const float* d_img, void* stream);
int affnet_detect_image_responses(affnet_ctx* ctx, const float* d_responses, void* stream);
int affnet_describe_detected(affnet_ctx* ctx, const affnet_nets* nets, int do_ori, float* d_lafs_px, float* d_resp,
                             int32_t* d_ids, float* d_desc, int32_t* d_count, void* stream);

int affnet_detect_image_onepass(affnet_ctx* ctx, const float* d_packed_fullconv, const float* d_img, void* stream);
int affnet_detect_image_onepass_responses(affnet_ctx* ctx, const float* d_packed_fullconv, const float* d_responses, void* stream);

int affnet_detected_list(affnet_ctx* ctx, float* d_resp, float* d_lafs, int32_t* d_ids, int32_t* d_count, void* stream);
int affnet_load_frames(affnet_ctx* ctx, const float* d_lafs, int normalised, const float* d_resp, const int32_t* d_ids,
                       const int32_t* d_count, int n_max, int ps, void* stream);

int affnet_describe_frames(affnet_ctx* ctx, const affnet_nets* nets, const float* d_img, const float* d_lafs_px, const float* d_resp_in,
                           const int32_t* d_count_in, int n_max, int do_ori, float* d_lafs_px_out, float* d_resp, int32_t* d_ids,
                           float* d_desc, int32_t* d_count, void* stream);

int64_t affnet_affmap_offset(const affnet_ctx* ctx, int octave);
int64_t affnet_affmap_image_stride(const affnet_ctx* ctx);

int affnet_graph_capture_extract(affnet_ctx* ctx, const affnet_nets* nets, const float* d_img, int do_ori, float* d_lafs_px, float* d_resp,
                                 int32_t* d_ids, float* d_desc, int32_t* d_count, void* stream);
int affnet_graph_launch(affnet_ctx* ctx, void* stream);

#define AFFNET_PROFILE_STAGES 8
int affnet_profile_enable(affnet_ctx* ctx, int on);
// ... 14 lines not shown
```

include/affnet_hip_probes.h:

```cpp
#ifndef AFFNET_HIP_PROBES_H
#define AFFNET_HIP_PROBES_H

#include "affnet_hip.h"

#ifdef __cplusplus
extern "C" {
#endif

int affnet_cnn32_probe(const float* d_packed, int layer, int probe, int reps, int n_blocks, float* d_out, void* stream);

int affnet_debug_stream(const void* d_src, void* d_dst, size_t n_bytes, int width, int mode, int halo, void* stream);

int affnet_split3_gemm(const float* d_A, const float* d_Bt, int M, int N, int K, int mode, float* d_C, void* stream);
int affnet_split3_rate(int reps, int terms, int n_blocks, float* d_out, void* stream);

#ifdef __cplusplus
}
#endif
#endif
```

Measured before the change: 1.457 million.

## Run AffNet shape pass with Winograd conv, re-evaluating near-threshold rows exactly

```diff
diff --git a/affnet_amd/SparseImgRepresenter.py b/affnet_amd/SparseImgRepresenter.py
--- a/affnet_amd/SparseImgRepresenter.py
+++ b/affnet_amd/SparseImgRepresenter.py
@@ -40,6 +40,7 @@
         self.max_keep = 16384
         self.raw_div = 4
         self.lazy_shape_rows = -1
+        self.shape_form = 1
 
     def _context(self, x, allow_batch=False):
         engine.require_cuda(x, "image")
@@ -56,6 +57,8 @@
                                        float(self.th), self.num, pre, self.max_keep, batch=x.size(0), baum_iters=self.num_Baum_iters, raw_div=self.raw_div,
                                        lazy_shape_rows=self.lazy_shape_rows, arith=self.arith)
             self._ctx_key = key
+        if self._ctx.shape_form != int(self.shape_form):
+            self._ctx.set_shape_form(self.shape_form)
         return self._ctx
 
     def _publish_pyramid(self, ctx):
@@ -217,6 +220,8 @@
                                         self.max_keep, batch=x.size(0), baum_iters=self.num_Baum_iters, raw_div=self.raw_div,
                                         lazy_shape_rows=self.lazy_shape_rows, arith=self.arith)
             self._fctx_key = key
+        if self._fctx.shape_form != int(self.shape_form):
+            self._fctx.set_shape_form(self.shape_form)
         return self._fctx
 
     def enqueue_frames(self, x, LAFs, responses=None, counts=None, do_ori=True, desc=None):
@@ -398,7 +403,11 @@
         aff_native = self.num_Baum_iters == 0 or self._native(self.AffNet)
         ori_native = (not do_ori) or self._native(self.OriNet)
         if aff_native and ori_native:
-            r = self.run(x, do_ori=do_ori)
+            form, self.shape_form = self.shape_form, 0
+            try:
+                r = self.run(x, do_ori=do_ori)
+            finally:
+                self.shape_form = form
             return r["LAFs"], r["responses"]
         return self._staged(x, do_ori)
 
diff --git a/affnet_amd/_lib.py b/affnet_amd/_lib.py
--- a/affnet_amd/_lib.py
+++ b/affnet_amd/_lib.py
@@ -22,6 +22,7 @@
     if int(arith) not in (ARITH_FP32_MFMA, ARITH_FP32_SPLIT3, ARITH_FP32_SPLIT2H):
         raise ValueError("arith must be AFFNET_ARITH_FP32_MFMA (0), AFFNET_ARITH_FP32_SPLIT3 (1) or AFFNET_ARITH_FP32_SPLIT2H (2)")
     return int(arith)
+SHAPE_FORM_DIRECT, SHAPE_FORM_WINOGRAD = 0, 1
 OK, ERR_INVALID, ERR_HIP, ERR_CAPACITY, ERR_EMPTY = 0, -1, -2, -3, -4
 
 
@@ -60,6 +61,8 @@
     "affnet_version": (C.c_char_p, []),
     "affnet_set_arith": (_I, [_P, _I]),
     "affnet_get_arith": (_I, [_P]),
+    "affnet_set_shape_form": (_I, [_P, _I]),
+    "affnet_get_shape_form": (_I, [_P]),
     "affnet_workspace_bytes": (_SZ, [_P]),
     "affnet_bind_workspace": (_I, [_P, _P, _SZ]),
     "affnet_pyramid_level_offset": (C.c_int64, [_P, _I, _I]),
@@ -139,6 +142,7 @@
     "affnet_split3_gemm": (_I, [_P, _P, _I, _I, _I, _I, _P, _P]),
     "affnet_split3_rate": (_I, [_I, _I, _I, _P, _P]),
     "affnet_debug_stream": (_I, [_P, _P, _SZ, _I, _I, _I, _P]),
+    "affnet_probe_shape_offsets": (_I, [_P, C.POINTER(C.c_int64 * 3)]),
 }
 
 
diff --git a/affnet_amd/csrc/cnn32.hip b/affnet_amd/csrc/cnn32.hip
--- a/affnet_amd/csrc/cnn32.hip
+++ b/affnet_amd/csrc/cnn32.hip
@@ -28,11 +28,11 @@
     return ctx->arith == AFFNET_ARITH_FP32_SPLIT2H ? 2 : (ctx->arith == AFFNET_ARITH_FP32_SPLIT3 ? 1 : 0);
 }
 
-static int trunk_launch(affnet_ctx* ctx, const CnnCall& c, const NetLayout& L, dim3 grid) {
+static int trunk_launch(affnet_ctx* ctx, const CnnCall& c, const NetLayout& L, dim3 grid, bool wino, const int32_t* reeval, int shape_op) {
     CnnArgs a;
     a.packed = c.packed; a.off = to_offsets(L, ctx->arith);
-    a.wino_u = nullptr;
-    if (c.kind == AFFNET_NET_ORINET && ctx->arith == AFFNET_ARITH_FP32_MFMA) {
+    a.wino_u = nullptr; a.reeval = reeval;
+    if ((c.kind == AFFNET_NET_ORINET || wino) && ctx->arith == AFFNET_ARITH_FP32_MFMA) {
         const int rc = aff_wino_derive_u(ctx, c.kind, c.packed, L, c.st, &a.wino_u);
         if (rc) return rc;
     }
@@ -40,13 +40,14 @@
     a.out = (c.dbg_layer < 0) ? c.scratch : c.out;
     a.dbg_layer = c.dbg_layer; a.dbg_out = c.dbg_out; a.dbg_time = ctx->dbg_time;
     a.row_begin = c.row_begin; a.skip_cnt = c.skip_cnt; a.skip_n = c.skip_n;
-    a.shape_cnt = (c.fuse && c.shape_op) ? c.fuse->cnt : nullptr; a.shape_op = c.shape_op;
+    a.shape_cnt = (c.fuse && shape_op) ? c.fuse->cnt : nullptr; a.shape_op = shape_op;
     a.s3_alt = ctx->split3_variant;
     PyrSrc ps;
     aff_fill_pyr_src(ctx, &ps);
     static_assert(AFFNET_NET_AFFNET == 0 && AFFNET_NET_ORINET == 1 && AFFNET_NET_HARDNET == 2, "trunk getter order");
     static TrunkKernel (*const trunk_of[3])(int, bool) = {aff_trunk_affnet, aff_trunk_orinet, aff_trunk_hardnet};
-    hipLaunchKernelGGL(trunk_of[c.kind](aff_arith_index(ctx), a.dbg_time || c.dbg_layer >= 0), grid, dim3(512), 0, c.st, a, ps);
+    const bool stamps = a.dbg_time || c.dbg_layer >= 0;
+    hipLaunchKernelGGL(wino ? aff_trunk_affnet_wino(stamps) : trunk_of[c.kind](aff_arith_index(ctx), stamps), grid, dim3(512), 0, c.st, a, ps);
     AFF_LAUNCH_CHECK(ctx);
     return AFFNET_OK;
 }
@@ -57,8 +58,16 @@
     if (rc || rows == 0) return rc;
     const NetLayout L = net_layout(c.kind);
     const int B = c.patches ? 1 : ctx->B;
-    rc = trunk_launch(ctx, c, L, dim3(rows, B));
+    const bool form1 = c.wino_reeval && c.kind == AFFNET_NET_AFFNET && c.fuse && c.dbg_layer < 0 && ctx->arith == AFFNET_ARITH_FP32_MFMA;
+    rc = trunk_launch(ctx, c, L, dim3(rows, B), form1, nullptr, c.shape_op);
     if (rc) return rc;
+    if (form1) {
+        int32_t* flags = reinterpret_cast<int32_t*>(c.scratch + (size_t)B * c.n_max * HEAD_PART_AFF);
+        rc = aff_margin_affnet(ctx, c, L, rows, B, flags);
+        if (rc) return rc;
+        rc = trunk_launch(ctx, c, L, dim3(rows, B), false, flags, 0);
+        if (rc) return rc;
+    }
     if (c.dbg_layer < 0 && c.kind != AFFNET_NET_HARDNET) {
         rc = c.kind == AFFNET_NET_AFFNET ? aff_finish_affnet(ctx, c, L, rows, B) : aff_finish_orinet(ctx, c, L, rows, B);
         if (rc) return rc;
@@ -95,6 +104,7 @@
     c.row_begin = row_begin; c.row_count = row_count;
     c.skip_cnt = lazy ? ctx->cnt : nullptr; c.skip_n = ctx->cfg.num_features;
     c.fuse = &sf; c.shape_op = shape_op;
+    c.wino_reeval = ctx->shape_form == AFFNET_SHAPE_FORM_WINOGRAD;
     return cnn_launch(ctx, c);
 }
 
diff --git a/affnet_amd/csrc/cnn_heads.hip b/affnet_amd/csrc/cnn_heads.hip
--- a/affnet_amd/csrc/cnn_heads.hip
+++ b/affnet_amd/csrc/cnn_heads.hip
@@ -4,6 +4,19 @@
 
 #include "cnn_mfma.h"
 #include "shape_filter.h"
+
+__device__ __forceinline__ f32x4 affnet_head_to_a(const float* __restrict__ part, const float* __restrict__ hb, size_t pidx) {
+    const f32x4* pp = reinterpret_cast<const f32x4*>(part + pidx * HEAD_PART_AFF);
+    f32x4 r[8];
+#pragma unroll
+    for (int w = 0; w < 8; ++w) r[w] = pp[w];
+    const f32x4 s = ((r[0] + r[1]) + (r[2] + r[3])) + ((r[4] + r[5]) + (r[6] + r[7]));
+    const float x0 = tanhf(s.x + hb[0]), x1 = tanhf(s.y + hb[1]), x2 = tanhf(s.z + hb[2]);
+    const float a00 = 1.0f + x0, a01 = 0.0f * x0, a10 = x1, a11 = 1.0f + x2;
+    const float det = sqrtf(fabsf(a00 * a11 - a10 * a01 + 1e-10f));
+    const float b2a2 = sqrtf(a01 * a01 + a00 * a00);
+    return (f32x4){b2a2 / det, 0.0f * det, (a11 * a01 + a10 * a00) / (b2a2 * det), det / b2a2};
+}
 
 __global__ __launch_bounds__(256) void affnet_finish_kernel(const float* __restrict__ part, const float* __restrict__ hb,
                                                             const int32_t* __restrict__ count, int n_max, float* __restrict__ out, int row_begin,
@@ -20,22 +33,27 @@
     }
     if (row >= n || skip) return;
     float* o = out + 4 * pidx;
-    const f32x4* pp = reinterpret_cast<const f32x4*>(part + pidx * HEAD_PART_AFF);
-    f32x4 r[8];
-#pragma unroll
-    for (int w = 0; w < 8; ++w) r[w] = pp[w];
-    const f32x4 s = ((r[0] + r[1]) + (r[2] + r[3])) + ((r[4] + r[5]) + (r[6] + r[7]));
-    const float x0 = tanhf(s.x + hb[0]), x1 = tanhf(s.y + hb[1]), x2 = tanhf(s.z + hb[2]);
-    const float a00 = 1.0f + x0, a01 = 0.0f * x0, a10 = x1, a11 = 1.0f + x2;
-    const float det = sqrtf(fabsf(a00 * a11 - a10 * a01 + 1e-10f));
-    const float b2a2 = sqrtf(a01 * a01 + a00 * a00);
-    const float o0 = b2a2 / det, o1 = 0.0f * det, o2 = (a11 * a01 + a10 * a00) / (b2a2 * det), o3 = det / b2a2;
+    const f32x4 A = affnet_head_to_a(part, hb, pidx);
+    const float o0 = A.x, o1 = A.y, o2 = A.z, o3 = A.w;
     o[0] = o0; o[1] = o1; o[2] = o2; o[3] = o3;
     if (sf.key) {
         const size_t bi = blockIdx.y;
         aff_shape_filter_row(sf.resp + bi * n_max, sf.lafs + bi * n_max * 6, o0, o1, o2, o3, row, sf.key + bi * n_max, sf.good + bi * n_max,
                              sf.cnt + bi * CNT_TOTAL);
     }
+}
+
+__global__ __launch_bounds__(256) void affnet_margin_kernel(const float* __restrict__ part, const float* __restrict__ hb, const int32_t* __restrict__ count,
+                                                            int n_max, int row_begin, int row_end, const int32_t* __restrict__ skip_cnt, int skip_n,
+                                                            const float* __restrict__ lafs, int32_t* __restrict__ flags, int32_t* __restrict__ cnt) {
+    const int row = row_begin + blockIdx.x * 256 + threadIdx.x;
+    const int n = min(count ? min(count[blockIdx.y], n_max) : n_max, row_end);
+    if (row >= n || lazy_skip(skip_cnt, skip_n, blockIdx.y)) return;
+    const size_t bi = blockIdx.y, pidx = bi * n_max + row;
+    const f32x4 A = affnet_head_to_a(part, hb, pidx);
+    const bool flag = aff_shape_margin_flag(lafs + bi * n_max * 6, A.x, A.y, A.z, A.w, row);
+    flags[pidx] = flag ? 1 : 0;
+    if (flag) atomicAdd(&cnt[bi * CNT_TOTAL + CNT_AFF_REEVAL], 1);
 }
 
 __global__ __launch_bounds__(256) void orinet_finish_kernel(const float* __restrict__ part, const float* __restrict__ hb,
@@ -282,6 +300,13 @@
     return AFFNET_OK;
 }
 
+int aff_margin_affnet(affnet_ctx* ctx, const CnnCall& c, const NetLayout& L, int rows, int B, int32_t* flags) {
+    hipLaunchKernelGGL(affnet_margin_kernel, dim3(aff_cdiv(rows, 256), B), dim3(256), 0, c.st, c.scratch, c.packed + L.head_b, c.count, c.n_max, c.row_begin,
+                       c.row_begin + rows, c.skip_cnt, c.skip_n, c.fuse->lafs, flags, c.fuse->cnt);
+    AFF_LAUNCH_CHECK(ctx);
+    return AFFNET_OK;
+}
+
 int aff_finish_orinet(affnet_ctx* ctx, const CnnCall& c, const NetLayout& L, int rows, int B) {
     DenormSel ds;
     memset(&ds, 0, sizeof(ds));
diff --git a/affnet_amd/csrc/cnn_trunk.h b/affnet_amd/csrc/cnn_trunk.h
--- a/affnet_amd/csrc/cnn_trunk.h
+++ b/affnet_amd/csrc/cnn_trunk.h
@@ -186,7 +186,9 @@
 
 template <int KIND, int NW, bool STAMPS, int S3 = 0>
 __global__ __launch_bounds__(NW * 64, (KIND == AFFNET_NET_HARDNET) ? NW / 4 : 4) void cnn32_trunk_kernel(CnnArgs a, PyrSrc ps) {
-    static_assert(S3 == 0 || S3 == 2 || S3 == 3, "S3 = number of terms of the split arithmetic");
+    static_assert(S3 == 0 || S3 == 2 || S3 == 3 || (S3 == 1 && KIND == AFFNET_NET_AFFNET), "S3 = number of terms of the split arithmetic; 1 = exact AffNet with Winograd conv1 / conv3");
+    constexpr bool EXACT = S3 <= 1;
+    constexpr bool WINO13 = (S3 == 0 && KIND == AFFNET_NET_ORINET) || S3 == 1;
     using S = TrunkShape<KIND, NW>;
     constexpr int CB = S::CB, NTHR = S::NTHR;
     static_assert((CB / 4) * LayC1::PSG <= TrunkLds<CB>::ACT && (CB / 2) * LayC3::PSG <= TrunkLds<CB>::ACT, "LDS layout");
@@ -198,11 +200,12 @@
     const int prow = blockIdx.x + a.row_begin;
     if (KIND == AFFNET_NET_AFFNET && a.shape_cnt && blockIdx.x == 0 && threadIdx.x == 0) {
         int32_t* c = a.shape_cnt + (size_t)blockIdx.y * CNT_TOTAL;
-        if (a.shape_op == 1) { c[CNT_SURVIVED] = 0; c[CNT_SURVIVED1] = 0; c[CNT_AFF_EVAL] = 0; }
+        if (a.shape_op == 1) { c[CNT_SURVIVED] = 0; c[CNT_SURVIVED1] = 0; c[CNT_AFF_EVAL] = 0; c[CNT_AFF_REEVAL] = 0; }
         else if (a.shape_op == 2) c[CNT_SURVIVED1] = c[CNT_SURVIVED];
     }
     if (prow >= n || lazy_skip(a.skip_cnt, a.skip_n, blockIdx.y, CNT_SURVIVED)) return;
     const size_t pidx = (size_t)blockIdx.y * a.n_max + prow;
+    if (KIND == AFFNET_NET_AFFNET && a.reeval && a.reeval[pidx] == 0) return;
     const int tid = threadIdx.x, wave = tid >> 6, lane = tid & 63;
     if (KIND == AFFNET_NET_HARDNET) __builtin_amdgcn_s_setprio(3);
     CNN_STAMP(0);
@@ -216,7 +219,7 @@
     f32x4 b1[1][S::T1N];
     f32x4 Ur[4];
     if constexpr (S3 == 0 && KIND == AFFNET_NET_AFFNET) prefetch_b0<NW, CB, 32, S::T1M, S::T1N, 1>(a.packed + a.off.w[1], b1, wave, lane);
-    if constexpr (S3 == 0 && KIND == AFFNET_NET_ORINET) wino_prefetch_u_row<NW, CB, CB, 32, Wino16::NB1>(a.wino_u, Ur, wave, lane);
+    if constexpr (WINO13) wino_prefetch_u_row<NW, CB, CB, 32, Wino16::NB1>(a.wino_u, Ur, wave, lane);
 
     constexpr int PPT = 1024 / NTHR;
     constexpr int RPT = 32 / PPT;
@@ -245,7 +248,7 @@
         const int y = e < 34 ? 0 : (e < 68 ? 33 : 1 + ((e - 68) >> 1)), x = e < 34 ? e : (e < 68 ? e - 34 : ((e - 68) & 1) * 33);
         patch[y * WP32 + x] = 0.0f;
     }
-    if constexpr (S3 == 0) zero_halo<LayC0, NTHR>(act, CB);
+    if constexpr (EXACT) zero_halo<LayC0, NTHR>(act, CB);
     else if constexpr (S3 == 2) zero_halo_q<typename SplitLays<CB>::LR0, NTHR>(act);
     else zero_halo_q<typename SplitLays<CB>::LQH, NTHR>(act);
     float sum = 0.f;
@@ -369,12 +372,12 @@
         __syncthreads();
         CNN_STAMP(12);
         if (STAMPS && a.dbg_layer == 5) { dump_planes<4 * CB, LayC5, NTHR>(act, a.dbg_out); return; }
-    } else if constexpr (S3 == 0) {
+    } else if constexpr (EXACT) {
         constexpr int T1M = S::T1M, T1N = S::T1N, T2M = S::T2M, T2N = S::T2N, T4M = S::T4M, T4N = S::T4N;
         static_assert(NW == 8 && CB == 16, "Wino16 describes the 16-channel trunks on 8 waves");
         f32x4 b4[S::G4][T4N];
         f32x4 bias4[T4N];
-        if constexpr (KIND == AFFNET_NET_ORINET) {
+        if constexpr (WINO13) {
             constexpr int NB1 = Wino16::NB1, NB3 = Wino16::NB3;
             {
                 f32x4 acc[T1M][T1N];
diff --git a/affnet_amd/csrc/cnn_trunk_affnet.hip b/affnet_amd/csrc/cnn_trunk_affnet.hip
--- a/affnet_amd/csrc/cnn_trunk_affnet.hip
+++ b/affnet_amd/csrc/cnn_trunk_affnet.hip
@@ -6,3 +6,7 @@
                                         {cnn32_trunk_kernel<AFFNET_NET_AFFNET, 8, false, 2>, cnn32_trunk_kernel<AFFNET_NET_AFFNET, 8, true, 2>}};
     return k[arith_index][stamps];
 }
+
+TrunkKernel aff_trunk_affnet_wino(bool stamps) {
+    return stamps ? cnn32_trunk_kernel<AFFNET_NET_AFFNET, 8, true, 1> : cnn32_trunk_kernel<AFFNET_NET_AFFNET, 8, false, 1>;
+}
diff --git a/affnet_amd/csrc/common.h b/affnet_amd/csrc/common.h
--- a/affnet_amd/csrc/common.h
+++ b/affnet_amd/csrc/common.h
@@ -30,6 +30,7 @@
     CNT_SURVIVED1,
     CNT_SEL_EQ_TOTAL,
     CNT_SEL_TIE_LO, CNT_SEL_TIE_HI,
+    CNT_AFF_REEVAL,
     CNT_POS0 = AFFNET_MAX_OCTAVES + 24,
     CNT_HYP0 = AFFNET_MAX_OCTAVES + 24 + (AFFNET_MAX_LEVELS - 2) * AFFNET_MAX_OCTAVES,
     CNT_TOTAL = AFFNET_MAX_OCTAVES + 24 + (AFFNET_MAX_LEVELS - 2) * AFFNET_MAX_OCTAVES + 8 * AFFNET_MAX_OCTAVES
@@ -96,6 +97,7 @@
     std::vector<hipEvent_t> prof_ev;
     int prof_calls = 0;
     unsigned long long* dbg_time = nullptr;
+    int shape_form = AFFNET_SHAPE_FORM_WINOGRAD;
     int arith = AFFNET_ARITH_FP32_MFMA;
     int split3_variant = 0;
     hipGraph_t graph = nullptr;
@@ -189,6 +191,7 @@
     const float* packed;
     NetOffsets off;
     const float* wino_u;
+    const int32_t* reeval;
     const float* patches;
     const float* lafs;
     const int32_t* ids;
@@ -237,6 +240,7 @@
     int row_begin = 0, row_count = -1;
     const int32_t* skip_cnt = nullptr; int skip_n = 0;
     const ShapeFuse* fuse = nullptr; int shape_op = 0;
+    bool wino_reeval = false;
     float* rot_lafs = nullptr; const DenormSel* denorm = nullptr;
 };
 
@@ -278,12 +282,14 @@
                                    int n_max, float* out, float* scratch, hipStream_t st);
 
 TrunkKernel aff_trunk_affnet(int arith_index, bool stamps);
+TrunkKernel aff_trunk_affnet_wino(bool stamps);
 TrunkKernel aff_trunk_orinet(int arith_index, bool stamps);
 TrunkKernel aff_trunk_hardnet(int arith_index, bool stamps);
 int aff_wino_u_ensure(affnet_ctx* ctx);
 int aff_wino_derive_u(affnet_ctx* ctx, int kind, const float* packed, const NetLayout& L, hipStream_t st, const float** u);
 
 int aff_finish_affnet(affnet_ctx* ctx, const CnnCall& c, const NetLayout& L, int rows, int B);
+int aff_margin_affnet(affnet_ctx* ctx, const CnnCall& c, const NetLayout& L, int rows, int B, int32_t* flags);
 int aff_finish_orinet(affnet_ctx* ctx, const CnnCall& c, const NetLayout& L, int rows, int B);
 int aff_hardnet_head(affnet_ctx* ctx, const CnnCall& c, const NetLayout& L, int B);
 
diff --git a/affnet_amd/csrc/context.hip b/affnet_amd/csrc/context.hip
--- a/affnet_amd/csrc/context.hip
+++ b/affnet_amd/csrc/context.hip
@@ -216,6 +216,14 @@
 }
 extern "C" int affnet_get_arith(const affnet_ctx* ctx) { return ctx ? ctx->arith : AFFNET_ERR_INVALID; }
 
+extern "C" int affnet_set_shape_form(affnet_ctx* ctx, int form) {
+    if (!ctx) return AFFNET_ERR_INVALID;
+    if (form != AFFNET_SHAPE_FORM_DIRECT && form != AFFNET_SHAPE_FORM_WINOGRAD) return aff_fail(ctx, AFFNET_ERR_INVALID, "shape form=%d (AFFNET_SHAPE_FORM_*)", form);
+    ctx->shape_form = form;
+    return AFFNET_OK;
+}
+extern "C" int affnet_get_shape_form(const affnet_ctx* ctx) { return ctx ? ctx->shape_form : AFFNET_ERR_INVALID; }
+
 extern "C" size_t affnet_workspace_bytes(const affnet_ctx* ctx) { return ctx ? ctx->ws_bytes : 0; }
 
 extern "C" int affnet_capacity_prefilter(const affnet_ctx* ctx) { return ctx ? ctx->cap_pre : 0; }
@@ -230,8 +238,8 @@
 extern "C" int64_t affnet_pyramid_image_stride(const affnet_ctx* ctx) { return ctx ? (int64_t)ctx->pyr_stride : 0; }
 
 extern "C" int64_t affnet_counter_offset(const affnet_ctx* ctx, int which) {
-    if (!ctx || ctx->ws_bytes == 0 || which < 0 || which > 3) return -1;
-    const int idx = which == 0 ? CNT_OVERFLOW : (which == 1 ? CNT_DET : (which == 2 ? CNT_SHAPED : CNT_AFF_EVAL));
+    if (!ctx || ctx->ws_bytes == 0 || which < 0 || which > 4) return -1;
+    const int idx = which == 0 ? CNT_OVERFLOW : (which == 1 ? CNT_DET : (which == 2 ? CNT_SHAPED : (which == 3 ? CNT_AFF_EVAL : CNT_AFF_REEVAL)));
     return (int64_t)(ctx->off_cnt / sizeof(int32_t)) + idx;
 }
 extern "C" int64_t affnet_counter_stride(const affnet_ctx* ctx) { return ctx ? (int64_t)CNT_TOTAL : 0; }
diff --git a/affnet_amd/csrc/debug.hip b/affnet_amd/csrc/debug.hip
--- a/affnet_amd/csrc/debug.hip
+++ b/affnet_amd/csrc/debug.hip
@@ -64,3 +64,11 @@
     }
     return hipGetLastError() == hipSuccess ? AFFNET_OK : AFFNET_ERR_HIP;
 }
+
+extern "C" int affnet_probe_shape_offsets(const affnet_ctx* ctx, int64_t out[3]) {
+    if (!ctx || !ctx->ws || !out) return AFFNET_ERR_INVALID;
+    out[0] = (int64_t)(reinterpret_cast<const char*>(ctx->st_A) - ctx->ws) / 4;
+    out[1] = (int64_t)(reinterpret_cast<const char*>(ctx->st_hard_scratch) - ctx->ws) / 4 + (int64_t)ctx->B * ctx->cap_pre * HEAD_PART_AFF;
+    out[2] = (int64_t)(reinterpret_cast<const char*>(ctx->st_det_lafs) - ctx->ws) / 4;
+    return AFFNET_OK;
+}
diff --git a/affnet_amd/csrc/pipeline.hip b/affnet_amd/csrc/pipeline.hip
--- a/affnet_amd/csrc/pipeline.hip
+++ b/affnet_amd/csrc/pipeline.hip
@@ -127,6 +127,14 @@
         rc = aff_shape_select(ctx, ctx->st_det_resp, ctx->st_det_lafs, ctx->st_det_ids, ctx->st_A, det_count, d_resp, ctx->st_lafs_shaped, d_ids,
                               d_count, st);
         if (rc) return rc;
+    } else if (nets->d_affnet && ctx->cfg.baum_iters <= 1 && N > 0) {
+        rc = aff_affnet_filter_rows(ctx, nets->d_affnet, ctx->st_det_resp, ctx->st_det_lafs, ctx->st_det_ids, det_count, ctx->st_A, ctx->st_hard_scratch,
+                                    0, P, false, 1, st);
+        if (rc) return rc;
+        aff_prof_mark(ctx, 3, st);
+        rc = aff_shape_select(ctx, ctx->st_det_resp, ctx->st_det_lafs, ctx->st_det_ids, ctx->st_A, det_count, d_resp, ctx->st_lafs_shaped, d_ids,
+                              d_count, st);
+        if (rc) return rc;
     } else if (nets->d_affnet || baumberg) {
         rc = shape_pass(ctx->st_det_lafs, ctx->st_A);
         if (rc) return rc;
diff --git a/affnet_amd/csrc/shape_filter.h b/affnet_amd/csrc/shape_filter.h
--- a/affnet_amd/csrc/shape_filter.h
+++ b/affnet_amd/csrc/shape_filter.h
@@ -26,6 +26,36 @@
     good[i] = ok ? 1 : 0;
     key[i] = resp[i] * (ok ? 1.0f : 0.0f);
     if (ok) atomicAdd(&cnt[CNT_SURVIVED], 1);
+}
+
+#define AFF_MARGIN_D1 1e-5f
+#define AFF_MARGIN_CORNER 1e-5f
+#define AFF_MARGIN_RATIO_REL 1e-3f
+__device__ __forceinline__ bool aff_shape_margin_flag(const float* __restrict__ lafs, float a00, float a01, float a10, float a11, int i) {
+    const float* L = lafs + 6 * (size_t)i;
+    const float n00 = fmaf(a01, L[3], a00 * L[0]), n01 = fmaf(a01, L[4], a00 * L[1]);
+    const float n10 = fmaf(a11, L[3], a10 * L[0]), n11 = fmaf(a11, L[4], a10 * L[1]);
+    const float cx = L[2], cy = L[5];
+    const float tr = a00 + a11;
+    const float p1 = a00 * a11, p2 = a10 * a01;
+    const float d1 = tr * tr - 4.0f * (p1 - p2);
+    const float mk = d1 > 0.f ? 1.0f : 0.0f;
+    const float dl = sqrtf(fabsf(d1));
+    const float l1 = mk * (tr + dl) / 2.0f + 1000.0f * (1.0f - mk);
+    const float l2 = mk * (tr - dl) / 2.0f + 0.0001f * (1.0f - mk);
+    const float ratio = fabsf(l1 / (l2 + 1e-8f));
+    const float iso = (a00 - a11) * (a00 - a11);
+    bool certain = iso >= AFF_MARGIN_D1 && fabsf(ratio - 6.0f) >= 6.0f * AFF_MARGIN_RATIO_REL &&
+                   fabsf(ratio - (float)(1.0 / 6.0)) >= AFF_MARGIN_RATIO_REL / 6.0f;
+    const float px[4] = {-1.f, -1.f, 1.f, 1.f}, py[4] = {-1.f, 1.f, -1.f, 1.f};
+#pragma unroll
+    for (int k = 0; k < 4; ++k) {
+        const float ox = fmaf(cx, 1.0f, fmaf(n01, py[k], n00 * px[k]));
+        const float oy = fmaf(cy, 1.0f, fmaf(n11, py[k], n10 * px[k]));
+        certain = certain && fabsf(ox) >= AFF_MARGIN_CORNER && fabsf(ox - 1.0f) >= AFF_MARGIN_CORNER && fabsf(oy) >= AFF_MARGIN_CORNER &&
+                  fabsf(oy - 1.0f) >= AFF_MARGIN_CORNER;
+    }
+    return !certain;
 }
 
 __device__ __forceinline__ int aff_level_argmin(float q0, float q1, float q3, float q4, float ps, const LevelTable& lt) {
diff --git a/affnet_amd/engine.py b/affnet_amd/engine.py
--- a/affnet_amd/engine.py
+++ b/affnet_amd/engine.py
@@ -43,6 +43,7 @@
         self.cfg = self.plan.fill_config(mr_size, threshold, num_features, num_prefilter, max_keep, raw_div=raw_div, batch=self.batch, baum_iters=baum_iters,
                                          onepass=onepass, lazy_shape_rows=lazy_shape_rows, arith=arith)
         self.arith = _lib.arith_code(arith)
+        self.shape_form = _lib.SHAPE_FORM_WINOGRAD
         self.device = device
         self.handle = C.c_void_p()
         idx = device.index if device.index is not None else torch.cuda.current_device()
@@ -58,6 +59,10 @@
     def set_arith(self, arith):
         self.arith = _lib.arith_code(arith)
         check(lib.affnet_set_arith(self.handle, self.arith), self.handle, "affnet_set_arith")
+
+    def set_shape_form(self, form):
+        check(lib.affnet_set_shape_form(self.handle, int(form)), self.handle, "affnet_set_shape_form")
+        self.shape_form = int(form)
 
     def pyramid_views(self, image=0):
         pyr = []
diff --git a/include/affnet_hip.h b/include/affnet_hip.h
--- a/include/affnet_hip.h
+++ b/include/affnet_hip.h
@@ -68,6 +68,11 @@
 int affnet_set_arith(affnet_ctx* ctx, int arith);
 int affnet_get_arith(const affnet_ctx* ctx);
 
+#define AFFNET_SHAPE_FORM_DIRECT 0
+#define AFFNET_SHAPE_FORM_WINOGRAD 1
+int affnet_set_shape_form(affnet_ctx* ctx, int form);
+int affnet_get_shape_form(const affnet_ctx* ctx);
+
 size_t affnet_workspace_bytes(const affnet_ctx* ctx);
 int affnet_bind_workspace(affnet_ctx* ctx, void* d_workspace, size_t bytes);
 int64_t affnet_pyramid_level_offset(const affnet_ctx* ctx, int octave, int level);
diff --git a/include/affnet_hip_probes.h b/include/affnet_hip_probes.h
--- a/include/affnet_hip_probes.h
+++ b/include/affnet_hip_probes.h
@@ -14,6 +14,8 @@
 int affnet_split3_gemm(const float* d_A, const float* d_Bt, int M, int N, int K, int mode, float* d_C, void* stream);
 int affnet_split3_rate(int reps, int terms, int n_blocks, float* d_out, void* stream);
 
+int affnet_probe_shape_offsets(const affnet_ctx* ctx, int64_t out[3]);
+
 #ifdef __cplusplus
 }
 #endif
```

Result: faster. 1.513 million (median of 6 runs) (+3.8%).
